# Huiweizhou/GCGCN

Measured on NVIDIA B200. Metric: document graphs/sec (fwd+bwd graph blocks), higher is better.
Workload: dtype f32

## Files before the change

### gcgcn_b200/_lib.py

```python
from __future__ import annotations

import ctypes
import glob
import os
import subprocess
import threading
from ctypes import c_float, c_int32, c_int64, c_size_t, c_uint64, c_void_p, c_char_p, POINTER

_HERE = os.path.dirname(os.path.abspath(__file__))
LIB_NAME = "libgcgcn_b200.so"
LIB_PATH = os.path.join(_HERE, LIB_NAME)
CSRC = os.path.join(_HERE, "csrc")
INCLUDE = os.path.join(os.path.dirname(_HERE), "include")

NVCC_FLAGS = [
    "-gencode", "arch=compute_100a,code=sm_100a", "-lineinfo", "-O3", "-std=c++17",
    "-Xcompiler", "-fPIC", "-shared",
]

F32, BF16 = 0, 1
STACK_RELU, STACK_RESIDUAL, STACK_LINEAR = 1, 2, 4


class GcgcnError(RuntimeError):
    pass


class Dropout(ctypes.Structure):
    _fields_ = [("seed", c_uint64), ("p_att", c_float), ("p_gcn", c_float)]


class Batch(ctypes.Structure):
    _fields_ = [
        ("num_docs", c_int32), ("total_nodes", c_int32), ("total_pairs", c_int64),
        ("max_nodes", c_int32), ("reserved", c_int32),
        ("node_ptr", c_void_p), ("pair_ptr", c_void_p), ("row_doc", c_void_p),
        ("doc_order", c_void_p), ("class_end", c_int32 * 4),
        ("tile_doc", c_void_p), ("num_tiles", c_int32), ("tile_rows", c_int32),
    ]


class EdgeTablesC(ctypes.Structure):
    _fields_ = [
        ("num_tokens", c_int32), ("num_slots", c_int32), ("num_pairs", c_int32), ("att_total", c_int32),
        ("dis_plus", c_int32), ("reserved", c_int32),
        ("tok_first", c_void_p), ("tok_slot_lo", c_void_p), ("tok_slot_hi", c_void_p),
        ("slot_tok0", c_void_p), ("slot_len", c_void_p), ("slot_span", c_void_p), ("slot_att", c_void_p),
        ("slot_rowi", c_void_p), ("slot_rowj", c_void_p), ("pair_idx", c_void_p), ("pair_slot_ptr", c_void_p),
        ("pair_denom", c_void_p), ("node_ctr_ptr", c_void_p), ("node_ctr", c_void_p),
        ("num_active_docs", c_int32), ("max_active_len", c_int32),
        ("adoc_tok0", c_void_p), ("adoc_len", c_void_p), ("adoc_slot_lo", c_void_p), ("adoc_slot_hi", c_void_p),
    ]


class RankResult(ctypes.Structure):
    _fields_ = [
        ("count", c_int64), ("total_recall", c_int64), ("best_pos", c_int64), ("w", c_int64),
        ("auc", ctypes.c_double), ("ign_auc", ctypes.c_double),
        ("f1", c_float), ("theta", c_float), ("f1_at_w", c_float), ("precision_at_w", c_float),
        ("recall_at_w", c_float), ("ign_f1", c_float), ("ign_f1_at_w", c_float), ("reserved", c_float),
    ]


def sources():
    return sorted(glob.glob(os.path.join(CSRC, "*.cu")))


def build(force: bool = False, verbose: bool = False) -> str:
    from concurrent.futures import ThreadPoolExecutor
    srcs = sources()
    hdrs = glob.glob(os.path.join(CSRC, "*.cuh")) + glob.glob(os.path.join(INCLUDE, "*.h"))
    newest_hdr = max(os.path.getmtime(p) for p in hdrs)
    if not force and os.path.exists(LIB_PATH):
        if os.path.getmtime(LIB_PATH) >= max([newest_hdr] + [os.path.getmtime(p) for p in srcs]):
            return LIB_PATH
    nvcc = os.environ.get("NVCC", "nvcc")
    objdir = os.path.join(os.path.dirname(_HERE), "build", "obj")
    os.makedirs(objdir, exist_ok=True)
    compile_flags = [f for f in NVCC_FLAGS if f != "-shared"]

    def compile_one(src):
        obj = os.path.join(objdir, os.path.basename(src)[:-3] + ".o")
        if not force and os.path.exists(obj) and os.path.getmtime(obj) >= max(newest_hdr, os.path.getmtime(src)):
            return obj, None
        cmd = [nvcc] + compile_flags + ["-I", INCLUDE, "-c", "-o", obj, src]
        if verbose:
            print(" ".join(cmd))
        res = subprocess.run(cmd, capture_output=True, text=True)
        return obj, (None if res.returncode == 0 else res.stdout + res.stderr)

    with ThreadPoolExecutor(max_workers=min(len(srcs), os.cpu_count() or 4)) as pool:
        results = list(pool.map(compile_one, srcs))
    errors = [e for _, e in results if e]
    if errors:
        raise GcgcnError("nvcc failed:\n" + "\n".join(errors))
    cmd = [nvcc, "-gencode", "arch=compute_100a,code=sm_100a", "-shared", "-o", LIB_PATH] + [o for o, _ in results]
    res = subprocess.run(cmd, capture_output=True, text=True)
    if res.returncode != 0:
        raise GcgcnError("nvcc link failed:\n" + res.stdout + res.stderr)
    return LIB_PATH


_P = c_void_p
_BT = POINTER(Batch)
_DP = POINTER(Dropout)
_ET = POINTER(EdgeTablesC)

SIGNATURES = {
    "gcgcn_version": (c_char_p, []),
    "gcgcn_last_error": (c_char_p, []),
    "gcgcn_launch_count": (c_uint64, []),
    "gcgcn_set_tile_blocks": (c_int32, [c_int32]),
    "gcgcn_device_info": (c_int32, [POINTER(c_int32)] * 3),
    "gcgcn_timing_begin": (c_int32, [_P]),
    "gcgcn_timing_end": (c_int32, [_P, c_char_p, c_size_t]),
    "gcgcn_workspace_bytes": (c_size_t, [c_int32, c_int64, c_int32]),
    "gcgcn_pool_fwd": (c_int32, [_P, _P, _P, _P, c_int32, _P, _P]),
    "gcgcn_pool_bwd": (c_int32, [_P, _P, _P, _P, c_int32, _P, _P]),
    "gcgcn_edge_mean_fwd": (c_int32, [_BT, _P, c_int32, _P, _P]),
    "gcgcn_edge_mean_bwd": (c_int32, [_BT, _P, c_int32, _P, _P]),
    "gcgcn_gat_fwd": (c_int32, [_BT, _P, _P, c_int32, _P, _P, _P, _P, c_int32, _P, _P, _P, _P,
                                _P, c_size_t, _P]),
    "gcgcn_gat_bwd": (c_int32, [_BT, _P, _P, c_int32, _P, _P, _P, c_int32, _P, _P, _P, _P,
                                _P, _P, _P, _P, _P, _P, c_size_t, _P]),
    "gcgcn_mha_fwd": (c_int32, [_BT, c_int32, _P, _P, _P, _P, _P, _P, _P, _P, c_size_t, _P]),
    "gcgcn_mha_bwd": (c_int32, [_BT, c_int32, _P, _P, _P, _P, _P, _P, _P, _P, _P, _P, c_size_t, _P]),
    "gcgcn_graphconv_stack_fwd": (c_int32, [_BT, c_int32, c_int32, c_int32, c_int32, c_int32]
                                  + [_P] * 13 + [_P, c_size_t, _P]),
    "gcgcn_graphconv_stack_bwd": (c_int32, [_BT, c_int32, c_int32, c_int32, c_int32, c_int32]
                                  + [_P] * 20 + [_P, c_size_t, _P]),
    "gcgcn_block_supported": (c_int32, [_BT, c_int32, c_int32, c_int32]),
    "gcgcn_dropout_mask": (c_int32, [c_uint64, c_int32, c_float, c_int64, _P, _P]),
    "gcgcn_mha_stack_fwd": (c_int32, [_BT, c_int32, c_int32] + [_P] * 15 + [_DP, _P, c_size_t, _P]),
    "gcgcn_mha_stack_bwd": (c_int32, [_BT, c_int32, c_int32] + [_P] * 22 + [_DP, _P, c_size_t, _P]),
    "gcgcn_pack_stack_weights": (c_int32, [_P, _P, c_int32, c_int32, c_int32, _P, _P, _P, _P]),
    "gcgcn_unpack_stack_grads": (c_int32, [_P, _P, _P, c_int32, c_int32, c_int32, _P, _P, _P]),
    "gcgcn_gat_collapse_fwd": (c_int32, [_P] * 8 + [c_int32, _P, _P]),
    "gcgcn_gat_collapse_bwd": (c_int32, [_P] * 8 + [c_int32] + [_P] * 8 + [_P]),
    "gcgcn_pack_rows": (c_int32, [_P, c_int32, c_int32, _P, _P]),
    "gcgcn_pair_gather_fwd": (c_int32, [_BT, _P, c_int32, _P, c_int32, _P, _P, _P, _P, _P, _P, _P]),
    "gcgcn_pair_gather_bwd": (c_int32, [_BT, _P, _P, c_int32, c_int32, c_int32, _P, _P, _P, _P,
                                        _P, c_size_t, _P]),
    "gcgcn_pair_dense_fwd": (c_int32, [_BT, _P, _P, _P, _P, _P, _P, _P, _P, _P]),
    "gcgcn_pair_dense_ws_bytes": (c_size_t, [c_int32]),
    "gcgcn_pair_dense_bwd": (c_int32, [_BT, _P, _P, _P, _P, c_int32, _P, _P, _P, _P, _P, _P, c_size_t, _P]),
    "gcgcn_block_saved_bytes": (c_size_t, [c_int32, c_int64, c_int32]),
    "gcgcn_caggc_fwd": (c_int32, [_BT, c_int32, _P, _P, c_int32] + [_P] * 8 + [_P, _P, _DP, _P, c_size_t, _P]),
    "gcgcn_caggc_bwd": (c_int32, [_BT, c_int32, _P, _P, c_int32] + [_P] * 6 + [_P, _P]
                        + [_P] * 10 + [_DP, _P, c_size_t, _P]),
    "gcgcn_maggc_fwd": (c_int32, [_BT, c_int32, c_int32, _P, _P, c_int32] + [_P] * 7
                        + [_P, _P, _DP, _P, c_size_t, _P]),
    "gcgcn_maggc_bwd": (c_int32, [_BT, c_int32, c_int32, _P, c_int32] + [_P] * 5 + [_P, _P]
                        + [_P] * 9 + [_DP, _P, c_size_t, _P]),
    "gcgcn_expand_pair_context": (c_int32, [_P, c_int32, c_int32, c_int32, c_int32, c_int32, _P, _P, _P, _P]),
    "gcgcn_edgefeat_ws_bytes": (c_size_t, [c_int32, c_int32, c_int32, c_int32, c_int64]),
    "gcgcn_word_table_fwd": (c_int32, [_P, _P, _P, _P, c_int32, _P, _P]),
    "gcgcn_word_table_bwd": (c_int32, [_P, _P, _P, _P, c_int32, _P, _P, _P, c_size_t, _P]),
    "gcgcn_word_pool_fwd": (c_int32, [_ET, _P, _P, _P, _P, _P]),
    "gcgcn_word_pool_bwd": (c_int32, [_ET, _P, _P, _P, _P, _P, _P, c_size_t, _P]),
    "gcgcn_sent_pool_fwd": (c_int32, [_ET, _P, _P, _P, _P, _P, _P, _P, _P]),
    "gcgcn_sent_pool_bwd": (c_int32, [_ET, c_int32] + [_P] * 10 + [_P, c_size_t, _P]),
    "gcgcn_edge_fill_fwd": (c_int32, [_P, _P, _P, c_int32, c_int64, c_int32, _P, _P]),
    "gcgcn_edge_fill_bwd": (c_int32, [_P, _P, c_int32, c_int64, c_int32, _P, _P, _P, c_size_t, _P]),
    "gcgcn_colsum": (c_int32, [_P, c_int32, c_int32, c_int32, _P, _P, c_size_t, _P]),
    "gcgcn_bilinear_ws_bytes": (c_size_t, [c_int32, c_int32]),
    "gcgcn_bilinear_fwd": (c_int32, [_P, _P, _P, _P, c_int32, c_int32, c_int32, _P, c_int32, _P, c_size_t, _P]),
    "gcgcn_bilinear_bwd_ws_bytes": (c_size_t, [c_int32, c_int32]),
    "gcgcn_bilinear_bwd": (c_int32, [_P, _P, _P, _P, _P, c_int32, c_int32, c_float, _P, _P, _P, _P, c_size_t, _P]),
    "gcgcn_bilinear_reduce_fwd": (c_int32, [_P, _P, _P, c_int32, c_int32, c_int32, _P, c_int32, _P]),
    "gcgcn_bilinear_outer_bwd": (c_int32, [_P, c_int32, _P, c_int32, c_int32, _P, _P]),
    "gcgcn_bilinear_dt_bwd": (c_int32, [_P, c_int32, _P, c_int32, c_int32, _P, _P]),
    "gcgcn_doc_bias_fwd": (c_int32, [_BT, _P, c_int32, _P, _P]),
    "gcgcn_doc_bias_bwd": (c_int32, [_BT, _P, c_int32, _P, _P]),
    "gcgcn_pair_bce_fwd": (c_int32, [_BT, _P, _P, c_int32, _P, _P]),
    "gcgcn_pair_bce_bwd": (c_int32, [_BT, _P, _P, c_int32, _P, _P, _P]),
    "gcgcn_rank_ws_bytes": (c_size_t, [c_int64]),
    "gcgcn_rank_candidates": (c_int32, [_BT, _P, c_int32, _P, _P, c_int64, _P, _P, _P, _P]),
    "gcgcn_rank_sort": (c_int32, [_P, _P, c_int64, _P, _P, _P, c_size_t, _P]),
    "gcgcn_rank_curve": (c_int32, [_P, _P, c_int64, c_int64, c_int32, ctypes.c_double, _P, _P, c_size_t, _P]),
    "gcgcn_rank_decode": (c_int32, [_P, _P, c_int64, c_int64, _P, _P, c_int32, c_int32, _P, _P, _P, _P, _P, _P]),
    "gcgcn_adam_step": (c_int32, [_P, _P, _P, _P, c_int64] + [c_float] * 6 + [c_int32, _P]),
    "gcgcn_gemm": (c_int32, [c_int32, c_int32, c_int32, c_int32, c_int32, c_float, _P, c_int32, _P,
                             c_int32, c_float, _P, c_int32, _P, _P, c_size_t, _P]),
}

_lib = None
_lock = threading.Lock()


def load() -> ctypes.CDLL:
    global _lib
    if _lib is not None:
        return _lib
    with _lock:
        if _lib is not None:
            return _lib
        if not os.path.exists(LIB_PATH):
            raise GcgcnError(
                f"{LIB_PATH} not found: run `python -c 'import __graft_entry__ as g; g.build()'`. "
                "gcgcn_b200 has no CPU or PyTorch fallback.")
        lib = ctypes.CDLL(LIB_PATH)
        for name, (res, args) in SIGNATURES.items():
            fn = getattr(lib, name)
            fn.restype = res
            fn.argtypes = args
        _lib = lib
    return _lib


def call(name: str, *args) -> None:
    lib = load()
    rc = getattr(lib, name)(*args)
    if rc != 0:
        raise GcgcnError(f"{name} failed (code {rc}): {lib.gcgcn_last_error().decode()}")


def launch_count() -> int:
    return int(load().gcgcn_launch_count())


def set_tile_blocks(enable: bool) -> bool:
    return bool(load().gcgcn_set_tile_blocks(1 if enable else 0))


def timing_begin(stream: int) -> None:
    call("gcgcn_timing_begin", stream)


def timing_end(stream: int) -> dict:
    buf = ctypes.create_string_buffer(1 << 16)
    call("gcgcn_timing_end", stream, buf, len(buf))
    out = {}
    for line in buf.value.decode().splitlines():
        name, cnt, ms, work = line.split("\t")
        out[name] = (int(cnt), float(ms), float(work))
    return out


def version() -> str:
    return load().gcgcn_version().decode()
```

### gcgcn_b200/csrc/api.cu

```cuda
#include <cstring>
#include <map>
#include <mutex>
#include <string>
#include <vector>

#include "common.cuh"

namespace gcgcn {

int launch_node_score(const float* x, const float* u, const float* c, float* ux, int rows, cudaStream_t st);
int launch_edge_fwd(const gcgcn_batch* bt, const void* e, int dtype, const float* v, const float* ux,
                    const uint8_t* mask, const float* keep, float* P, float* A, float* ebar, cudaStream_t st);
int launch_edge_bwd(const gcgcn_batch* bt, const void* e, int dtype, const float* v, const float* dS,
                    const float* debar, void* de, float* dv_partial, cudaStream_t st);
int edge_bwd_grid();
int node_bwd_grid();
int launch_softmax_bwd(const gcgcn_batch* bt, int heads, const float* P, const float* keep, const float* dA,
                       const uint8_t* mask, float* dS, cudaStream_t st);
int launch_gat_node_bwd(const gcgcn_batch* bt, const float* dS, const float* x, const float* u, float* dx,
                        float* partial, int* parts_out, cudaStream_t st);
int launch_reduce_partials(const float* partial, int parts, int width, float* out0, int width0, float* out1,
                           cudaStream_t st);
int launch_mha_fwd(const gcgcn_batch* bt, int heads, const float* q, const float* keep, float* P, float* A,
                   cudaStream_t st);
int launch_mha_bwd(const gcgcn_batch* bt, int heads, const float* q, const float* dS, float* dq, cudaStream_t st);
int launch_stack_fwd(const gcgcn_batch* bt, int heads, int layers, int slab, int flags, const float* A, float* Z,
                     const float* E, const float* Winner, const float* keep, const float* x, float* G, float* F,
                     float* frag_ws, cudaStream_t st);
int launch_stack_bwd(const gcgcn_batch* bt, int heads, int layers, int slab, int flags, const float* A, const float* Z,
                     const float* G, const float* Winner, const float* keep, const float* dF, float* dZ,
                     float* dE, float* dA, float* frag_ws, cudaStream_t st);
bool block_kernels_usable(const gcgcn_batch* bt, int heads, int layers, int slab, bool mha);
bool set_tile_blocks(bool on);
int launch_block_fwd(const gcgcn_batch* bt, int heads, int layers, const float* A, const float* q, float* P,
                     float* Z, const float* E, const float* Winner, const float* x, float* G, float* F,
                     float* frag_ws, const BlockDrop& drop, cudaStream_t st);
int launch_block_bwd(const gcgcn_batch* bt, int heads, int layers, int out_mode, const float* A, const float* q,
                     const float* Z, const float* G, const float* Winner, const float* dF, float* dZ, float* dE,
                     float* dOut, float* frag_ws, const BlockDrop& drop, cudaStream_t st);
int launch_dropout_mask(unsigned long long seed, uint32_t stream, uint32_t thr, float inv, long long count, float* out,
                        cudaStream_t st);
size_t block_frag_floats(int heads, int layers);
enum { ATT_GRAD_DA = 0, ATT_GRAD_DS = 1, ATT_GRAD_DQ = 2 };
int launch_gemm(int ta, int tb, int M, int N, int K, float alpha, const float* A, int lda, const float* B,
                int ldb, float beta, float* C, int ldc, const float* bias, void* ws, size_t ws_bytes,
                cudaStream_t st);
size_t gemm_presplit_bytes(int rows);
int launch_colsum(const float* X, int M, int N, int ldx, float* out, void* ws, size_t ws_bytes, cudaStream_t st);
int launch_gemm_batched(int ta, int tb, int M, int N, int K, float alpha, const float* A, int lda, const float* B,
                        int ldb, float beta, float* C, int ldc, int batch, long long sA, long long sB, long long sC,
                        void* ws, size_t ws_bytes, cudaStream_t st);
int launch_csr_gather(const float* src, const int* ptr, const int* idx, const float* w, int rows, float* out,
                      cudaStream_t st);
int launch_pair_gather_fwd(const gcgcn_batch* bt, const float* feat, int feat_w, const float* dis, int dis_w,
                           const int* h_idx, const int* t_idx, const int* dis_h, const int* dis_t, float* out_h,
                           float* out_t, cudaStream_t st);
int launch_pair_gather_bwd(const gcgcn_batch* bt, const float* dout_h, const float* dout_t, int feat_w,
                           int dis_w, int dis_rows, const int* dis_h, const int* dis_t, float* dfeat,
                           float* ddis, void* ws, size_t ws_bytes, cudaStream_t st);
int pair_dis_warps();
int launch_pair_dense_fwd(const gcgcn_batch* bt, const float* U, const float* Vd, const int* h_idx, const int* t_idx,
                          const int* dis_h, const int* dis_t, float* out_h, float* out_t, cudaStream_t st);
int launch_pair_dense_bwd(const gcgcn_batch* bt, const float* dout_h, const float* dout_t, const float* out_h,
                          const float* out_t, int dis_rows, const int* dis_h, const int* dis_t, float* dU, float* dVd,
                          float* dpre, void* ws, size_t ws_bytes, cudaStream_t st);
int launch_pack_stack(const float* const* wn_ptrs, const float* const* we_ptrs, int heads, int layers, int slab,
                      float* WnX, float* We, float* Winner, cudaStream_t st);
int launch_expand_pair_context(const int* slots, int num_slots, int n, int S, int L, int dis_plus, unsigned char* sen,
                               long long* pos_h, long long* pos_t, cudaStream_t st);
int launch_adam(float* p, const float* g, float* m, float* v, long long count, float lr, float b1, float b2,
                float eps, float wd, float gscale, int step, cudaStream_t st);
int launch_unpack_stack(const float* dWnX, const float* dWe, const float* dWinner, int heads, int layers, int slab,
                        float* dwn_flat, float* dwe_flat, cudaStream_t st);

int launch_word_table_fwd(const float* SF, const float* DF, const float* wa, const float* ba, int tokens, float* T,
                          cudaStream_t st);
int word_table_parts(int tokens);
int launch_word_table_bwd(const float* SF, const float* DF, const float* wa, const float* dT, int tokens, float* dSF,
                          float* out, float* partial, cudaStream_t st);
int launch_word_pool_fwd(const gcgcn_edge_tables* t, const float* T, const float* ctx, float* att, float* cwa,
                         cudaStream_t st);
int launch_word_pool_bwd(const gcgcn_edge_tables* t, const float* ctx, const float* att, const float* dcwa, float* dlog,
                         float* dctx, float* dT, cudaStream_t st);
int launch_sent_pool_fwd(const gcgcn_edge_tables* t, const float* cw, const float* sfeat, const float* nfeat,
                         const float* va, const float* ca, float* score, float* csa, cudaStream_t st);
int sent_pool_parts(int pairs);
int launch_sent_pool_bwd(const gcgcn_edge_tables* t, int total_nodes, const float* cw, const float* sfeat,
                         const float* nfeat, const float* va, const float* score, const float* dcsa, float* dcw,
                         float* dsfeat, float* dnfeat, float* out, float* dpre, float* partial, cudaStream_t st);
int launch_edge_fill_fwd(const float* bias, const float* rows, const void* pair_idx, int pairs, long long total_pairs,
                         int dtype, void* e, cudaStream_t st);
int edge_colsum_parts(long long total_pairs);
int launch_edge_fill_bwd(const void* de, const void* pair_idx, int pairs, long long total_pairs, int dtype, float* drows,
                         float* dbias, float* partial, cudaStream_t st);

int launch_bilinear_reduce(const float* Y, const float* t, const float* bias, int rows, int R, int accumulate, float* out,
                           int ldo, cudaStream_t st);
int launch_bilinear_finish(const float* part, long long ld, const float* bias, int rows, int R, int accumulate, float* out,
                           int ldo, cudaStream_t st);
int launch_gemm_rowop(int mode, int M, int N, int K, const float* A, int lda, const float* B, int ldb, const float* T,
                      float* out, long long ld, void* ws, size_t ws_bytes, cudaStream_t st);
int launch_gemm_wgrad_scaled(int M, int tiles, int K, const float* A, int lda, const float* T, const float* scale, int lds,
                             float beta, float* C, int ldc, void* ws, size_t ws_bytes, cudaStream_t st, void* pre_ws,
                             size_t pre_bytes);
int launch_bilinear_outer(const float* dout, int ldd, const float* t, int rows, int R, float* dY, cudaStream_t st);
int launch_bilinear_dt(const float* dout, int ldd, const float* Y, int rows, int R, float* dt, cudaStream_t st);
int launch_doc_bias_fwd(const gcgcn_batch* bt, const float* v, int R, float* z, cudaStream_t st);
int launch_doc_bias_bwd(const gcgcn_batch* bt, const float* dz, int R, float* dv, cudaStream_t st);
int launch_pair_bce_fwd(const gcgcn_batch* bt, const float* z, const float* y, int R, float* loss, cudaStream_t st);
int launch_pair_bce_bwd(const gcgcn_batch* bt, const float* z, const float* y, int R, const float* dloss, float* dz,
                        cudaStream_t st);

int launch_gat_collapse_fwd(const float* Wh, const float* bh, const float* Wt, const float* bt, const float* Wr,
                            const float* br, const float* w, const float* b, int hid, float* out, cudaStream_t st);
int launch_gat_collapse_bwd(const float* Wh, const float* bh, const float* Wt, const float* bt, const float* Wr,
                            const float* br, const float* w, const float* dout, int hid, float* dWh, float* dbh, float* dWt,
                            float* dbt, float* dWr, float* dbr, float* dw, float* db, cudaStream_t st);
int launch_pack_rows(const float* const* ptrs, int count, int elems, float* out, cudaStream_t st);
size_t rank_ws_bytes(long long count);
int launch_rank_candidates(const gcgcn_batch* bt, const float* z, const float* labels, const uint8_t* intrain, int R,
                           long long base_id, float* score, uint32_t* payload, unsigned long long* counters,
                           cudaStream_t st);
int launch_rank_sort(const float* score, const uint32_t* payload, long long count, uint32_t* sorted_key,
                     uint32_t* sorted_payload, void* ws, size_t ws_bytes, cudaStream_t st);
int launch_rank_curve(const uint32_t* key, const uint32_t* pay, long long count, long long T, int has_intrain,
                      double input_theta, gcgcn_rank_result* res, void* ws, size_t ws_bytes, cudaStream_t st);
int launch_rank_decode(const uint32_t* key, const uint32_t* pay, long long rows, const long long* doc_off,
                       const int* doc_n, int docs, int R, int* doc, int* row, int* col, int* rel, float* score,
                       cudaStream_t st);

std::atomic<uint64_t> g_launches{0};
std::atomic<bool> g_timing{false};

namespace {
// ... 363 lines not shown
    GCGCN_API_ENTER(stream);
    GCGCN_TRY(check_batch(bt));
    GCGCN_REQUIRE(heads >= 1 && D % heads == 0, "mha_bwd: head_num %d must divide %d", heads, D);
    if (bt->total_nodes == 0) return GCGCN_OK;
    GCGCN_TRY(check_device_ptr(x, "node_feat"));
    GCGCN_TRY(check_device_ptr(q, "q"));
    GCGCN_TRY(check_device_ptr(P, "P"));
    GCGCN_TRY(check_device_ptr(dA, "dA"));
    GCGCN_TRY(check_device_ptr(dx, "dx"));
    cudaStream_t st = static_cast<cudaStream_t>(stream);
    Arena ar(ws, ws_bytes);
    float* dS = ar.take<float>(static_cast<size_t>(bt->total_pairs) * heads);
    float* dq = ar.take<float>(static_cast<size_t>(bt->total_nodes) * D);
    float* gws = ar.take<float>(GEMM_WS_BYTES / sizeof(float));
    if (dS == nullptr || dq == nullptr || gws == nullptr)
        return fail(GCGCN_ERR_WORKSPACE, "mha_bwd: workspace too small");
    GCGCN_TRY(launch_softmax_bwd(bt, heads, P, keep, dA, nullptr, dS, st));
    GCGCN_TRY(launch_mha_bwd(bt, heads, q, dS, dq, st));
    GCGCN_TRY(launch_gemm(0, 0, bt->total_nodes, D, D, 1.f, dq, D, Wq, D, 0.f, dx, D, nullptr, gws, GEMM_WS_BYTES, st));
    if (dWq != nullptr)
        GCGCN_TRY(launch_gemm(1, 0, D, D, bt->total_nodes, 1.f, dq, D, x, D, 0.f, dWq, D, nullptr, gws, GEMM_WS_BYTES, st));
    if (dbq != nullptr) GCGCN_TRY(launch_colsum(dq, bt->total_nodes, D, D, dbq, gws, GEMM_WS_BYTES, st));
    return GCGCN_OK;
}

static int stack_fwd_impl(const gcgcn_batch* bt, int32_t heads, int32_t layers, int32_t in_dim, int32_t slab,
                          int32_t flags, const float* x, const float* ebar, const float* A, const float* q, float* P,
                          const float* WnX, const float* We, const float* Winner, const float* Wout,
                          const float* bout, const float* keep, float* Z, float* G, float* F, float* y, void* ws,
                          size_t ws_bytes, cudaStream_t st, const BlockDrop& drop = BlockDrop{}) {
    const bool linear = flags & GCGCN_STACK_LINEAR;
    const int HD = heads * slab, M = bt->total_nodes;
    Arena ar(ws, ws_bytes);
    float* E = ar.take<float>(static_cast<size_t>(M) * HD);
    float* gws = ar.take<float>(GEMM_WS_BYTES / sizeof(float));
    float* frag = (slab == D && layers > 1 && D % layers == 0) ? ar.take<float>(block_frag_floats(heads, layers)) : nullptr;
    if (E == nullptr || gws == nullptr) return fail(GCGCN_ERR_WORKSPACE, "stack_fwd: workspace too small");
    GCGCN_TRY(launch_gemm(0, 0, M, HD, in_dim, 1.f, x, in_dim, WnX, HD, 0.f, Z, HD, nullptr, gws, GEMM_WS_BYTES, st));
    GCGCN_TRY(launch_gemm(0, 0, M, HD, D, 1.f, ebar, D, We, HD, 0.f, E, HD, nullptr, gws, GEMM_WS_BYTES, st));
    float* Fout = linear ? F : y;
    if (q != nullptr)
        GCGCN_TRY(launch_block_fwd(bt, heads, layers, nullptr, q, P, Z, E, Winner, x, G, Fout, frag, drop, st));
    else if (drop_active(drop))
        GCGCN_TRY(launch_block_fwd(bt, heads, layers, A, nullptr, nullptr, Z, E, Winner, x, G, Fout, frag, drop, st));
    else
        GCGCN_TRY(launch_stack_fwd(bt, heads, layers, slab, flags, A, Z, E, Winner, keep, x, G, Fout, frag, st));
    if (linear)
        GCGCN_TRY(launch_gemm(0, 1, M, D, HD, 1.f, F, HD, Wout, HD, 0.f, y, D, bout, gws, GEMM_WS_BYTES, st));
    return GCGCN_OK;
}

int gcgcn_graphconv_stack_fwd(const gcgcn_batch* bt, int32_t heads, int32_t layers, int32_t in_dim,
                              int32_t slab, int32_t flags, const float* x, const float* ebar, const float* A,
                              const float* WnX, const float* We, const float* Winner, const float* Wout,
                              const float* bout, const float* keep, float* Z, float* G, float* F, float* y,
                              void* ws, size_t ws_bytes, void* stream) {
    GCGCN_API_ENTER(stream);
    GCGCN_TRY(check_batch(bt));
    GCGCN_REQUIRE(heads >= 1 && layers >= 1 && in_dim >= 1 && slab >= 1, "stack_fwd: bad heads/layers/widths");
    const bool linear = flags & GCGCN_STACK_LINEAR;
    GCGCN_REQUIRE(linear || heads == 1, "stack_fwd: without the output linear there can be only one head");
    GCGCN_REQUIRE(!(flags & GCGCN_STACK_RESIDUAL) || in_dim == slab,
                  "stack_fwd: the residual needs input width %d == output width %d", in_dim, slab);
    if (bt->total_nodes == 0) return GCGCN_OK;
    GCGCN_TRY(check_device_ptr(x, "node_feat"));
    GCGCN_TRY(check_device_ptr(ebar, "ebar"));
    GCGCN_TRY(check_device_ptr(A, "adj_matrix"));
    GCGCN_TRY(check_device_ptr(WnX, "WnX"));
    GCGCN_TRY(check_device_ptr(We, "We"));
    GCGCN_TRY(check_device_ptr(Z, "Z"));
    GCGCN_TRY(check_device_ptr(G, "G"));
    GCGCN_TRY(check_device_ptr(y, "y"));
    if (linear) GCGCN_TRY(check_device_ptr(F, "F"));
    return stack_fwd_impl(bt, heads, layers, in_dim, slab, flags, x, ebar, A, nullptr, nullptr, WnX, We, Winner, Wout,
                          bout, keep, Z, G, F, y, ws, ws_bytes, static_cast<cudaStream_t>(stream));
}

static int stack_bwd_impl(const gcgcn_batch* bt, int32_t heads, int32_t layers, int32_t in_dim, int32_t slab,
                          int32_t flags, int att_grad, const float* x, const float* ebar, const float* A,
                          const float* q, const float* WnX, const float* We, const float* Winner, const float* Wout,
                          const float* keep, const float* Z, const float* G, const float* F, const float* dy,
                          float* dx, float* debar, float* att_out, float* dWnX, float* dWe, float* dWinner,
                          float* dWout, float* dbout, void* ws, size_t ws_bytes, cudaStream_t st,
                          const BlockDrop& drop = BlockDrop{}) {
    const bool linear = flags & GCGCN_STACK_LINEAR;
    const int HD = heads * slab, M = bt->total_nodes, gd = slab / layers;
    Arena ar(ws, ws_bytes);
    float* dFbuf = linear ? ar.take<float>(static_cast<size_t>(M) * HD) : nullptr;
    float* dZ = ar.take<float>(static_cast<size_t>(M) * HD);
    float* dE = ar.take<float>(static_cast<size_t>(M) * HD);
    float* gws = ar.take<float>(GEMM_WS_BYTES / sizeof(float));
    float* frag = (slab == D && layers > 1 && D % layers == 0) ? ar.take<float>(block_frag_floats(heads, layers)) : nullptr;
    if ((linear && dFbuf == nullptr) || dZ == nullptr || dE == nullptr || gws == nullptr)
        return fail(GCGCN_ERR_WORKSPACE, "stack_bwd: workspace too small");
    const float* dF = dy;
    if (linear) {
        GCGCN_TRY(launch_gemm(0, 0, M, HD, D, 1.f, dy, D, Wout, HD, 0.f, dFbuf, HD, nullptr, gws, GEMM_WS_BYTES, st));
        if (dWout != nullptr)
            GCGCN_TRY(launch_gemm(1, 0, D, HD, M, 1.f, dy, D, F, HD, 0.f, dWout, HD, nullptr, gws, GEMM_WS_BYTES, st));
        if (dbout != nullptr) GCGCN_TRY(launch_colsum(dy, M, D, D, dbout, gws, GEMM_WS_BYTES, st));
        dF = dFbuf;
    }
    if (att_grad == ATT_GRAD_DA)
        GCGCN_TRY(launch_stack_bwd(bt, heads, layers, slab, flags, A, Z, G, Winner, keep, dF, dZ, dE, att_out, frag, st));
    else
        GCGCN_TRY(launch_block_bwd(bt, heads, layers, att_grad, A, q, Z, G, Winner, dF, dZ, dE, att_out, frag, drop, st));
    float beta = 0.f;
    if (flags & GCGCN_STACK_RESIDUAL) {
        float* Wsum = (linear && heads > 1 && slab == D && in_dim == D) ? ar.take<float>(static_cast<size_t>(D) * D) : nullptr;
        if (Wsum != nullptr) {
            wout_head_sum_kernel<<<ceil_div(D * D, 256), 256, 0, st>>>(Wout, heads, Wsum);
            GCGCN_CHECK_LAUNCH("wout_head_sum");
            GCGCN_TRY(launch_gemm(0, 0, M, D, D, 1.f, dy, D, Wsum, D, 0.f, dx, D, nullptr, gws, GEMM_WS_BYTES, st));
        } else {
            GCGCN_TRY(launch_head_sum(dF, heads, M, dx, st));
        }
        beta = 1.f;
    }
    GCGCN_TRY(launch_gemm(0, 1, M, in_dim, HD, 1.f, dZ, HD, WnX, HD, beta, dx, in_dim, nullptr, gws, GEMM_WS_BYTES, st));
    GCGCN_TRY(launch_gemm(0, 1, M, D, HD, 1.f, dE, HD, We, HD, 0.f, debar, D, nullptr, gws, GEMM_WS_BYTES, st));
    if (dWnX != nullptr)
        GCGCN_TRY(launch_gemm(1, 0, in_dim, HD, M, 1.f, x, in_dim, dZ, HD, 0.f, dWnX, HD, nullptr, gws, GEMM_WS_BYTES, st));
    if (dWe != nullptr)
        GCGCN_TRY(launch_gemm(1, 0, D, HD, M, 1.f, ebar, D, dE, HD, 0.f, dWe, HD, nullptr, gws, GEMM_WS_BYTES, st));
    if (dWinner != nullptr && layers > 1) {
        GCGCN_TRY(cuda_ok(cudaMemsetAsync(dWinner, 0, static_cast<size_t>(heads) * layers * slab * gd * sizeof(float), st),
                          "memset dWinner"));
        for (int l = 1; l < layers; ++l)
            GCGCN_TRY(launch_gemm_batched(1, 0, l * gd, gd, M, 1.f, G, HD, dZ + l * gd, HD, 0.f,
                                          dWinner + static_cast<size_t>(l) * slab * gd, gd, heads, slab, slab,
                                          static_cast<long long>(layers) * slab * gd, gws, GEMM_WS_BYTES, st));
    }
    return GCGCN_OK;
}

int gcgcn_graphconv_stack_bwd(const gcgcn_batch* bt, int32_t heads, int32_t layers, int32_t in_dim,
                              int32_t slab, int32_t flags, const float* x, const float* ebar, const float* A,
                              const float* WnX, const float* We, const float* Winner, const float* Wout,
                              const float* keep, const float* Z, const float* G, const float* F,
                              const float* dy, float* dx, float* debar, float* dA, float* dWnX, float* dWe,
                              float* dWinner, float* dWout, float* dbout, void* ws, size_t ws_bytes,
                              void* stream) {
    GCGCN_API_ENTER(stream);
    GCGCN_TRY(check_batch(bt));
    GCGCN_REQUIRE(heads >= 1 && layers >= 1 && in_dim >= 1 && slab >= 1 && slab % layers == 0,
                  "stack_bwd: bad heads/layers/widths");
    const bool linear = flags & GCGCN_STACK_LINEAR;
    GCGCN_REQUIRE(linear || heads == 1, "stack_bwd: without the output linear there can be only one head");
    GCGCN_REQUIRE(!(flags & GCGCN_STACK_RESIDUAL) || (in_dim == slab && slab == D),
                  "stack_bwd: the residual needs input width == output width == %d", D);
    if (bt->total_nodes == 0) return GCGCN_OK;
    GCGCN_TRY(check_device_ptr(x, "node_feat"));
    GCGCN_TRY(check_device_ptr(A, "adj_matrix"));
    GCGCN_TRY(check_device_ptr(Z, "Z"));
    GCGCN_TRY(check_device_ptr(G, "G"));
    GCGCN_TRY(check_device_ptr(dy, "dy"));
    GCGCN_TRY(check_device_ptr(dx, "dx"));
    GCGCN_TRY(check_device_ptr(debar, "debar"));
    GCGCN_TRY(check_device_ptr(dA, "dA"));
    return stack_bwd_impl(bt, heads, layers, in_dim, slab, flags, ATT_GRAD_DA, x, ebar, A, nullptr, WnX, We, Winner,
                          Wout, keep, Z, G, F, dy, dx, debar, dA, dWnX, dWe, dWinner, dWout, dbout, ws, ws_bytes,
                          static_cast<cudaStream_t>(stream));
}

int gcgcn_dropout_mask(uint64_t seed, int32_t stream_id, float p, int64_t count, float* out, void* stream) {
    GCGCN_API_ENTER(stream);
    GCGCN_REQUIRE(p >= 0.f && p < 1.f && count >= 0 && stream_id >= 0, "dropout_mask: bad arguments");
    if (count == 0) return GCGCN_OK;
    GCGCN_TRY(check_device_ptr(out, "out"));
    return launch_dropout_mask(seed, static_cast<uint32_t>(stream_id), drop_threshold(p), 1.0f / (1.0f - p), count, out,
                               static_cast<cudaStream_t>(stream));
}

int gcgcn_block_supported(const gcgcn_batch* bt, int32_t heads, int32_t layers, int32_t mha) {
    if (bt == nullptr || layers < 1 || D % layers != 0) return 0;
    return block_kernels_usable(bt, heads, layers, D, mha != 0) ? 1 : 0;
}

int gcgcn_mha_stack_fwd(const gcgcn_batch* bt, int32_t heads, int32_t layers, const float* x, const float* ebar,
                        const float* Wq, const float* bq, const float* WnX, const float* We, const float* Winner,
                        const float* Wout, const float* bout, float* q, float* P, float* Z, float* G, float* F,
                        float* y, const gcgcn_dropout* dropout, void* ws, size_t ws_bytes, void* stream) {
    GCGCN_API_ENTER(stream);
    GCGCN_TRY(check_batch(bt));
    BlockDrop drop;
    GCGCN_TRY(make_block_drop(dropout, DROP_STREAM_MHA, DROP_STREAM_MAGGC, &drop));
    GCGCN_REQUIRE(heads >= 1 && layers >= 1 && D % layers == 0, "mha_stack_fwd: bad heads/layers");
    if (!block_kernels_usable(bt, heads, layers, D, true))
        return fail(GCGCN_ERR_UNSUPPORTED, "mha_stack_fwd: needs documents of <= 64 nodes, 2 or 4 sub-layers and 4 or 8 "
                    "heads (got max_nodes %d, layers %d, heads %d); use gcgcn_mha_fwd + gcgcn_graphconv_stack_fwd",
                    bt->max_nodes, layers, heads);
    if (bt->total_nodes == 0) return GCGCN_OK;
    GCGCN_TRY(check_device_ptr(x, "node_feat"));
    GCGCN_TRY(check_device_ptr(ebar, "ebar"));
    GCGCN_TRY(check_device_ptr(Wq, "Wq"));
    GCGCN_TRY(check_device_ptr(WnX, "WnX"));
    GCGCN_TRY(check_device_ptr(We, "We"));
    GCGCN_TRY(check_device_ptr(Wout, "Wout"));
    GCGCN_TRY(check_device_ptr(q, "q"));
    GCGCN_TRY(check_device_ptr(P, "P"));
    GCGCN_TRY(check_device_ptr(Z, "Z"));
    GCGCN_TRY(check_device_ptr(G, "G"));
    GCGCN_TRY(check_device_ptr(F, "F"));
    GCGCN_TRY(check_device_ptr(y, "y"));
    cudaStream_t st = static_cast<cudaStream_t>(stream);
    GCGCN_TRY(launch_gemm(0, 1, bt->total_nodes, D, D, 1.f, x, D, Wq, D, 0.f, q, D, bq, ws, ws_bytes, st));
    return stack_fwd_impl(bt, heads, layers, D, D, BLOCK_FLAGS_ALL, x, ebar, nullptr, q, P, WnX, We, Winner, Wout, bout,
                          nullptr, Z, G, F, y, ws, ws_bytes, st, drop);
}

int gcgcn_mha_stack_bwd(const gcgcn_batch* bt, int32_t heads, int32_t layers, const float* x, const float* ebar,
                        const float* Wq, const float* WnX, const float* We, const float* Winner, const float* Wout,
                        const float* q, const float* P, const float* Z, const float* G, const float* F,
                        const float* dy, float* dx, float* debar, float* dWq, float* dbq, float* dWnX, float* dWe,
                        float* dWinner, float* dWout, float* dbout, const gcgcn_dropout* dropout, void* ws,
                        size_t ws_bytes, void* stream) {
    GCGCN_API_ENTER(stream);
    GCGCN_TRY(check_batch(bt));
    BlockDrop drop;
    GCGCN_TRY(make_block_drop(dropout, DROP_STREAM_MHA, DROP_STREAM_MAGGC, &drop));
    GCGCN_REQUIRE(heads >= 1 && layers >= 1 && D % layers == 0, "mha_stack_bwd: bad heads/layers");
    if (!block_kernels_usable(bt, heads, layers, D, true))
        return fail(GCGCN_ERR_UNSUPPORTED, "mha_stack_bwd: unsupported configuration (see gcgcn_mha_stack_fwd)");
    if (bt->total_nodes == 0) return GCGCN_OK;
    GCGCN_TRY(check_device_ptr(x, "node_feat"));
    GCGCN_TRY(check_device_ptr(q, "q"));
    GCGCN_TRY(check_device_ptr(P, "P"));
    GCGCN_TRY(check_device_ptr(Z, "Z"));
    GCGCN_TRY(check_device_ptr(G, "G"));
    GCGCN_TRY(check_device_ptr(dy, "dy"));
    GCGCN_TRY(check_device_ptr(dx, "dx"));
    GCGCN_TRY(check_device_ptr(debar, "debar"));
    cudaStream_t st = static_cast<cudaStream_t>(stream);
    Arena ar(ws, ws_bytes);
    float* dq = ar.take<float>(static_cast<size_t>(bt->total_nodes) * D);
    if (dq == nullptr) return fail(GCGCN_ERR_WORKSPACE, "mha_stack_bwd: workspace too small");
    void* rest = static_cast<char*>(ws) + ar.off;
    const size_t rest_bytes = ws_bytes - ar.off;
    GCGCN_TRY(stack_bwd_impl(bt, heads, layers, D, D, BLOCK_FLAGS_ALL, ATT_GRAD_DQ, x, ebar, P, q, WnX, We, Winner, Wout,
                             nullptr, Z, G, F, dy, dx, debar, dq, dWnX, dWe, dWinner, dWout, dbout, rest, rest_bytes, st,
                             drop));
    Arena ar2(rest, rest_bytes);
    float* gws = ar2.take<float>(GEMM_WS_BYTES / sizeof(float));
    if (gws == nullptr) return fail(GCGCN_ERR_WORKSPACE, "mha_stack_bwd: workspace too small");
    GCGCN_TRY(launch_gemm(0, 0, bt->total_nodes, D, D, 1.f, dq, D, Wq, D, 1.f, dx, D, nullptr, gws, GEMM_WS_BYTES, st));
    if (dWq != nullptr)
        GCGCN_TRY(launch_gemm(1, 0, D, D, bt->total_nodes, 1.f, dq, D, x, D, 0.f, dWq, D, nullptr, gws, GEMM_WS_BYTES, st));
    if (dbq != nullptr) GCGCN_TRY(launch_colsum(dq, bt->total_nodes, D, D, dbq, gws, GEMM_WS_BYTES, st));
    return GCGCN_OK;
}

int gcgcn_pack_stack_weights(const void* wn_ptrs, const void* we_ptrs, int32_t heads, int32_t layers, int32_t slab,
                             float* WnX, float* We, float* Winner, void* stream) {
    GCGCN_API_ENTER(stream);
    GCGCN_REQUIRE(heads >= 1 && layers >= 1 && slab >= 1 && slab % layers == 0, "pack_stack: bad heads/layers/slab");
    GCGCN_REQUIRE(layers == 1 || Winner != nullptr, "pack_stack: Winner is required when layers > 1");
    GCGCN_TRY(check_device_ptr(wn_ptrs, "wn_ptrs"));
    GCGCN_TRY(check_device_ptr(we_ptrs, "we_ptrs"));
    GCGCN_TRY(check_device_ptr(WnX, "WnX"));
    GCGCN_TRY(check_device_ptr(We, "We"));
    return launch_pack_stack(static_cast<const float* const*>(wn_ptrs), static_cast<const float* const*>(we_ptrs),
                             heads, layers, slab, WnX, We, Winner, static_cast<cudaStream_t>(stream));
}

int gcgcn_unpack_stack_grads(const float* dWnX, const float* dWe, const float* dWinner, int32_t heads,
                             int32_t layers, int32_t slab, float* dwn_flat, float* dwe_flat, void* stream) {
    GCGCN_API_ENTER(stream);
    GCGCN_REQUIRE(heads >= 1 && layers >= 1 && slab >= 1 && slab % layers == 0, "unpack_stack: bad heads/layers/slab");
    GCGCN_REQUIRE(layers == 1 || dWinner != nullptr, "unpack_stack: dWinner is required when layers > 1");
    GCGCN_TRY(check_device_ptr(dWnX, "dWnX"));
    GCGCN_TRY(check_device_ptr(dWe, "dWe"));
    GCGCN_TRY(check_device_ptr(dwn_flat, "dwn_flat"));
    GCGCN_TRY(check_device_ptr(dwe_flat, "dwe_flat"));
    return launch_unpack_stack(dWnX, dWe, dWinner, heads, layers, slab, dwn_flat, dwe_flat,
                               static_cast<cudaStream_t>(stream));
}

int gcgcn_gat_collapse_fwd(const float* Wh, const float* bh, const float* Wt, const float* bt, const float* Wr,
                           const float* br, const float* w, const float* b, int32_t hid, float* out, void* stream) {
    GCGCN_API_ENTER(stream);
    GCGCN_REQUIRE(hid >= 1, "gat_collapse_fwd: hidden_dim < 1");
    const void* ps[] = {Wh, bh, Wt, bt, Wr, br, w, b, out};
    for (const void* p : ps) GCGCN_TRY(check_device_ptr(p, "gat_collapse operand"));
    return launch_gat_collapse_fwd(Wh, bh, Wt, bt, Wr, br, w, b, hid, out, static_cast<cudaStream_t>(stream));
}
int gcgcn_gat_collapse_bwd(const float* Wh, const float* bh, const float* Wt, const float* bt, const float* Wr,
                           const float* br, const float* w, const float* dout, int32_t hid, float* dWh, float* dbh,
                           float* dWt, float* dbt, float* dWr, float* dbr, float* dw, float* db, void* stream) {
    GCGCN_API_ENTER(stream);
    GCGCN_REQUIRE(hid >= 1, "gat_collapse_bwd: hidden_dim < 1");
    const void* ps[] = {Wh, bh, Wt, bt, Wr, br, w, dout, dWh, dbh, dWt, dbt, dWr, dbr, dw, db};
    for (const void* p : ps) GCGCN_TRY(check_device_ptr(p, "gat_collapse operand"));
    return launch_gat_collapse_bwd(Wh, bh, Wt, bt, Wr, br, w, dout, hid, dWh, dbh, dWt, dbt, dWr, dbr, dw, db,
                                   static_cast<cudaStream_t>(stream));
}
int gcgcn_pack_rows(const void* ptrs, int32_t count, int32_t elems, float* out, void* stream) {
    GCGCN_API_ENTER(stream);
    GCGCN_REQUIRE(count >= 0 && elems >= 0, "pack_rows: negative size");
    if (count == 0 || elems == 0) return GCGCN_OK;
    GCGCN_TRY(check_device_ptr(ptrs, "ptrs"));
    GCGCN_TRY(check_device_ptr(out, "out"));
    return launch_pack_rows(static_cast<const float* const*>(ptrs), count, elems, out, static_cast<cudaStream_t>(stream));
}

int gcgcn_pair_gather_fwd(const gcgcn_batch* bt, const float* feat, int32_t feat_w, const float* dis,
                          int32_t dis_w, const int32_t* h_idx, const int32_t* t_idx, const int32_t* dis_h,
                          const int32_t* dis_t, float* out_h, float* out_t, void* stream) {
    GCGCN_API_ENTER(stream);
    GCGCN_TRY(check_batch(bt));
    GCGCN_REQUIRE(feat_w > 0 && feat_w % 4 == 0 && dis_w >= 0 && dis_w % 4 == 0,
                  "pair_gather: widths must be multiples of 4 (feat_w=%d, dis_w=%d)", feat_w, dis_w);
    if (bt->total_pairs == 0) return GCGCN_OK;
    GCGCN_TRY(check_device_ptr(feat, "feat"));
    GCGCN_TRY(check_device_ptr(h_idx, "h_idx"));
    GCGCN_TRY(check_device_ptr(t_idx, "t_idx"));
    GCGCN_TRY(check_device_ptr(out_h, "out_h"));
    GCGCN_TRY(check_device_ptr(out_t, "out_t"));
    if (dis_w > 0) {
        GCGCN_TRY(check_device_ptr(dis, "dis"));
        GCGCN_TRY(check_device_ptr(dis_h, "dis_h"));
        GCGCN_TRY(check_device_ptr(dis_t, "dis_t"));
    }
    return launch_pair_gather_fwd(bt, feat, feat_w, dis, dis_w, h_idx, t_idx, dis_h, dis_t, out_h, out_t,
                                  static_cast<cudaStream_t>(stream));
}

int gcgcn_pair_gather_bwd(const gcgcn_batch* bt, const float* dout_h, const float* dout_t, int32_t feat_w,
                          int32_t dis_w, int32_t dis_rows, const int32_t* dis_h, const int32_t* dis_t,
                          float* dfeat, float* ddis, void* ws, size_t ws_bytes, void* stream) {
    GCGCN_API_ENTER(stream);
// ... 399 lines not shown
                     int32_t has_intrain, double input_theta, gcgcn_rank_result* result, void* ws, size_t ws_bytes,
                     void* stream) {
    GCGCN_API_ENTER(stream);
    GCGCN_REQUIRE(count >= 1 && count < GCGCN_RANK_MAX_CANDIDATES, "rank_curve: count %lld outside [1, 2^30)",
                  static_cast<long long>(count));
    GCGCN_TRY(check_device_ptr(sorted_key, "sorted_key"));
    GCGCN_TRY(check_device_ptr(sorted_payload, "sorted_payload"));
    GCGCN_REQUIRE((reinterpret_cast<uintptr_t>(sorted_payload) & 15) == 0, "rank_curve: sorted_payload not 16-byte aligned");
    GCGCN_TRY(check_device_ptr(result, "result"));
    GCGCN_TRY(check_device_ptr(ws, "ws"));
    GCGCN_REQUIRE(ws_bytes >= rank_ws_bytes(count), "rank_curve: ws_bytes %zu < gcgcn_rank_ws_bytes = %zu", ws_bytes,
                  rank_ws_bytes(count));
    return launch_rank_curve(sorted_key, sorted_payload, count, total_recall < 1 ? 1 : total_recall, has_intrain ? 1 : 0,
                             input_theta, result, ws, ws_bytes, static_cast<cudaStream_t>(stream));
}
int gcgcn_rank_decode(const uint32_t* sorted_key, const uint32_t* sorted_payload, int64_t rows, int64_t count,
                      const int64_t* doc_offsets, const int32_t* doc_n, int32_t num_docs, int32_t relations, int32_t* doc,
                      int32_t* row, int32_t* col, int32_t* relation, float* score, void* stream) {
    GCGCN_API_ENTER(stream);
    GCGCN_REQUIRE(rows >= 0 && num_docs >= 1 && relations >= 2, "rank_decode: bad shape");
    GCGCN_REQUIRE(rows <= count, "rank_decode: rows %lld > count %lld of the ranking", static_cast<long long>(rows),
                  static_cast<long long>(count));
    if (rows == 0) return GCGCN_OK;
    GCGCN_TRY(check_device_ptr(sorted_key, "sorted_key"));
    GCGCN_TRY(check_device_ptr(sorted_payload, "sorted_payload"));
    GCGCN_TRY(check_device_ptr(doc_offsets, "doc_offsets"));
    GCGCN_TRY(check_device_ptr(doc_n, "doc_n"));
    GCGCN_TRY(check_device_ptr(doc, "doc"));
    GCGCN_TRY(check_device_ptr(row, "row"));
    GCGCN_TRY(check_device_ptr(col, "col"));
    GCGCN_TRY(check_device_ptr(relation, "relation"));
    GCGCN_TRY(check_device_ptr(score, "score"));
    return launch_rank_decode(sorted_key, sorted_payload, rows, reinterpret_cast<const long long*>(doc_offsets), doc_n,
                              num_docs, relations, doc, row, col, relation, score, static_cast<cudaStream_t>(stream));
}

int gcgcn_expand_pair_context(const int32_t* slots, int32_t num_slots, int32_t n, int32_t max_num, int32_t length,
                              int32_t dis_plus, uint8_t* sen_matrix, int64_t* pos_matrix_h, int64_t* pos_matrix_t,
                              void* stream) {
    GCGCN_API_ENTER(stream);
    GCGCN_REQUIRE(num_slots >= 0 && n >= 0 && max_num >= 0 && length >= 0, "expand_pair_context: negative size");
    if (static_cast<size_t>(n) * n * max_num * length == 0) return GCGCN_OK;
    GCGCN_TRY(check_device_ptr(sen_matrix, "sen_matrix"));
    GCGCN_TRY(check_device_ptr(pos_matrix_h, "pos_matrix_h"));
    GCGCN_TRY(check_device_ptr(pos_matrix_t, "pos_matrix_t"));
    if (num_slots > 0) GCGCN_TRY(check_device_ptr(slots, "slots"));
    return launch_expand_pair_context(slots, num_slots, n, max_num, length, dis_plus, sen_matrix,
                                      reinterpret_cast<long long*>(pos_matrix_h),
                                      reinterpret_cast<long long*>(pos_matrix_t), static_cast<cudaStream_t>(stream));
}

int gcgcn_adam_step(float* params, const float* grads, float* exp_avg, float* exp_avg_sq, int64_t count,
                    float lr, float beta1, float beta2, float eps, float weight_decay, float grad_scale,
                    int32_t step, void* stream) {
    GCGCN_API_ENTER(stream);
    GCGCN_REQUIRE(count >= 0 && step >= 1, "adam_step: count >= 0 and step >= 1 required");
    GCGCN_REQUIRE(beta1 >= 0.f && beta1 < 1.f && beta2 >= 0.f && beta2 < 1.f && eps > 0.f, "adam_step: bad betas/eps");
    if (count == 0) return GCGCN_OK;
    GCGCN_TRY(check_device_ptr(params, "params"));
    GCGCN_TRY(check_device_ptr(grads, "grads"));
    GCGCN_TRY(check_device_ptr(exp_avg, "exp_avg"));
    GCGCN_TRY(check_device_ptr(exp_avg_sq, "exp_avg_sq"));
    GCGCN_REQUIRE(((reinterpret_cast<uintptr_t>(params) | reinterpret_cast<uintptr_t>(grads) |
                    reinterpret_cast<uintptr_t>(exp_avg) | reinterpret_cast<uintptr_t>(exp_avg_sq)) & 15) == 0,
                  "adam_step: buffers must be 16-byte aligned");
    return launch_adam(params, grads, exp_avg, exp_avg_sq, count, lr, beta1, beta2, eps, weight_decay, grad_scale,
                       step, static_cast<cudaStream_t>(stream));
}

int gcgcn_gemm(int32_t ta, int32_t tb, int32_t M, int32_t N, int32_t K, float alpha, const float* A,
               int32_t lda, const float* B, int32_t ldb, float beta, float* C, int32_t ldc, const float* bias,
               void* ws, size_t ws_bytes, void* stream) {
    GCGCN_API_ENTER(stream);
    GCGCN_REQUIRE(M >= 0 && N >= 0 && K >= 0, "gemm: negative dimension");
    if (M == 0 || N == 0) return GCGCN_OK;
    GCGCN_TRY(check_device_ptr(C, "C"));
    if (K > 0) {
        GCGCN_TRY(check_device_ptr(A, "A"));
        GCGCN_TRY(check_device_ptr(B, "B"));
    }
    const size_t head = ws_bytes < GEMM_WS_BYTES ? ws_bytes : GEMM_WS_BYTES;
    return launch_gemm(ta, tb, M, N, K, alpha, A, lda, B, ldb, beta, C, ldc, bias, ws, head,
                       static_cast<cudaStream_t>(stream));
}

namespace {
struct CagSaved { float *P, *ebar, *Z, *G, *F; };
struct MagSaved { float *ebar, *q, *P, *Z, *G, *F; };

CagSaved carve_cag(void* saved, int nodes, long long pairs) {
    Arena ar(saved, ~size_t(0) >> 1);
    CagSaved s;
    s.P = ar.take<float>(pairs);
    s.ebar = ar.take<float>(static_cast<size_t>(nodes) * D);
    s.Z = ar.take<float>(static_cast<size_t>(nodes) * D);
    s.G = ar.take<float>(static_cast<size_t>(nodes) * D);
    s.F = ar.take<float>(static_cast<size_t>(nodes) * D);
    return s;
}
MagSaved carve_mag(void* saved, int nodes, long long pairs, int heads) {
    Arena ar(saved, ~size_t(0) >> 1);
    MagSaved s;
    s.ebar = ar.take<float>(static_cast<size_t>(nodes) * D);
    s.q = ar.take<float>(static_cast<size_t>(nodes) * D);
    s.P = ar.take<float>(static_cast<size_t>(pairs) * heads);
    s.Z = ar.take<float>(static_cast<size_t>(nodes) * heads * D);
    s.G = ar.take<float>(static_cast<size_t>(nodes) * heads * D);
    s.F = ar.take<float>(static_cast<size_t>(nodes) * heads * D);
    return s;
}
constexpr int BLOCK_FLAGS = GCGCN_STACK_RELU | GCGCN_STACK_RESIDUAL | GCGCN_STACK_LINEAR;
}

size_t gcgcn_block_saved_bytes(int32_t total_nodes, int64_t total_pairs, int32_t heads) {
    const size_t nodes = static_cast<size_t>(total_nodes), h = static_cast<size_t>(heads < 1 ? 1 : heads);
    return align256(static_cast<size_t>(total_pairs) * h * sizeof(float)) +
           2 * align256(nodes * D * sizeof(float)) + 3 * align256(nodes * h * D * sizeof(float)) + 1024;
}

int gcgcn_caggc_fwd(const gcgcn_batch* bt, int32_t layers, const float* x, const void* e, int32_t edge_dtype,
                    const float* u, const float* v, const float* c, const float* WnX, const float* We,
                    const float* Winner, const float* Wout, const float* bout, float* y, void* saved,
                    const gcgcn_dropout* dropout, void* ws, size_t ws_bytes, void* stream) {
    ::gcgcn::StreamDeviceGuard outer_guard__(static_cast<cudaStream_t>(stream));
    GCGCN_TRY(check_batch(bt));
    GCGCN_TRY(check_device_ptr(saved, "saved"));
    BlockDrop drop;
    GCGCN_TRY(make_block_drop(dropout, DROP_STREAM_GAT, DROP_STREAM_CAGGC, &drop));
    CagSaved s = carve_cag(saved, bt->total_nodes, bt->total_pairs);
    GCGCN_TRY(gcgcn_gat_fwd(bt, x, e, edge_dtype, u, v, c, nullptr, 0, nullptr, s.P, s.P, s.ebar, ws, ws_bytes, stream));
    if (!drop_active(drop))
        return gcgcn_graphconv_stack_fwd(bt, 1, layers, D, D, BLOCK_FLAGS, x, s.ebar, s.P, WnX, We, Winner, Wout, bout,
                                         nullptr, s.Z, s.G, s.F, y, ws, ws_bytes, stream);
    if (!block_kernels_usable(bt, 1, layers, D, false))
        return fail(GCGCN_ERR_UNSUPPORTED, "caggc_fwd: in-kernel dropout needs documents of <= 64 nodes and 2 or 4 "
                    "sub-layers; pass keep masks through gcgcn_gat_fwd / gcgcn_graphconv_stack_fwd instead");
    GCGCN_API_ENTER(stream);
    return stack_fwd_impl(bt, 1, layers, D, D, BLOCK_FLAGS, x, s.ebar, s.P, nullptr, nullptr, WnX, We, Winner, Wout, bout,
                          nullptr, s.Z, s.G, s.F, y, ws, ws_bytes, static_cast<cudaStream_t>(stream), drop);
}

int gcgcn_caggc_bwd(const gcgcn_batch* bt, int32_t layers, const float* x, const void* e, int32_t edge_dtype,
                    const float* u, const float* v, const float* WnX, const float* We, const float* Winner,
                    const float* Wout, const float* dy, const void* saved, float* dx, void* de, float* du,
                    float* dv, float* dc, float* dWnX, float* dWe, float* dWinner, float* dWout, float* dbout,
                    const gcgcn_dropout* dropout, void* ws, size_t ws_bytes, void* stream) {
    ::gcgcn::StreamDeviceGuard outer_guard__(static_cast<cudaStream_t>(stream));
    GCGCN_TRY(check_batch(bt));
    GCGCN_TRY(check_device_ptr(saved, "saved"));
    BlockDrop drop;
    GCGCN_TRY(make_block_drop(dropout, DROP_STREAM_GAT, DROP_STREAM_CAGGC, &drop));
    CagSaved s = carve_cag(const_cast<void*>(saved), bt->total_nodes, bt->total_pairs);
    Arena ar(ws, ws_bytes);
    float* dx_stack = ar.take<float>(static_cast<size_t>(bt->total_nodes) * D);
    float* debar = ar.take<float>(static_cast<size_t>(bt->total_nodes) * D);
    float* dA = ar.take<float>(bt->total_pairs);
    if (dx_stack == nullptr || debar == nullptr || dA == nullptr)
        return fail(GCGCN_ERR_WORKSPACE, "caggc_bwd: workspace too small");
    void* rest = static_cast<char*>(ws) + ar.off;
    const size_t rest_bytes = ws_bytes - ar.off;
    cudaStream_t st = static_cast<cudaStream_t>(stream);
    if (block_kernels_usable(bt, 1, layers, D, false)) {
        float* dS = dA;
        GCGCN_API_ENTER(stream);
        GCGCN_TRY(stack_bwd_impl(bt, 1, layers, D, D, BLOCK_FLAGS, ATT_GRAD_DS, x, s.ebar, s.P, nullptr, WnX, We, Winner,
                                 Wout, nullptr, s.Z, s.G, s.F, dy, dx_stack, debar, dS, dWnX, dWe, dWinner, dWout, dbout,
// ... 68 lines not shown
```

### gcgcn_b200/csrc/common.cuh

```cuda
#pragma once

#include <cuda_bf16.h>
#include <cuda_runtime.h>

#include <algorithm>
#include <atomic>
#include <cstdarg>
#include <cstdint>
#include <cstdio>

#include "../../include/gcgcn_b200.h"

namespace gcgcn {

constexpr int D = GCGCN_HIDDEN;
constexpr int WARP = 32;

char* error_buffer();
int fail(int code, const char* fmt, ...);
extern std::atomic<uint64_t> g_launches;
extern std::atomic<bool> g_timing;
void timing_mark(const char* name, cudaStream_t st);
void timing_set_work(double work);

// ... 16 lines not shown
    explicit StreamDeviceGuard(cudaStream_t st) {
        int dev = -1;
        if (st == nullptr) return;
        cudaStreamCaptureStatus cap = cudaStreamCaptureStatusNone;
        if (cudaStreamIsCapturing(st, &cap) != cudaSuccess) { cudaGetLastError(); return; }
        if (cap != cudaStreamCaptureStatusNone) return;
        if (cudaStreamGetDevice(st, &dev) != cudaSuccess) { cudaGetLastError(); return; }
        if (cudaGetDevice(&prev) != cudaSuccess) { cudaGetLastError(); return; }
        if (prev != dev && cudaSetDevice(dev) == cudaSuccess) switched = true;
    }
    ~StreamDeviceGuard() { if (switched) cudaSetDevice(prev); }
    StreamDeviceGuard(const StreamDeviceGuard&) = delete;
    StreamDeviceGuard& operator=(const StreamDeviceGuard&) = delete;
};

inline bool device_prepared(const std::atomic<unsigned long long>& mask) {
    int dev = 0;
    if (cudaGetDevice(&dev) != cudaSuccess || dev < 0 || dev >= 64) return false;
    return (mask.load(std::memory_order_acquire) >> dev) & 1ULL;
}
inline void device_mark_prepared(std::atomic<unsigned long long>& mask) {
    int dev = 0;
    if (cudaGetDevice(&dev) != cudaSuccess || dev < 0 || dev >= 64) return;
    mask.fetch_or(1ULL << dev, std::memory_order_release);
}

template <typename K>
inline int set_smem(K kernel, size_t bytes, const char* name) {
    if (bytes > 227 * 1024)
        return fail(GCGCN_ERR_UNSUPPORTED, "%s needs %zu bytes of shared memory (> 227 KB): documents "
                    "this large are not supported", name, bytes);
    if (bytes > 48 * 1024)
        return cuda_ok(cudaFuncSetAttribute(kernel, cudaFuncAttributeMaxDynamicSharedMemorySize,
                                            static_cast<int>(bytes)), name);
    return GCGCN_OK;
}
template <typename K>
inline int set_smem_once(std::atomic<unsigned long long>& mask, K kernel, size_t bytes, const char* name) {
    if (device_prepared(mask)) return GCGCN_OK;
    const int rc = set_smem(kernel, bytes, name);
    if (rc == GCGCN_OK) device_mark_prepared(mask);
    return rc;
}

#define GCGCN_API_ENTER(stream)                                                          \
    ::gcgcn::StreamDeviceGuard device_guard__(static_cast<cudaStream_t>(stream));        \
    do {                                                                                 \
        if (::gcgcn::g_timing.load(std::memory_order_relaxed))                           \
            ::gcgcn::timing_mark("(between calls)", static_cast<cudaStream_t>(stream));  \
    } while (0)

#define GCGCN_TRY(expr)                    \
    do {                                   \
        int rc__ = (expr);                 \
        if (rc__ != GCGCN_OK) return rc__; \
    } while (0)

#define GCGCN_REQUIRE(cond, ...)                                        \
    do {                                                                \
        if (!(cond)) return ::gcgcn::fail(GCGCN_ERR_INVALID_ARG, __VA_ARGS__); \
    } while (0)

int sm_count();
int check_batch(const gcgcn_batch* bt);
int check_device_ptr(const void* p, const char* name);

struct Arena {
    char* base;
    size_t cap;
    size_t off = 0;
    Arena(void* p, size_t bytes) : base(static_cast<char*>(p)), cap(bytes) {}
    template <typename T>
    T* take(size_t count) {
        size_t bytes = (count * sizeof(T) + 255) & ~size_t(255);
        if (base == nullptr || off + bytes > cap) return nullptr;
        T* p = reinterpret_cast<T*>(base + off);
        off += bytes;
        return p;
    }
};

static inline int ceil_div(long long a, long long b) { return static_cast<int>((a + b - 1) / b); }

template <class LaunchFn>
inline int for_each_size_class(const gcgcn_batch* bt, LaunchFn fn) {
    if (bt->doc_order == nullptr) return fn(bt->num_docs, 0, bt->max_nodes, static_cast<const int*>(nullptr));
    static const int cap[4] = {64, 48, 32, 16};
    int first = 0;
    for (int c = 0; c < 4; ++c) {
        const int count = bt->class_end[c] - first;
        if (count > 0) GCGCN_TRY(fn(count, first, cap[c] < bt->max_nodes ? cap[c] : bt->max_nodes, bt->doc_order));
        first = bt->class_end[c] > first ? bt->class_end[c] : first;
    }
    return GCGCN_OK;
}

__device__ __forceinline__ float logit_sigmoid(float z) { return 1.0f / (1.0f + expf(-z)); }
__device__ __forceinline__ float warp_sum(float v) {
#pragma unroll
    for (int o = 16; o > 0; o >>= 1) v += __shfl_xor_sync(0xffffffffu, v, o);
    return v;
}
__device__ __forceinline__ float warp_max(float v) {
#pragma unroll
    for (int o = 16; o > 0; o >>= 1) v = fmaxf(v, __shfl_xor_sync(0xffffffffu, v, o));
    return v;
}

struct BlockDrop {
    unsigned long long seed;
    uint32_t thr_att, thr_gcn;
    float inv_att, inv_gcn;
    uint32_t s_att, s_gcn;
};
__host__ __device__ __forceinline__ unsigned long long drop_hash(unsigned long long seed, uint32_t stream,
                                                                  unsigned long long pair_idx) {
    unsigned long long z = seed + 0x9E3779B97F4A7C15ULL * (pair_idx + (static_cast<unsigned long long>(stream) << 56) + 1ULL);
    z = (z ^ (z >> 30)) * 0xBF58476D1CE4E5B9ULL;
    z = (z ^ (z >> 27)) * 0x94D049BB133111EBULL;
    return z ^ (z >> 31);
}
__host__ __device__ __forceinline__ float drop_keep(unsigned long long seed, uint32_t stream, unsigned long long idx,
                                                    uint32_t thr, float inv) {
    const unsigned long long h = drop_hash(seed, stream, idx >> 1);
    const uint32_t r = (idx & 1ULL) ? static_cast<uint32_t>(h >> 32) : static_cast<uint32_t>(h);
    return r >= thr ? inv : 0.f;
}
__host__ __device__ __forceinline__ float2 drop_keep2(unsigned long long seed, uint32_t stream, unsigned long long idx,
                                                      uint32_t thr, float inv) {
    const unsigned long long h = drop_hash(seed, stream, idx >> 1);
    return make_float2(static_cast<uint32_t>(h) >= thr ? inv : 0.f, static_cast<uint32_t>(h >> 32) >= thr ? inv : 0.f);
}

template <typename T>
struct Vec4;

template <>
struct Vec4<float> {
    static __device__ __forceinline__ float4 load(const float* p) {
        float4 r;
        asm volatile("ld.global.nc.L1::no_allocate.v4.f32 {%0,%1,%2,%3}, [%4];"
                     : "=f"(r.x), "=f"(r.y), "=f"(r.z), "=f"(r.w)
                     : "l"(p));
        return r;
    }
    static __device__ __forceinline__ void store(float* p, float4 v) {
        asm volatile("st.global.L1::no_allocate.v4.f32 [%0], {%1,%2,%3,%4};" ::"l"(p), "f"(v.x),
                     "f"(v.y), "f"(v.z), "f"(v.w)
                     : "memory");
    }
};

template <>
struct Vec4<__nv_bfloat16> {
    static __device__ __forceinline__ float4 load(const __nv_bfloat16* p) {
        uint32_t a, b;
        asm volatile("ld.global.nc.L1::no_allocate.v2.u32 {%0,%1}, [%2];" : "=r"(a), "=r"(b) : "l"(p));
        float4 r;
        r.x = __uint_as_float(a << 16);
        r.y = __uint_as_float(a & 0xffff0000u);
        r.z = __uint_as_float(b << 16);
        r.w = __uint_as_float(b & 0xffff0000u);
        return r;
    }
    static __device__ __forceinline__ void store(__nv_bfloat16* p, float4 v) {
        __nv_bfloat162 lo = __floats2bfloat162_rn(v.x, v.y);
// ... 10 lines not shown
```

### gcgcn_b200/csrc/gemm.cu

```cuda
#include "common.cuh"

namespace gcgcn {

constexpr int GM = 64, GN = 64, GK = 16, GEMM_THREADS = 256;
constexpr int LDS_A = GM + 4, LDS_B = GN + 4;

template <bool TA, bool TB>
__global__ void __launch_bounds__(GEMM_THREADS)
gemm_kernel(int M, int N, int K, float alpha, const float* __restrict__ A, int lda,
            const float* __restrict__ B, int ldb, float beta, float* __restrict__ C, int ldc,
            const float* __restrict__ bias, float* __restrict__ partial, int k_per_split) {
    __shared__ __align__(16) float As[2][GK * LDS_A];
    __shared__ __align__(16) float Bs[2][GK * LDS_B];
    const int m0 = blockIdx.y * GM, n0 = blockIdx.x * GN;
    const int kbeg = blockIdx.z * k_per_split;
    const int kend = min(K, kbeg + k_per_split);
    const int tid = threadIdx.x;
    const int tx = tid & 15, ty = tid >> 4;

    float acc[4][4];
#pragma unroll
    for (int i = 0; i < 4; ++i)
#pragma unroll
        for (int j = 0; j < 4; ++j) acc[i][j] = 0.f;
// ... 25 lines not shown
            }
        } else {
            const int m = tid >> 2, k4 = (tid & 3) * 4;
            float v[4];
            if (a_vec && m0 + m < M && k0 + k4 + 4 <= kend) {
                float4 t = *reinterpret_cast<const float4*>(A + static_cast<size_t>(m0 + m) * lda + k0 + k4);
                v[0] = t.x; v[1] = t.y; v[2] = t.z; v[3] = t.w;
            } else {
#pragma unroll
                for (int q = 0; q < 4; ++q) v[q] = a_at(m0 + m, k0 + k4 + q);
            }
#pragma unroll
            for (int q = 0; q < 4; ++q) as[(k4 + q) * LDS_A + m] = v[q];
        }
        if (!TB) {
            const int k = tid >> 4, n4 = (tid & 15) * 4;
            if (b_vec && k0 + k < kend) {
                float4 v = *reinterpret_cast<const float4*>(B + static_cast<size_t>(k0 + k) * ldb + n0 + n4);
                *reinterpret_cast<float4*>(bs + k * LDS_B + n4) = v;
            } else {
#pragma unroll
                for (int q = 0; q < 4; ++q) bs[k * LDS_B + n4 + q] = b_at(k0 + k, n0 + n4 + q);
            }
        } else {
            const int n = tid >> 2, k4 = (tid & 3) * 4;
            float v[4];
            if (b_vec && n0 + n < N && k0 + k4 + 4 <= kend) {
                float4 t = *reinterpret_cast<const float4*>(B + static_cast<size_t>(n0 + n) * ldb + k0 + k4);
                v[0] = t.x; v[1] = t.y; v[2] = t.z; v[3] = t.w;
            } else {
#pragma unroll
                for (int q = 0; q < 4; ++q) v[q] = b_at(k0 + k4 + q, n0 + n);
            }
#pragma unroll
            for (int q = 0; q < 4; ++q) bs[(k4 + q) * LDS_B + n] = v[q];
        }
    };

    int buf = 0;
    if (kbeg < kend) load_tiles(0, kbeg);
    __syncthreads();
    for (int k0 = kbeg; k0 < kend; k0 += GK) {
        if (k0 + GK < kend) load_tiles(buf ^ 1, k0 + GK);
        const float* as = As[buf];
        const float* bs = Bs[buf];
#pragma unroll
        for (int k = 0; k < GK; ++k) {
            const float4 a = *reinterpret_cast<const float4*>(as + k * LDS_A + ty * 4);
            const float4 b = *reinterpret_cast<const float4*>(bs + k * LDS_B + tx * 4);
            const float av[4] = {a.x, a.y, a.z, a.w};
            const float bv[4] = {b.x, b.y, b.z, b.w};
#pragma unroll
            for (int i = 0; i < 4; ++i)
#pragma unroll
                for (int j = 0; j < 4; ++j) acc[i][j] = fmaf(av[i], bv[j], acc[i][j]);
        }
        __syncthreads();
        buf ^= 1;
    }

#pragma unroll
    for (int i = 0; i < 4; ++i) {
        const int m = m0 + ty * 4 + i;
        if (m >= M) continue;
#pragma unroll
        for (int j = 0; j < 4; ++j) {
            const int n = n0 + tx * 4 + j;
            if (n >= N) continue;
            if (partial != nullptr) {
                partial[(static_cast<size_t>(blockIdx.z) * M + m) * N + n] = acc[i][j];
            } else {
                float v = alpha * acc[i][j];
                if (bias != nullptr) v += bias[n];
                float* c = C + static_cast<size_t>(m) * ldc + n;
                if (beta != 0.f) v += beta * (*c);
                *c = v;
            }
        }
    }
}

__global__ void __launch_bounds__(256)
splitk_reduce_kernel(const float* __restrict__ partial, int splits, int M, int N, float alpha, float beta,
                     float* __restrict__ C, int ldc, const float* __restrict__ bias, long long batch_stride_c) {
    const size_t idx = static_cast<size_t>(blockIdx.x) * blockDim.x + threadIdx.x;
    const size_t total = static_cast<size_t>(M) * N;
    if (idx >= total) return;
    partial += static_cast<size_t>(blockIdx.y) * splits * total;
    C += static_cast<size_t>(blockIdx.y) * batch_stride_c;
    float s0 = 0.f, s1 = 0.f, s2 = 0.f, s3 = 0.f;
    int p = 0;
    for (; p + 4 <= splits; p += 4) {
        s0 += partial[(p + 0) * total + idx];
        s1 += partial[(p + 1) * total + idx];
        s2 += partial[(p + 2) * total + idx];
        s3 += partial[(p + 3) * total + idx];
    }
    for (; p < splits; ++p) s0 += partial[p * total + idx];
    const float s = (s0 + s1) + (s2 + s3);
    const int m = static_cast<int>(idx / N), n = static_cast<int>(idx - static_cast<size_t>(m) * N);
    float v = alpha * s;
    if (bias != nullptr) v += bias[n];
    float* c = C + static_cast<size_t>(m) * ldc + n;
    if (beta != 0.f) v += beta * (*c);
    *c = v;
}

__global__ void __launch_bounds__(256)
splitk_reduce4_kernel(const float* __restrict__ partial, int splits, int M, int N, float alpha, float beta,
                      float* __restrict__ C, int ldc, const float* __restrict__ bias, long long batch_stride_c) {
    const size_t idx = static_cast<size_t>(blockIdx.x) * blockDim.x + threadIdx.x;
    const size_t total4 = static_cast<size_t>(M) * N / 4;
    if (idx >= total4) return;
    const float4* part = reinterpret_cast<const float4*>(partial) + static_cast<size_t>(blockIdx.y) * splits * total4;
    C += static_cast<size_t>(blockIdx.y) * batch_stride_c;
    float4 a = make_float4(0.f, 0.f, 0.f, 0.f), b = a;
    int p = 0;
    for (; p + 2 <= splits; p += 2) {
        const float4 u = part[(p + 0) * total4 + idx], w = part[(p + 1) * total4 + idx];
        a.x += u.x; a.y += u.y; a.z += u.z; a.w += u.w;
        b.x += w.x; b.y += w.y; b.z += w.z; b.w += w.w;
    }
    if (p < splits) {
        const float4 u = part[p * total4 + idx];
        a.x += u.x; a.y += u.y; a.z += u.z; a.w += u.w;
    }
    const int m = static_cast<int>(idx / (N / 4)), n = static_cast<int>(idx - static_cast<size_t>(m) * (N / 4)) * 4;
    float4 v = make_float4(alpha * (a.x + b.x), alpha * (a.y + b.y), alpha * (a.z + b.z), alpha * (a.w + b.w));
    if (bias != nullptr) {
        const float4 bb = *reinterpret_cast<const float4*>(bias + n);
        v.x += bb.x; v.y += bb.y; v.z += bb.z; v.w += bb.w;
    }
    float4* c = reinterpret_cast<float4*>(C + static_cast<size_t>(m) * ldc + n);
    if (beta != 0.f) {
        const float4 cur = *c;
        v.x += beta * cur.x; v.y += beta * cur.y; v.z += beta * cur.z; v.w += beta * cur.w;
    }
    *c = v;
}

__global__ void __launch_bounds__(256)
splitk_reduce4_wide_kernel(const float* __restrict__ partial, int splits, int M, int N, float alpha, float beta,
                           float* __restrict__ C, int ldc, const float* __restrict__ bias, long long batch_stride_c) {
    __shared__ float4 sm[8][32];
    const int cx = threadIdx.x & 31, sy = threadIdx.x >> 5;
    const size_t idx = static_cast<size_t>(blockIdx.x) * 32 + cx;
    const size_t total4 = static_cast<size_t>(M) * N / 4;
    const float4* part = reinterpret_cast<const float4*>(partial) + static_cast<size_t>(blockIdx.y) * splits * total4;
    C += static_cast<size_t>(blockIdx.y) * batch_stride_c;
    float4 a = make_float4(0.f, 0.f, 0.f, 0.f);
    if (idx < total4) {
#pragma unroll 4
        for (int p = sy; p < splits; p += 8) {
            const float4 u = part[static_cast<size_t>(p) * total4 + idx];
            a.x += u.x; a.y += u.y; a.z += u.z; a.w += u.w;
        }
    }
    sm[sy][cx] = a;
    __syncthreads();
    if (sy != 0 || idx >= total4) return;
#pragma unroll
    for (int y = 1; y < 8; ++y) {
        const float4 u = sm[y][cx];
        a.x += u.x; a.y += u.y; a.z += u.z; a.w += u.w;
    }
    const int m = static_cast<int>(idx / (N / 4)), n = static_cast<int>(idx - static_cast<size_t>(m) * (N / 4)) * 4;
    float4 v = make_float4(alpha * a.x, alpha * a.y, alpha * a.z, alpha * a.w);
    if (bias != nullptr) {
        const float4 bb = *reinterpret_cast<const float4*>(bias + n);
        v.x += bb.x; v.y += bb.y; v.z += bb.z; v.w += bb.w;
    }
    float4* c = reinterpret_cast<float4*>(C + static_cast<size_t>(m) * ldc + n);
    if (beta != 0.f) {
        const float4 cur = *c;
        v.x += beta * cur.x; v.y += beta * cur.y; v.z += beta * cur.z; v.w += beta * cur.w;
    }
    *c = v;
}

__global__ void __launch_bounds__(256)
colsum_partial_kernel(const float* __restrict__ X, int M, int N, int ldx, int rows_per_block,
                      float* __restrict__ partial) {
    const int c = blockIdx.x * blockDim.x + threadIdx.x;
    if (c >= N) return;
    const int r0 = blockIdx.y * rows_per_block;
    const int r1 = min(M, r0 + rows_per_block);
    float s = 0.f;
    for (int r = r0; r < r1; ++r) s += X[static_cast<size_t>(r) * ldx + c];
    partial[static_cast<size_t>(blockIdx.y) * N + c] = s;
}

__global__ void __launch_bounds__(256)
colsum128_partial_kernel(const float* __restrict__ X, int M, int ldx, int rows_per_block, float* __restrict__ partial) {
    __shared__ float4 red[8][32];
    const int cl = threadIdx.x & 31, rl = threadIdx.x >> 5;
    const int r0 = blockIdx.x * rows_per_block;
    const int r1 = min(M, r0 + rows_per_block);
    float4 s = make_float4(0.f, 0.f, 0.f, 0.f);
    for (int r = r0 + rl; r < r1; r += 8) {
        const float4 v = *reinterpret_cast<const float4*>(X + static_cast<size_t>(r) * ldx + 4 * cl);
        s.x += v.x; s.y += v.y; s.z += v.z; s.w += v.w;
    }
    red[rl][cl] = s;
    __syncthreads();
    if (rl == 0) {
        float4 t = red[0][cl];
#pragma unroll
        for (int r = 1; r < 8; ++r) { const float4 v = red[r][cl]; t.x += v.x; t.y += v.y; t.z += v.z; t.w += v.w; }
        *reinterpret_cast<float4*>(partial + static_cast<size_t>(blockIdx.x) * 128 + 4 * cl) = t;
    }
}

int launch_reduce_partials(const float* partial, int parts, int width, float* out0, int width0,
                           float* out1, cudaStream_t st);

int launch_splitk_reduce(const float* partial, int splits, int M, int N, float alpha, float beta, float* C,
                         int ldc, const float* bias, cudaStream_t st, int batch = 1, long long sC = 0) {
    const size_t total = static_cast<size_t>(M) * N;
    const bool vec = N % 4 == 0 && ldc % 4 == 0 && sC % 4 == 0 && (reinterpret_cast<uintptr_t>(C) & 15) == 0 &&
                     (reinterpret_cast<uintptr_t>(partial) & 15) == 0 &&
                     (bias == nullptr || (reinterpret_cast<uintptr_t>(bias) & 15) == 0);
    if (vec && splits >= 16 && total / 4 <= 64 * 1024) {
        dim3 grid(ceil_div(total / 4, 32), batch);
        splitk_reduce4_wide_kernel<<<grid, 256, 0, st>>>(partial, splits, M, N, alpha, beta, C, ldc, bias, sC);
    } else if (vec) {
        dim3 grid(ceil_div(total / 4, 256), batch);
        splitk_reduce4_kernel<<<grid, 256, 0, st>>>(partial, splits, M, N, alpha, beta, C, ldc, bias, sC);
    } else {
        dim3 grid(ceil_div(total, 256), batch);
        splitk_reduce_kernel<<<grid, 256, 0, st>>>(partial, splits, M, N, alpha, beta, C, ldc, bias, sC);
    }
    GCGCN_CHECK_LAUNCH("splitk_reduce");
    return GCGCN_OK;
}

int launch_gemm_tc(int ta, int tb, int M, int N, int K, float alpha, const float* A, int lda, const float* B,
                   int ldb, float beta, float* C, int ldc, const float* bias, void* ws, size_t ws_bytes,
                   cudaStream_t st, int* taken, int batch, long long sA, long long sB, long long sC, void* pre_ws,
                   size_t pre_bytes, const float* bscale = nullptr, int lds = 0);

int launch_gemm(int ta, int tb, int M, int N, int K, float alpha, const float* A, int lda,
                const float* B, int ldb, float beta, float* C, int ldc, const float* bias, void* ws,
                size_t ws_bytes, cudaStream_t st) {
    if (M <= 0 || N <= 0) return GCGCN_OK;
    if (K < 0) return fail(GCGCN_ERR_INVALID_ARG, "gemm: K < 0");
    int taken = 0;
    GCGCN_TRY(launch_gemm_tc(ta, tb, M, N, K, alpha, A, lda, B, ldb, beta, C, ldc, bias, ws, ws_bytes, st, &taken,
                             1, 0, 0, 0, nullptr, 0));
    if (taken) return GCGCN_OK;
    const int tiles = ceil_div(M, GM) * ceil_div(N, GN);
    int splits = 1;
    const int target = 2 * sm_count();
    if (tiles < target && K >= 2048) {
        splits = min(ceil_div(target, tiles), ceil_div(K, 512));
        const size_t per = static_cast<size_t>(M) * N * sizeof(float);
        if (ws == nullptr || per == 0) splits = 1;
        else splits = static_cast<int>(std::min<size_t>(splits, ws_bytes / per));
        if (splits < 2) splits = 1;
    }
    int k_per = K;
    float* partial = nullptr;
    if (splits > 1) {
        k_per = ceil_div(ceil_div(K, splits), GK) * GK;
        splits = ceil_div(K, k_per);
        partial = static_cast<float*>(ws);
    }
    if (k_per == 0) k_per = GK;
    dim3 grid(ceil_div(N, GN), ceil_div(M, GM), splits);
#define GCGCN_GEMM(TA, TB)                                                                          \
    gemm_kernel<TA, TB><<<grid, GEMM_THREADS, 0, st>>>(M, N, K, alpha, A, lda, B, ldb, beta, C, ldc, \
                                                       bias, partial, k_per)
    if (!ta && !tb) GCGCN_GEMM(false, false);
    else if (!ta && tb) GCGCN_GEMM(false, true);
    else if (ta && !tb) GCGCN_GEMM(true, false);
    else GCGCN_GEMM(true, true);
#undef GCGCN_GEMM
    timing_set_work(2.0 * M * N * K);
    GCGCN_CHECK_LAUNCH(ta ? (tb ? "gemm_tt" : "gemm_tn") : (tb ? "gemm_nt" : "gemm_nn"));
    if (splits > 1) GCGCN_TRY(launch_splitk_reduce(partial, splits, M, N, alpha, beta, C, ldc, bias, st));
    return GCGCN_OK;
}

int launch_gemm_wgrad_scaled(int M, int tiles, int K, const float* A, int lda, const float* T, const float* scale, int lds,
                             float beta, float* C, int ldc, void* ws, size_t ws_bytes, cudaStream_t st, void* pre_ws,
                             size_t pre_bytes) {
    int taken = 0;
    GCGCN_TRY(launch_gemm_tc(1, 0, M, tiles * 128, K, 1.f, A, lda, T, 128, beta, C, ldc, nullptr, ws, ws_bytes, st, &taken, 1, 0,
                             0, 0, pre_ws, pre_bytes, scale, lds));
    if (!taken) return fail(GCGCN_ERR_UNSUPPORTED, "gemm_wgrad_scaled: shape not covered by the tensor-core path");
    return GCGCN_OK;
}

int launch_gemm_batched(int ta, int tb, int M, int N, int K, float alpha, const float* A, int lda, const float* B,
                        int ldb, float beta, float* C, int ldc, int batch, long long sA, long long sB, long long sC,
                        void* ws, size_t ws_bytes, cudaStream_t st) {
    if (M <= 0 || N <= 0 || batch <= 0) return GCGCN_OK;
    int taken = 0;
    GCGCN_TRY(launch_gemm_tc(ta, tb, M, N, K, alpha, A, lda, B, ldb, beta, C, ldc, nullptr, ws, ws_bytes, st, &taken,
                             batch, sA, sB, sC, nullptr, 0));
    if (taken) return GCGCN_OK;
    for (int b = 0; b < batch; ++b)
        GCGCN_TRY(launch_gemm(ta, tb, M, N, K, alpha, A + b * sA, lda, B + b * sB, ldb, beta, C + b * sC, ldc, nullptr,
                              ws, ws_bytes, st));
    return GCGCN_OK;
}

int launch_colsum(const float* X, int M, int N, int ldx, float* out, void* ws, size_t ws_bytes,
                  cudaStream_t st) {
    if (N <= 0) return GCGCN_OK;
    if (N == D && ldx % 4 == 0 && (reinterpret_cast<uintptr_t>(X) & 15) == 0 && M > 0) {
        const int rows_per_block = max(64, ceil_div(M, sm_count() * 4));
        const int parts = ceil_div(M, rows_per_block);
        if (ws == nullptr || ws_bytes < static_cast<size_t>(parts) * N * sizeof(float))
            return fail(GCGCN_ERR_WORKSPACE, "colsum: workspace too small");
        colsum128_partial_kernel<<<parts, 256, 0, st>>>(X, M, ldx, rows_per_block, static_cast<float*>(ws));
        GCGCN_CHECK_LAUNCH("colsum_partial");
        return launch_reduce_partials(static_cast<const float*>(ws), parts, N, out, N, nullptr, st);
    }
    int parts = max(1, min(ceil_div(M, 64), sm_count() * 16));
    const size_t need = static_cast<size_t>(parts) * N * sizeof(float);
    if (ws == nullptr || ws_bytes < need) return fail(GCGCN_ERR_WORKSPACE, "colsum: workspace too small");
    const int rows_per_block = max(1, ceil_div(M, parts));
    parts = max(1, ceil_div(M, rows_per_block));
    dim3 grid(ceil_div(N, 256), parts);
    colsum_partial_kernel<<<grid, 256, 0, st>>>(X, M, N, ldx, rows_per_block, static_cast<float*>(ws));
    GCGCN_CHECK_LAUNCH("colsum_partial");
    return launch_reduce_partials(static_cast<const float*>(ws), parts, N, out, N, nullptr, st);
}

}
```

### gcgcn_b200/csrc/gemm_tc.cu

```cuda
#include "common.cuh"
#include "tc_ptx.cuh"

namespace gcgcn {

constexpr int TC_BM = 128, TC_BN = 128, TC_BK = 32, TC_STAGES = 3;
constexpr int TC_PLANE_BYTES = 128 * 16 + 16;
constexpr int TC_PART_BYTES = (TC_BK / 4) * TC_PLANE_BYTES;
constexpr int TC_STAGE_BYTES = 4 * TC_PART_BYTES;
constexpr int TC_EPI_WARP_FLOATS = 32 * 32;
constexpr int TC_EPI_BYTES = 4 * TC_EPI_WARP_FLOATS * 4;
constexpr int tc_threads(int groups) { return (4 * groups + 5) * 32; }
constexpr int TC_TMEM_COLS = 256;
constexpr size_t TC_SMEM_BYTES = size_t(TC_STAGES) * TC_STAGE_BYTES + TC_EPI_BYTES + 1024  + 256 ;

struct TcArgs {
    int M, N, K, lda, ldb, ldc;
    const float* A;
    const float* B;
    const float* bias;
    float* C;
    float* partial;
    float alpha, beta;
    int tiles_m, tiles_n, k_splits, k_per_split;
    const uint8_t* Bpre;
    const uint8_t* Apre;
    int kblocks;
    int batch;
    long long sA, sB, sC;
    const float* rd_t;
    float* rd_out;
    long long rd_ld;
    const float* bscale;
    int lds;
    int seq_k;
};


__device__ __forceinline__ uint64_t make_desc(uint32_t smem_addr) {
    uint64_t d = (smem_addr >> 4) & 0x3FFFu;
    d |= static_cast<uint64_t>(TC_PLANE_BYTES >> 4) << 16;
    d |= static_cast<uint64_t>(128 >> 4) << 32;
    d |= static_cast<uint64_t>(1) << 46;
    return d;
}
constexpr uint32_t TC_IDESC = (1u << 4) | (2u << 7) | (2u << 10) | ((TC_BN >> 3) << 17) | ((TC_BM >> 4) << 24);

__device__ __forceinline__ void split_store(float* hi_base, float* lo_base, int chunk, int row, float4 a) {
    float4 h, l;
    h.x = __uint_as_float(__float_as_uint(a.x) & 0xffffe000u);
    h.y = __uint_as_float(__float_as_uint(a.y) & 0xffffe000u);
    h.z = __uint_as_float(__float_as_uint(a.z) & 0xffffe000u);
    h.w = __uint_as_float(__float_as_uint(a.w) & 0xffffe000u);
    l.x = a.x - h.x; l.y = a.y - h.y; l.z = a.z - h.z; l.w = a.w - h.w;
    const int off = chunk * (TC_PLANE_BYTES / 4) + row * 4;
    *reinterpret_cast<float4*>(hi_base + off) = h;
    *reinterpret_cast<float4*>(lo_base + off) = l;
}

template <bool KCONTIG>
__device__ __forceinline__ void tile_coord(int tid, int i, int& row, int& chunk) {
    if (KCONTIG) {
        const int w = tid >> 5, l = tid & 31;
        row = 32 * w + 4 * i + (l >> 3);
        chunk = l & 7;
    } else {
        row = tid;
        chunk = i;
    }
}

template <bool KCONTIG>
__device__ __forceinline__ void fetch_operand(const float* __restrict__ src, int ld, int row0, int rows_total,
                                              int k0, int kend, bool vec_ok, int tid, float4 (&v)[8]) {
#pragma unroll
    for (int i = 0; i < 8; ++i) {
        int r, c;
        tile_coord<KCONTIG>(tid, i, r, c);
        const int row = row0 + r, k = k0 + 4 * c;
        const bool row_ok = row < rows_total;
        if (KCONTIG) {
            const float* p = src + static_cast<size_t>(row) * ld + k;
            if (row_ok && vec_ok && k + 4 <= kend) {
                v[i] = *reinterpret_cast<const float4*>(p);
            } else {
                float t[4];
#pragma unroll
                for (int q = 0; q < 4; ++q) t[q] = (row_ok && k + q < kend) ? p[q] : 0.f;
                v[i] = make_float4(t[0], t[1], t[2], t[3]);
            }
        } else {
            float t[4];
#pragma unroll
            for (int q = 0; q < 4; ++q)
                t[q] = (row_ok && k + q < kend) ? src[static_cast<size_t>(k + q) * ld + row] : 0.f;
            v[i] = make_float4(t[0], t[1], t[2], t[3]);
        }
    }
}

template <bool KCONTIG>
__device__ __forceinline__ void store_operand(float* hi, float* lo, int tid, const float4 (&v)[8]) {
#pragma unroll
    for (int i = 0; i < 8; ++i) {
        int r, c;
        tile_coord<KCONTIG>(tid, i, r, c);
        split_store(hi, lo, c, r, v[i]);
    }
}

constexpr int TC_MN_BLOCK_BYTES = TC_BK * 128;
constexpr int TC_MN_PART_BYTES = 4 * TC_MN_BLOCK_BYTES;
static_assert(4 * TC_MN_PART_BYTES <= TC_STAGE_BYTES, "MN-major parts fit a stage");
__device__ __forceinline__ uint64_t make_desc_mn(uint32_t smem_addr) {
    uint64_t d = (smem_addr >> 4) & 0x3FFFu;
    d |= static_cast<uint64_t>(TC_MN_BLOCK_BYTES >> 4) << 16;
    d |= static_cast<uint64_t>(512 >> 4) << 32;
    d |= static_cast<uint64_t>(1) << 46;
    d |= static_cast<uint64_t>(1) << 61;
    return d;
}
constexpr uint32_t TC_IDESC_MN = TC_IDESC | (1u << 15) | (1u << 16);
__device__ __forceinline__ void fetch_operand_mn(const float* __restrict__ src, int ld, int mn0, int mn_total, int k0, int kend,
                                                 bool vec_ok, int tid, float4 (&v)[8]) {
    const int w = tid >> 5, l = tid & 31;
    const int mn = mn0 + 32 * w + 4 * (l & 7);
#pragma unroll
    for (int i = 0; i < 8; ++i) {
        const int k = k0 + 4 * i + (l >> 3);
        const float* p = src + static_cast<size_t>(k) * ld + mn;
        if (k < kend && vec_ok && mn + 4 <= mn_total) {
            v[i] = *reinterpret_cast<const float4*>(p);
        } else {
            float t[4];
#pragma unroll
            for (int q = 0; q < 4; ++q) t[q] = (k < kend && mn + q < mn_total) ? p[q] : 0.f;
            v[i] = make_float4(t[0], t[1], t[2], t[3]);
        }
    }
}
__device__ __forceinline__ void store_operand_mn(uint8_t* hi, uint8_t* lo, int tid, const float4 (&v)[8]) {
    const int w = tid >> 5, l = tid & 31, c = l & 7;
#pragma unroll
    for (int i = 0; i < 8; ++i) {
        const int krow = 4 * i + (l >> 3);
        const int off = w * TC_MN_BLOCK_BYTES + krow * 128 + (((((c >> 1) ^ (krow & 3)) << 1) | (c & 1)) << 4);
        const float4 a = v[i];
        float4 h, lw;
        h.x = __uint_as_float(__float_as_uint(a.x) & 0xffffe000u);
        h.y = __uint_as_float(__float_as_uint(a.y) & 0xffffe000u);
        h.z = __uint_as_float(__float_as_uint(a.z) & 0xffffe000u);
        h.w = __uint_as_float(__float_as_uint(a.w) & 0xffffe000u);
        lw.x = a.x - h.x; lw.y = a.y - h.y; lw.z = a.z - h.z; lw.w = a.w - h.w;
        *reinterpret_cast<float4*>(hi + off) = h;
        *reinterpret_cast<float4*>(lo + off) = lw;
    }
}

__device__ __forceinline__ void tc_epilogue_tile(const TcArgs& args, uint32_t tmem_base, int acc, uint32_t tempty_bar_addr,
                                                 int quarter, float* stg, int m0, int n0, int bi, int ks, bool has_k,
                                                 int lane, int chunk0 = 0, int chunks = TC_BN / 32, float beta_override = -1.f) {
    const float beta = beta_override >= 0.f ? beta_override : args.beta;
    const int row_base = m0 + quarter * 32;
    float* out_base;
    int ldo;
    if (args.partial != nullptr) {
        out_base = args.partial + (static_cast<size_t>(bi) * args.k_splits + ks) * args.M * args.N;
        ldo = args.N;
    } else {
        out_base = args.C + bi * args.sC;
        ldo = args.ldc;
    }
    const int rows_valid = min(32, args.M - row_base);
    const bool final_out = args.partial == nullptr;
    const bool vec = (ldo % 4 == 0) && ((reinterpret_cast<uintptr_t>(out_base) & 15) == 0) && (n0 + TC_BN <= args.N);
#pragma unroll 1
    for (int chunk = chunk0; chunk < chunk0 + chunks; ++chunk) {
        uint32_t v[32];
        const uint32_t taddr = tmem_base + (static_cast<uint32_t>(quarter * 32) << 16) +
                               static_cast<uint32_t>(acc * TC_BN + chunk * 32);
        tmem_ld32(taddr, v);
        if (chunk == chunk0 + chunks - 1) {
            tc_fence_before();
            __syncwarp();
            if (lane == 0) mbar_arrive(tempty_bar_addr);
        }
#pragma unroll
        for (int j = 0; j < 32; j += 4)
            *reinterpret_cast<float4*>(stg + lane * 32 + (((j >> 2) ^ (lane & 7)) << 2)) =
                has_k ? make_float4(__uint_as_float(v[j]), __uint_as_float(v[j + 1]), __uint_as_float(v[j + 2]),
                                    __uint_as_float(v[j + 3]))
                      : make_float4(0.f, 0.f, 0.f, 0.f);
        __syncwarp();
        if (vec) {
            const int c4 = (lane & 7) * 4, col = n0 + chunk * 32 + c4;
            float4 bias4 = make_float4(0.f, 0.f, 0.f, 0.f);
            if (final_out && args.bias != nullptr) bias4 = *reinterpret_cast<const float4*>(args.bias + col);
            float4 cold[8];
            const bool rmw = final_out && beta != 0.f;
            if (rmw) {
#pragma unroll
                for (int it = 0; it < 8; ++it) {
                    const int rr = 4 * it + (lane >> 3);
                    cold[it] = make_float4(0.f, 0.f, 0.f, 0.f);
                    if (rr < rows_valid)
                        cold[it] = *reinterpret_cast<const float4*>(out_base + static_cast<size_t>(row_base + rr) * ldo + col);
                }
            }
#pragma unroll
            for (int it = 0; it < 8; ++it) {
                const int rr = 4 * it + (lane >> 3);
                if (rr < rows_valid) {
                    float4 val = *reinterpret_cast<const float4*>(stg + rr * 32 + (((lane & 7) ^ (rr & 7)) << 2));
                    float4* p = reinterpret_cast<float4*>(out_base + static_cast<size_t>(row_base + rr) * ldo + col);
                    if (final_out) {
                        val.x = val.x * args.alpha + bias4.x; val.y = val.y * args.alpha + bias4.y;
                        val.z = val.z * args.alpha + bias4.z; val.w = val.w * args.alpha + bias4.w;
                        if (rmw) {
                            val.x += beta * cold[it].x; val.y += beta * cold[it].y;
                            val.z += beta * cold[it].z; val.w += beta * cold[it].w;
                        }
                    }
                    *p = val;
                }
            }
        } else {
            const int col = n0 + chunk * 32 + lane;
            if (col < args.N) {
                const float bias = (final_out && args.bias != nullptr) ? args.bias[col] : 0.f;
                for (int rr = 0; rr < rows_valid; ++rr) {
                    float val = stg[rr * 32 + ((((lane >> 2) ^ (rr & 7)) << 2) | (lane & 3))];
                    float* p = out_base + static_cast<size_t>(row_base + rr) * ldo + col;
                    if (final_out) {
                        val = val * args.alpha + bias;
                        if (beta != 0.f) val += beta * (*p);
                    }
                    *p = val;
                }
            }
        }
        __syncwarp();
    }
}

constexpr uint32_t TC_B_BLOB_BYTES = 2 * TC_PART_BYTES;

template <bool A_KCONTIG, bool B_KCONTIG, int GROUPS, bool BPRE, bool APRE = false, bool MNMAJ = false>
__global__ void __launch_bounds__(tc_threads(GROUPS), 1) gemm_tc_kernel(const TcArgs args) {
    constexpr int TC_PRODUCER_WARPS = 4 * GROUPS, TC_MMA_WARP = 4 * GROUPS, TC_GROUPS = GROUPS;
    static_assert(GROUPS <= TC_STAGES, "a producer group may run at most one stage-round ahead of the MMA warp");
    extern __shared__ __align__(1024) uint8_t smem[];
    float* epi_stage = reinterpret_cast<float*>(smem + size_t(TC_STAGES) * TC_STAGE_BYTES);
    uint64_t* bars = reinterpret_cast<uint64_t*>(smem + size_t(TC_STAGES) * TC_STAGE_BYTES + TC_EPI_BYTES);
    uint32_t* tmem_slot = reinterpret_cast<uint32_t*>(bars + 10);
    const uint32_t bar0 = smem_u32(bars);
    auto full_bar = [&](int s) { return bar0 + 8u * s; };
    auto empty_bar = [&](int s) { return bar0 + 8u * (TC_STAGES + s); };
    auto tfull_bar = [&](int a) { return bar0 + 8u * (2 * TC_STAGES + a); };
    auto tempty_bar = [&](int a) { return bar0 + 8u * (2 * TC_STAGES + 2 + a); };

    const int warp = threadIdx.x >> 5, lane = threadIdx.x & 31;

    if (threadIdx.x == 0) {
        for (int s = 0; s < TC_STAGES; ++s) {
            mbar_init(full_bar(s), (BPRE || APRE) ? 5 : 4);
            mbar_init(empty_bar(s), 1);
        }
        for (int a = 0; a < 2; ++a) {
            mbar_init(tfull_bar(a), 1);
            mbar_init(tempty_bar(a), 4);
        }
        fence_barrier_init();
    }
    if (warp == TC_MMA_WARP) tmem_alloc(smem_u32(tmem_slot), TC_TMEM_COLS);
    tc_fence_before();
    __syncthreads();
    tc_fence_after();
    const uint32_t tmem_base = *tmem_slot;

    const int tiles_mn = args.tiles_m * args.tiles_n;
    const int total_tiles = tiles_mn * args.k_splits * args.batch;

    if (warp < TC_PRODUCER_WARPS) {
        const bool a_vec = (args.lda % 4 == 0) && ((reinterpret_cast<uintptr_t>(args.A) & 15) == 0) && (args.sA % 4 == 0);
        const bool b_vec = (args.ldb % 4 == 0) && ((reinterpret_cast<uintptr_t>(args.B) & 15) == 0) && (args.sB % 4 == 0);
        const int group = warp >> 2, tid = threadIdx.x & 127;
        if (BPRE) {
            const int kblocks = args.kblocks;
            const int my_tiles = blockIdx.x < total_tiles ? (total_tiles - 1 - blockIdx.x) / static_cast<int>(gridDim.x) + 1 : 0;
            const int total_q = my_tiles * kblocks;
            auto fetch = [&](int q, float4 (&v)[8]) {
                const int tile = blockIdx.x + (q / kblocks) * gridDim.x, kb = q % kblocks;
                fetch_operand<A_KCONTIG>(args.A, args.lda, (tile / args.tiles_n) * TC_BM, args.M, kb * TC_BK, args.K, a_vec,
                                         tid, v);
            };
            auto commit = [&](int q, const float4 (&v)[8]) {
                const int stage = q % TC_STAGES;
                const uint32_t phase = (q / TC_STAGES) & 1;
                mbar_wait(empty_bar(stage), phase ^ 1);
                uint8_t* stb = smem + size_t(stage) * TC_STAGE_BYTES;
                if (tid == 0) {
                    const int tile = blockIdx.x + (q / kblocks) * gridDim.x, kb = q % kblocks;
                    const uint8_t* blob = args.Bpre + (static_cast<size_t>(tile % args.tiles_n) * kblocks + kb) * TC_B_BLOB_BYTES;
                    mbar_arrive_expect_tx(full_bar(stage), TC_B_BLOB_BYTES);
                    bulk_copy_g2s(smem_u32(stb + 2 * TC_PART_BYTES), blob, TC_B_BLOB_BYTES, full_bar(stage));
                }
                float* st = reinterpret_cast<float*>(stb);
                store_operand<A_KCONTIG>(st, st + TC_PART_BYTES / 4, tid, v);
                fence_proxy_async();
                __syncwarp();
                if (lane == 0) mbar_arrive(full_bar(stage));
            };
            float4 va0[8], va1[8];
            int q = group;
            if (q < total_q) fetch(q, va0);
            while (q < total_q) {
                if (q + GROUPS < total_q) fetch(q + GROUPS, va1);
                commit(q, va0);
                q += GROUPS;
                if (q >= total_q) break;
                if (q + GROUPS < total_q) fetch(q + GROUPS, va0);
                commit(q, va1);
                q += GROUPS;
            }
        }
        if (APRE) {
            int jbase = 0;
            for (int t = blockIdx.x; t < total_tiles; t += gridDim.x) {
                const int ks = t / tiles_mn, rem = t - ks * tiles_mn;
                const int mtile = rem / args.tiles_n, n0 = (rem % args.tiles_n) * TC_BN;
                const int kbeg = ks * args.k_per_split, kend = min(args.K, kbeg + args.k_per_split);
                const int total_q = kend > kbeg ? (kend - kbeg + TC_BK - 1) / TC_BK : 0;
                auto fetch = [&](int q, float4 (&v)[8]) {
                    if (args.bscale == nullptr) {
                        fetch_operand<B_KCONTIG>(args.B, args.ldb, n0, args.N, kbeg + q * TC_BK, kend, b_vec, tid, v);
                    } else {
                        const int kq = kbeg + q * TC_BK, nt = n0 / TC_BN;
                        fetch_operand<B_KCONTIG>(args.B, args.ldb, 0, TC_BN, kq, kend, b_vec, tid, v);
#pragma unroll
                        for (int i = 0; i < 8; ++i) {
                            int r, c;
                            tile_coord<B_KCONTIG>(tid, i, r, c);
                            const int k = kq + 4 * c;
                            const float* sp = args.bscale + static_cast<size_t>(k) * args.lds + nt;
                            v[i].x *= k < kend ? sp[0] : 0.f;
                            v[i].y *= k + 1 < kend ? sp[args.lds] : 0.f;
                            v[i].z *= k + 2 < kend ? sp[2 * static_cast<size_t>(args.lds)] : 0.f;
                            v[i].w *= k + 3 < kend ? sp[3 * static_cast<size_t>(args.lds)] : 0.f;
                        }
                    }
                };
                auto commit = [&](int q, const float4 (&v)[8]) {
                    const int j = jbase + q, stage = j % TC_STAGES;
                    const uint32_t phase = (j / TC_STAGES) & 1;
                    mbar_wait(empty_bar(stage), phase ^ 1);
                    uint8_t* stb = smem + size_t(stage) * TC_STAGE_BYTES;
                    if (tid == 0) {
                        const uint8_t* blob = args.Apre + (static_cast<size_t>(mtile) * args.kblocks + kbeg / TC_BK + q) * TC_B_BLOB_BYTES;
                        mbar_arrive_expect_tx(full_bar(stage), TC_B_BLOB_BYTES);
                        bulk_copy_g2s(smem_u32(stb), blob, TC_B_BLOB_BYTES, full_bar(stage));
                    }
                    float* st = reinterpret_cast<float*>(stb);
                    store_operand<B_KCONTIG>(st + 2 * (TC_PART_BYTES / 4), st + 3 * (TC_PART_BYTES / 4), tid, v);
                    fence_proxy_async();
                    __syncwarp();
                    if (lane == 0) mbar_arrive(full_bar(stage));
                };
                float4 vb0[8], vb1[8];
                int q = ((group - jbase) % GROUPS + GROUPS) % GROUPS;
                if (q < total_q) fetch(q, vb0);
                while (q < total_q) {
                    if (q + GROUPS < total_q) fetch(q + GROUPS, vb1);
                    commit(q, vb0);
                    q += GROUPS;
                    if (q >= total_q) break;
                    if (q + GROUPS < total_q) fetch(q + GROUPS, vb0);
                    commit(q, vb1);
                    q += GROUPS;
                }
                jbase += total_q;
            }
        }
        int j = 0;
        for (int t = blockIdx.x; !BPRE && !APRE && t < total_tiles; t += gridDim.x) {
            const int bi = t / (tiles_mn * args.k_splits), tb = t - bi * (tiles_mn * args.k_splits);
            const int ks = tb / tiles_mn, rem = tb - ks * tiles_mn;
            const int m0 = (rem / args.tiles_n) * TC_BM, n0 = (rem % args.tiles_n) * TC_BN;
            const int kbeg = ks * args.k_per_split;
            const int kend = min(args.K, kbeg + args.k_per_split);
            const float* Ab = args.A + bi * args.sA;
            const float* Bb = args.B + bi * args.sB;
            for (int k0 = kbeg; k0 < kend; k0 += TC_BK, ++j) {
                if ((j % TC_GROUPS) != group) continue;
                const int stage = j % TC_STAGES;
                const uint32_t phase = (j / TC_STAGES) & 1;
                float4 va[8], vb[8];
                if (MNMAJ) {
                    fetch_operand_mn(Ab, args.lda, m0, args.M, k0, kend, a_vec, tid, va);
                    fetch_operand_mn(Bb, args.ldb, n0, args.N, k0, kend, b_vec, tid, vb);
                } else {
                    fetch_operand<A_KCONTIG>(Ab, args.lda, m0, args.M, k0, kend, a_vec, tid, va);
                    fetch_operand<B_KCONTIG>(Bb, args.ldb, n0, args.N, k0, kend, b_vec, tid, vb);
                }
                mbar_wait(empty_bar(stage), phase ^ 1);
                float* st = reinterpret_cast<float*>(smem + size_t(stage) * TC_STAGE_BYTES);
                if (MNMAJ) {
                    uint8_t* sb = smem + size_t(stage) * TC_STAGE_BYTES;
                    store_operand_mn(sb, sb + TC_MN_PART_BYTES, tid, va);
                    store_operand_mn(sb + 2 * TC_MN_PART_BYTES, sb + 3 * TC_MN_PART_BYTES, tid, vb);
                } else {
                    store_operand<A_KCONTIG>(st, st + TC_PART_BYTES / 4, tid, va);
                    store_operand<B_KCONTIG>(st + 2 * (TC_PART_BYTES / 4), st + 3 * (TC_PART_BYTES / 4), tid, vb);
                }
                fence_proxy_async();
                __syncwarp();
                if (lane == 0) mbar_arrive(full_bar(stage));
            }
        }
    } else if (warp == TC_MMA_WARP) {
        if (lane == 0) {
            int stage = 0;
            uint32_t phase = 0;
            int acc = 0;
            uint32_t acc_phase = 0;
            for (int t = blockIdx.x; t < total_tiles; t += gridDim.x) {
                const int ks = (t % (tiles_mn * args.k_splits)) / tiles_mn;
                const int kbeg = ks * args.k_per_split;
                const int kend = min(args.K, kbeg + args.k_per_split);
                mbar_wait(tempty_bar(acc), acc_phase ^ 1);
                tc_fence_after();
                const uint32_t d_tmem = tmem_base + static_cast<uint32_t>(acc * TC_BN);
                uint32_t accumulate = 0;
                for (int k0 = kbeg; k0 < kend; k0 += TC_BK) {
                    mbar_wait(full_bar(stage), phase);
                    tc_fence_after();
                    const uint32_t sa = smem_u32(smem + size_t(stage) * TC_STAGE_BYTES);
                    if (MNMAJ) {
                        const uint32_t a_hi = sa, a_lo = sa + TC_MN_PART_BYTES;
                        const uint32_t b_hi = sa + 2 * TC_MN_PART_BYTES, b_lo = sa + 3 * TC_MN_PART_BYTES;
#pragma unroll
                        for (int kk = 0; kk < TC_BK / 8; ++kk) {
                            const uint32_t koff = kk * 8 * 128;
                            umma_tf32(d_tmem, make_desc_mn(a_lo + koff), make_desc_mn(b_hi + koff), TC_IDESC_MN, accumulate);
                            umma_tf32(d_tmem, make_desc_mn(a_hi + koff), make_desc_mn(b_lo + koff), TC_IDESC_MN, 1u);
                            umma_tf32(d_tmem, make_desc_mn(a_hi + koff), make_desc_mn(b_hi + koff), TC_IDESC_MN, 1u);
                            accumulate = 1u;
                        }
                    } else {
                        const uint32_t a_hi = sa, a_lo = sa + TC_PART_BYTES;
                        const uint32_t b_hi = sa + 2 * TC_PART_BYTES, b_lo = sa + 3 * TC_PART_BYTES;
#pragma unroll
                        for (int kk = 0; kk < TC_BK / 8; ++kk) {
                            const uint32_t koff = kk * 2 * TC_PLANE_BYTES;
                            umma_tf32(d_tmem, make_desc(a_lo + koff), make_desc(b_hi + koff), TC_IDESC, accumulate);
                            umma_tf32(d_tmem, make_desc(a_hi + koff), make_desc(b_lo + koff), TC_IDESC, 1u);
                            umma_tf32(d_tmem, make_desc(a_hi + koff), make_desc(b_hi + koff), TC_IDESC, 1u);
                            accumulate = 1u;
                        }
                    }
                    umma_commit(empty_bar(stage));
                    if (++stage == TC_STAGES) { stage = 0; phase ^= 1; }
                }
                umma_commit(tfull_bar(acc));
                if (++acc == 2) { acc = 0; acc_phase ^= 1; }
            }
        }
        __syncwarp();
    } else {
        const int quarter = warp & 3;
        float* stg = epi_stage + quarter * TC_EPI_WARP_FLOATS;
        int acc = 0;
        uint32_t acc_phase = 0;
        for (int t = blockIdx.x; t < total_tiles; t += gridDim.x) {
            const int bi = t / (tiles_mn * args.k_splits), tb = t - bi * (tiles_mn * args.k_splits);
            const int ks = tb / tiles_mn, rem = tb - ks * tiles_mn;
            const int m0 = (rem / args.tiles_n) * TC_BM, n0 = (rem % args.tiles_n) * TC_BN;
            const bool has_k = ks * args.k_per_split < args.K;
            mbar_wait(tfull_bar(acc), acc_phase);
            tc_fence_after();
            tc_epilogue_tile(args, tmem_base, acc, tempty_bar(acc), quarter, stg, m0, n0, bi, ks, has_k, lane, 0, TC_BN / 32,
                             (args.seq_k && ks > 0) ? 1.f : -1.f);
            if (++acc == 2) { acc = 0; acc_phase ^= 1; }
        }
    }

    tc_fence_before();
    __syncthreads();
    if (warp == TC_MMA_WARP) tmem_dealloc(tmem_base, TC_TMEM_COLS);
}

constexpr int TA_PRODUCER_WARPS = 8, TA_LOADER_WARP = 8, TA_MMA_WARP = 9, TA_KB = 4;
constexpr int TA_BSTAGES = 5, TA_EPI_WARPS = 8, TA_THREADS = (10 + TA_EPI_WARPS) * 32;
constexpr size_t TA_EPI_BYTES = size_t(TA_EPI_WARPS) * TC_EPI_WARP_FLOATS * 4;
constexpr size_t TA_SMEM_BYTES = size_t(TA_BSTAGES) * TC_B_BLOB_BYTES + TA_EPI_BYTES + 768 + 256;
constexpr uint32_t TA_COL_AHI = 256, TA_COL_ALO = 384;

template <int MODE>
__global__ void __launch_bounds__(TA_THREADS, 1) gemm_tc_tmema_kernel(const TcArgs args) {
    constexpr bool ROWDOT = MODE == 1, ROWACC = MODE == 2;
    extern __shared__ __align__(1024) uint8_t smem[];
    uint8_t* b_stage = smem;
    float* epi_stage = reinterpret_cast<float*>(b_stage + size_t(TA_BSTAGES) * TC_B_BLOB_BYTES);
    uint64_t* bars = reinterpret_cast<uint64_t*>(reinterpret_cast<uint8_t*>(epi_stage) + TA_EPI_BYTES);
    uint32_t* tmem_slot = reinterpret_cast<uint32_t*>(bars + 6 + 2 * TA_BSTAGES);
    const uint32_t bar0 = smem_u32(bars);
    const uint32_t a_full = bar0, a_empty = bar0 + 8;
    auto tfull_bar = [&](int a) { return bar0 + 8u * (2 + a); };
    auto tempty_bar = [&](int a) { return bar0 + 8u * (4 + a); };
    auto b_full = [&](int s) { return bar0 + 8u * (6 + s); };
    auto b_empty = [&](int s) { return bar0 + 8u * (6 + TA_BSTAGES + s); };
    const int warp = threadIdx.x >> 5, lane = threadIdx.x & 31;

    if (threadIdx.x == 0) {
        mbar_init(a_full, TA_PRODUCER_WARPS);
        mbar_init(a_empty, 1);
        for (int a = 0; a < 2; ++a) { mbar_init(tfull_bar(a), 1); mbar_init(tempty_bar(a), TA_EPI_WARPS); }
        for (int i = 0; i < TA_BSTAGES; ++i) { mbar_init(b_full(i), 1); mbar_init(b_empty(i), 1); }
        fence_barrier_init();
    }
    if (warp == TA_MMA_WARP) tmem_alloc(smem_u32(tmem_slot), 512);
    tc_fence_before();
    __syncthreads();
    tc_fence_after();
    const uint32_t tmem_base = *tmem_slot;
    const int kblocks = args.kblocks, tiles_n = args.tiles_n, tiles_m = args.tiles_m;

    if (warp < TA_PRODUCER_WARPS) {
        const int quarter = warp & 3, khalf = warp >> 2;
        const bool a_vec = (args.lda % 4 == 0) && ((reinterpret_cast<uintptr_t>(args.A) & 15) == 0);
        int it = 0;
        for (int mi = blockIdx.x; mi < tiles_m; mi += gridDim.x, ++it) {
            const int row = mi * TC_BM + quarter * 32 + lane;
            const float* src = args.A + static_cast<size_t>(row) * args.lda;
            float4 av[16];
            const int kbase = khalf * 64;
#pragma unroll
            for (int j = 0; j < 16; ++j) {
                const int k = kbase + 4 * j;
                if (k >= kblocks * TC_BK) {
                    av[j] = make_float4(0.f, 0.f, 0.f, 0.f);
                } else if (row < args.M && a_vec && k + 4 <= args.K) {
                    av[j] = *reinterpret_cast<const float4*>(src + k);
                } else {
                    float t[4];
#pragma unroll
                    for (int e = 0; e < 4; ++e) t[e] = (row < args.M && k + e < args.K) ? src[k + e] : 0.f;
                    av[j] = make_float4(t[0], t[1], t[2], t[3]);
                }
            }
            mbar_wait(a_empty, (it & 1) ^ 1);
            tc_fence_after();
#pragma unroll
            for (int c16 = 0; c16 < 4; ++c16) {
                const int k0 = kbase + c16 * 16;
                if (k0 >= kblocks * TC_BK) break;
                uint32_t hi[16], lo[16];
#pragma unroll
                for (int j = 0; j < 4; ++j) {
                    const float4 v = av[4 * c16 + j];
                    const float t[4] = {v.x, v.y, v.z, v.w};
#pragma unroll
                    for (int e = 0; e < 4; ++e) {
                        const uint32_t h = __float_as_uint(t[e]) & 0xffffe000u;
                        hi[4 * j + e] = h;
                        lo[4 * j + e] = __float_as_uint(t[e] - __uint_as_float(h));
                    }
                }
                const uint32_t lane_base = tmem_base + (static_cast<uint32_t>(quarter * 32) << 16);
                tmem_st16(lane_base + TA_COL_AHI + k0, hi);
                tmem_st16(lane_base + TA_COL_ALO + k0, lo);
            }
// ... 58 lines not shown
        float* stg = epi_stage + ew * TC_EPI_WARP_FLOATS;
        int acc = 0;
        uint32_t acc_phase = 0;
        if (ROWDOT) {
            static_assert(CH == 2, "row-dot epilogue assumes two 32-column chunks per epilogue warp");
            const int half = ew / 4;
            for (int mi = blockIdx.x; mi < tiles_m; mi += gridDim.x) {
                const int row = mi * TC_BM + quarter * 32 + lane;
                float4 t[16];
#pragma unroll
                for (int j = 0; j < 16; ++j)
                    t[j] = row < args.M ? *reinterpret_cast<const float4*>(args.rd_t + static_cast<size_t>(row) * 128 + half * 64 + 4 * j)
                                        : make_float4(0.f, 0.f, 0.f, 0.f);
                for (int n = 0; n < tiles_n; ++n) {
                    mbar_wait(tfull_bar(acc), acc_phase);
                    tc_fence_after();
                    float s = 0.f;
#pragma unroll
                    for (int c = 0; c < 2; ++c) {
                        uint32_t v[32];
                        const uint32_t taddr = tmem_base + (static_cast<uint32_t>(quarter * 32) << 16) +
                                               static_cast<uint32_t>(acc * TC_BN + (half * 2 + c) * 32);
                        tmem_ld32(taddr, v);
                        if (c == 1) {
                            tc_fence_before();
                            __syncwarp();
                            if (lane == 0) mbar_arrive(tempty_bar(acc));
                        }
#pragma unroll
                        for (int j = 0; j < 8; ++j) {
                            const float4 tv = t[c * 8 + j];
                            s += __uint_as_float(v[4 * j]) * tv.x + __uint_as_float(v[4 * j + 1]) * tv.y +
                                 __uint_as_float(v[4 * j + 2]) * tv.z + __uint_as_float(v[4 * j + 3]) * tv.w;
                        }
                    }
                    if (row < args.M) args.rd_out[(static_cast<long long>(n) * 2 + half) * args.rd_ld + row] = s;
                    if (++acc == 2) { acc = 0; acc_phase ^= 1; }
                }
            }
        } else if (ROWACC) {
            static_assert(CH == 2, "row-accumulate epilogue assumes two 32-column chunks per epilogue warp");
            const int half = ew / 4;
            for (int mi = blockIdx.x; mi < tiles_m; mi += gridDim.x) {
                const int row = mi * TC_BM + quarter * 32 + lane;
                const float* wrow = args.rd_t + static_cast<size_t>(row < args.M ? row : 0) * args.rd_ld;
                float4 sum[16];
#pragma unroll
                for (int j = 0; j < 16; ++j) sum[j] = make_float4(0.f, 0.f, 0.f, 0.f);
                for (int n = 0; n < tiles_n; ++n) {
                    const float wgt = row < args.M ? wrow[n] : 0.f;
                    mbar_wait(tfull_bar(acc), acc_phase);
                    tc_fence_after();
#pragma unroll
                    for (int c = 0; c < 2; ++c) {
                        uint32_t v[32];
                        const uint32_t taddr = tmem_base + (static_cast<uint32_t>(quarter * 32) << 16) +
                                               static_cast<uint32_t>(acc * TC_BN + (half * 2 + c) * 32);
                        tmem_ld32(taddr, v);
                        if (c == 1) {
                            tc_fence_before();
                            __syncwarp();
                            if (lane == 0) mbar_arrive(tempty_bar(acc));
                        }
#pragma unroll
                        for (int j = 0; j < 8; ++j) {
                            float4& a4 = sum[c * 8 + j];
                            a4.x += wgt * __uint_as_float(v[4 * j]);     a4.y += wgt * __uint_as_float(v[4 * j + 1]);
                            a4.z += wgt * __uint_as_float(v[4 * j + 2]); a4.w += wgt * __uint_as_float(v[4 * j + 3]);
                        }
                    }
                    if (++acc == 2) { acc = 0; acc_phase ^= 1; }
                }
                if (row < args.M) {
                    float* o = args.rd_out + static_cast<size_t>(row) * 128 + half * 64;
#pragma unroll
                    for (int j = 0; j < 16; ++j) *reinterpret_cast<float4*>(o + 4 * j) = sum[j];
                }
            }
        } else {
            for (int mi = blockIdx.x; mi < tiles_m; mi += gridDim.x)
                for (int n = 0; n < tiles_n; ++n) {
                    mbar_wait(tfull_bar(acc), acc_phase);
                    tc_fence_after();
                    tc_epilogue_tile(args, tmem_base, acc, tempty_bar(acc), quarter, stg, mi * TC_BM, n * TC_BN, 0, 0, true, lane,
                                     (ew / 4) * CH, CH);
                    if (++acc == 2) { acc = 0; acc_phase ^= 1; }
                }
        }
    }
    tc_fence_before();
    __syncthreads();
    if (warp == TA_MMA_WARP) tmem_dealloc(tmem_base, 512);
}

__global__ void __launch_bounds__(256)
tc_presplit_b_kernel(const float* __restrict__ B, int ldb, int b_kcontig, int N, int K, int kblocks,
                     uint8_t* __restrict__ blobs) {
    const int blob = blockIdx.x, nt = blob / kblocks, kb = blob - nt * kblocks;
    const int n0 = nt * TC_BN, k0 = kb * TC_BK;
    float* hi = reinterpret_cast<float*>(blobs + static_cast<size_t>(blob) * TC_B_BLOB_BYTES);
    float* lo = hi + TC_PART_BYTES / 4;
    for (int idx = blockIdx.y * 256 + threadIdx.x; idx < TC_BN * (TC_BK / 4); idx += 256 * gridDim.y) {
        int r, c;
        if (b_kcontig) { c = idx & 7; r = idx >> 3; } else { r = idx & (TC_BN - 1); c = idx >> 7; }
        const int n = n0 + r, k = k0 + 4 * c;
        float t[4];
#pragma unroll
        for (int q = 0; q < 4; ++q) {
            t[q] = 0.f;
            if (n < N && k + q < K)
                t[q] = b_kcontig ? B[static_cast<size_t>(n) * ldb + k + q] : B[static_cast<size_t>(k + q) * ldb + n];
        }
        split_store(hi, lo, c, r, make_float4(t[0], t[1], t[2], t[3]));
    }
}

size_t gemm_presplit_bytes(int rows) {
    return static_cast<size_t>(ceil_div(rows < 0 ? 0 : rows, TC_BK)) * TC_B_BLOB_BYTES;
}

int launch_splitk_reduce(const float* partial, int splits, int M, int N, float alpha, float beta, float* C,
                         int ldc, const float* bias, cudaStream_t st, int batch, long long sC);

int launch_gemm_tc(int ta, int tb, int M, int N, int K, float alpha, const float* A, int lda, const float* B,
                   int ldb, float beta, float* C, int ldc, const float* bias, void* ws, size_t ws_bytes,
                   cudaStream_t st, int* taken, int batch, long long sA, long long sB, long long sC, void* pre_ws,
                   size_t pre_bytes, const float* bscale, int lds) {
    *taken = 0;
    if (K < 1 || batch < 1) return GCGCN_OK;
    if (static_cast<double>(M) * N * K * batch < 2.0e6) return GCGCN_OK;
    TcArgs a;
    a.M = M; a.N = N; a.K = K; a.lda = lda; a.ldb = ldb; a.ldc = ldc;
    a.A = A; a.B = B; a.bias = bias; a.C = C; a.alpha = alpha; a.beta = beta;
    a.tiles_m = ceil_div(M, TC_BM);
    a.tiles_n = ceil_div(N, TC_BN);
    a.batch = batch; a.sA = sA; a.sB = sB; a.sC = sC;
    a.rd_t = nullptr; a.rd_out = nullptr; a.rd_ld = 0; a.bscale = bscale; a.lds = lds; a.seq_k = 0;
    const int tiles = a.tiles_m * a.tiles_n * batch;
    const int sms = sm_count();
    int splits = 1;
    if (tiles < sms && K >= 4096) {
        splits = std::min(std::max(sms / tiles, 1), ceil_div(K, 512));
        const size_t per = static_cast<size_t>(M) * N * sizeof(float) * batch;
        if (ws == nullptr) splits = 1;
        else splits = static_cast<int>(std::min<size_t>(splits, ws_bytes / per));
        if (splits < 2) splits = 1;
    }
    a.k_per_split = K;
    a.partial = nullptr;
    if (splits > 1) {
        a.k_per_split = ceil_div(ceil_div(K, splits), TC_BK) * TC_BK;
        splits = ceil_div(K, a.k_per_split);
        a.partial = static_cast<float*>(ws);
    }
    a.k_splits = splits;
    int grid = std::min(sms, tiles * splits);
    const bool seq = bscale != nullptr;
    if (seq) {
        a.k_per_split = 4096;
        a.k_splits = splits = ceil_div(K, a.k_per_split);
        const size_t per = static_cast<size_t>(M) * N * sizeof(float);
        if (splits > 1 && ws != nullptr && per * splits <= ws_bytes && (reinterpret_cast<uintptr_t>(ws) & 15) == 0) {
            a.partial = static_cast<float*>(ws);
            a.seq_k = 0;
            grid = std::min(sms, tiles * splits);
        } else {
            a.partial = nullptr;
            a.seq_k = splits > 1 ? 1 : 0;
            grid = std::min(sms, tiles);
        }
    }
    a.Bpre = nullptr;
    a.kblocks = ceil_div(K, TC_BK);
    const size_t blob_total = static_cast<size_t>(a.tiles_n) * a.kblocks * TC_B_BLOB_BYTES;
    const bool bpre = batch == 1 && splits == 1 && !seq && !ta && M >= 4096 &&
                      static_cast<size_t>(N) * K * sizeof(float) <= (size_t(8) << 20) && ws != nullptr &&
                      blob_total <= ws_bytes && (reinterpret_cast<uintptr_t>(ws) & 15) == 0;
    if (bpre) {
        tc_presplit_b_kernel<<<dim3(a.tiles_n * a.kblocks, 4), 256, 0, st>>>(B, ldb, tb != 0, N, K, a.kblocks, static_cast<uint8_t*>(ws));
        GCGCN_CHECK_LAUNCH("gemm_presplit_b");
        a.Bpre = static_cast<const uint8_t*>(ws);
    }
    a.Apre = nullptr;
    const size_t ablob_total = static_cast<size_t>(a.tiles_m) * a.kblocks * TC_B_BLOB_BYTES;
    const bool apre = bscale != nullptr && !bpre && batch == 1 && ta && !tb && K >= 8192 && M <= 2 * TC_BM &&
                      a.tiles_n >= 2 && (seq ? (a.partial != nullptr || tiles <= sms) : tiles * splits <= sms) &&
                      pre_ws != nullptr && ablob_total <= pre_bytes && (reinterpret_cast<uintptr_t>(pre_ws) & 15) == 0;
    if (bscale != nullptr && !apre)
        return fail(GCGCN_ERR_UNSUPPORTED, "gemm: the generated-operand product needs the pre-split weight-gradient path "
                    "(A transposed, K >= 8192, M <= 256, N >= 256, a pre-split workspace)");
    if (apre) {
        tc_presplit_b_kernel<<<dim3(a.tiles_m * a.kblocks, 4), 256, 0, st>>>(A, lda, 0, M, K, a.kblocks,
                                                                  static_cast<uint8_t*>(pre_ws));
        GCGCN_CHECK_LAUNCH("gemm_presplit_a");
        a.Apre = static_cast<const uint8_t*>(pre_ws);
    }
    const bool a_kc = !ta, b_kc = (tb != 0);
#define GCGCN_TC_LAUNCH(AK, BK, G, ...)                                                                                 \
    do {                                                                                                                \
        static std::atomic<unsigned long long> prepared{0};                                                             \
        GCGCN_TRY(set_smem_once(prepared, gemm_tc_kernel<AK, BK, G, __VA_ARGS__>, TC_SMEM_BYTES, "gemm_tc smem"));      \
        gemm_tc_kernel<AK, BK, G, __VA_ARGS__><<<grid, tc_threads(G), TC_SMEM_BYTES, st>>>(a);                          \
    } while (0)
    const bool tmema = bpre && a.kblocks <= TA_KB;
    if (tmema) {
        static std::atomic<unsigned long long> prepared{0};
        GCGCN_TRY(set_smem_once(prepared, gemm_tc_tmema_kernel<0>, TA_SMEM_BYTES, "gemm_tc_tmema smem"));
        gemm_tc_tmema_kernel<0><<<std::min(sms, a.tiles_m), TA_THREADS, TA_SMEM_BYTES, st>>>(a);
    } else if (apre) GCGCN_TC_LAUNCH(false, false, 2, false, true);
    else if (bpre) GCGCN_TC_LAUNCH(true, true, 3, true);
    else if (a_kc && b_kc) GCGCN_TC_LAUNCH(true, true, 3, false);
    else if (a_kc && !b_kc) GCGCN_TC_LAUNCH(true, false, 3, false);
    else if (!a_kc && b_kc) GCGCN_TC_LAUNCH(false, true, 3, false);
    else GCGCN_TC_LAUNCH(false, false, 3, false, false, true);
#undef GCGCN_TC_LAUNCH
    timing_set_work(2.0 * M * N * K * batch);
    GCGCN_CHECK_LAUNCH(tmema ? "gemm_tc_nn<A in TMEM>"
                             : apre ? "gemm_tc_tn<presplit A>"
                             : bpre ? (tb ? "gemm_tc_nt<presplit B>" : "gemm_tc_nn<presplit B>")
                             : ta ? (tb ? "gemm_tc_tt" : "gemm_tc_tn<MN-major>") : (tb ? "gemm_tc_nt" : "gemm_tc_nn"));
    if (splits > 1 && a.partial != nullptr)
        GCGCN_TRY(launch_splitk_reduce(a.partial, splits, M, N, alpha, beta, C, ldc, bias, st, batch, sC));
    *taken = 1;
    return GCGCN_OK;
}

int launch_gemm_rowop(int mode, int M, int N, int K, const float* A, int lda, const float* B, int ldb, const float* T,
                      float* out, long long ld, void* ws, size_t ws_bytes, cudaStream_t st) {
    if (M <= 0 || N <= 0) return GCGCN_OK;
    if (K < 1 || K > TA_KB * TC_BK || N % TC_BN != 0)
        return fail(GCGCN_ERR_UNSUPPORTED, "gemm_rowop: needs 1 <= K <= %d and N a multiple of %d (K %d, N %d)", TA_KB * TC_BK,
                    TC_BN, K, N);
    TcArgs a;
    a.M = M; a.N = N; a.K = K; a.lda = lda; a.ldb = ldb; a.ldc = 0;
    a.A = A; a.B = B; a.bias = nullptr; a.C = nullptr; a.partial = nullptr; a.alpha = 1.f; a.beta = 0.f;
    a.tiles_m = ceil_div(M, TC_BM); a.tiles_n = N / TC_BN; a.k_splits = 1; a.k_per_split = K;
    a.kblocks = ceil_div(K, TC_BK); a.batch = 1; a.sA = a.sB = a.sC = 0; a.Apre = nullptr;
    a.rd_t = T; a.rd_out = out; a.rd_ld = ld; a.bscale = nullptr; a.lds = 0; a.seq_k = 0;
    const size_t blob_total = static_cast<size_t>(a.tiles_n) * a.kblocks * TC_B_BLOB_BYTES;
    if (ws == nullptr || blob_total > ws_bytes || (reinterpret_cast<uintptr_t>(ws) & 15) != 0)
        return fail(GCGCN_ERR_WORKSPACE, "gemm_rowop: workspace of %zu bytes needed for the pre-split weights", blob_total);
    tc_presplit_b_kernel<<<dim3(a.tiles_n * a.kblocks, 4), 256, 0, st>>>(B, ldb, 0, N, K, a.kblocks, static_cast<uint8_t*>(ws));
    GCGCN_CHECK_LAUNCH("gemm_presplit_b");
    a.Bpre = static_cast<const uint8_t*>(ws);
    const int grid = std::min(sm_count(), a.tiles_m);
    if (mode == 1) {
        static std::atomic<unsigned long long> prepared{0};
        GCGCN_TRY(set_smem_once(prepared, gemm_tc_tmema_kernel<1>, TA_SMEM_BYTES, "gemm_tc_rowdot smem"));
        gemm_tc_tmema_kernel<1><<<grid, TA_THREADS, TA_SMEM_BYTES, st>>>(a);
    } else {
        static std::atomic<unsigned long long> prepared{0};
        GCGCN_TRY(set_smem_once(prepared, gemm_tc_tmema_kernel<2>, TA_SMEM_BYTES, "gemm_tc_rowacc smem"));
        gemm_tc_tmema_kernel<2><<<grid, TA_THREADS, TA_SMEM_BYTES, st>>>(a);
    }
    timing_set_work(2.0 * M * N * K);
    GCGCN_CHECK_LAUNCH(mode == 1 ? "gemm_tc_rowdot<A in TMEM>" : "gemm_tc_rowacc<A in TMEM>");
    return GCGCN_OK;
}

}
```

### gcgcn_b200/functional.py

```python
from __future__ import annotations

from typing import Optional

import torch
from torch.autograd import Function

from . import _lib
from .batch import PairTables, PoolTable, RaggedBatch

D = 128

_WS: dict = {}


def _stream(device) -> int:
    return torch.cuda.current_stream(device).cuda_stream


def workspace(device: torch.device, nbytes: int) -> torch.Tensor:
    key = (device.index, _stream(device))
    t = _WS.get(key)
    if t is None or t.numel() < nbytes:
        t = torch.empty(int(nbytes) + (1 << 20), dtype=torch.uint8, device=device)
        _WS[key] = t
    return t


def _ws_for(batch: RaggedBatch, heads: int, device):
    n = _lib.load().gcgcn_workspace_bytes(batch.total_nodes, batch.total_pairs, heads)
    t = workspace(device, n)
    return t.data_ptr(), t.numel()


def _p(t: Optional[torch.Tensor]):
    return None if t is None else t.data_ptr()


def _cuda(t: torch.Tensor, name: str, dtype=torch.float32) -> torch.Tensor:
    if not t.is_cuda:
        raise _lib.GcgcnError(f"{name} is a CPU tensor: gcgcn_b200 runs on CUDA only (no CPU fallback)")
    if dtype is not None and t.dtype != dtype:
        t = t.to(dtype)
    return t.contiguous()


def _edge(t: torch.Tensor, name: str):
    if not t.is_cuda:
        raise _lib.GcgcnError(f"{name} is a CPU tensor: gcgcn_b200 runs on CUDA only (no CPU fallback)")
    if t.dtype == torch.float32:
        return t.contiguous(), _lib.F32
    if t.dtype == torch.bfloat16:
        return t.contiguous(), _lib.BF16
    raise _lib.GcgcnError(f"{name}: edge features must be float32 or bfloat16, got {t.dtype}")


class PoolFn(Function):

    @staticmethod
    def forward(ctx, context: torch.Tensor, table: PoolTable):
        context = _cuda(context, "context_output")
        if context.shape != (table.total_tokens, D):
            raise _lib.GcgcnError(f"context must be [{table.total_tokens}, {D}], got {tuple(context.shape)}")
        x0 = torch.empty(table.total_nodes, D, device=context.device, dtype=torch.float32)
        _lib.call("gcgcn_pool_fwd", _p(context), _p(table.ent_ptr), _p(table.tok_idx), _p(table.w),
                  table.total_nodes, _p(x0), _stream(context.device))
        ctx.table = table
        return x0

    @staticmethod
    def backward(ctx, dx0):
        t = ctx.table
        dx0 = _cuda(dx0, "dx0")
        dctx = torch.empty(t.total_tokens, D, device=dx0.device, dtype=torch.float32)
        _lib.call("gcgcn_pool_bwd", _p(dx0), _p(t.tok_ptr), _p(t.ent_idx), _p(t.w_t), t.total_tokens,
                  _p(dctx), _stream(dx0.device))
        return dctx, None


class EdgeMeanFn(Function):

    @staticmethod
    def forward(ctx, e: torch.Tensor, batch: RaggedBatch):
        e, dt = _edge(e, "edge_feat")
        ebar = torch.empty(batch.total_nodes, D, device=e.device, dtype=torch.float32)
# ... 331 lines not shown
        ctx.rows, ctx.count = ps[0].shape[0], len(ps)
        ctx._keepalive = ps
        return out

    @staticmethod
    def backward(ctx, dout):
        return tuple(dout[i * ctx.rows:(i + 1) * ctx.rows] for i in range(ctx.count))


class PairGatherFn(Function):

    @staticmethod
    def forward(ctx, feat, dis, tables: PairTables, batch: RaggedBatch):
        feat = _cuda(feat, "node_feats")
        fw = feat.shape[1]
        dw = 0
        if dis is not None:
            dis = _cuda(dis, "dis_embed")
            dw = dis.shape[1]
            if not tables.has_dis:
                raise _lib.GcgcnError("PairTables were built without node_relative_pos")
            tables.check_dis_rows(dis.shape[0])
        dev = feat.device
        out_h = torch.empty(batch.total_pairs, fw + dw, device=dev)
        out_t = torch.empty(batch.total_pairs, fw + dw, device=dev)
        _lib.call("gcgcn_pair_gather_fwd", batch.ref, _p(feat), fw, _p(dis), dw, _p(tables.h_idx),
                  _p(tables.t_idx), _p(tables.dis_h) if dw else None, _p(tables.dis_t) if dw else None,
                  _p(out_h), _p(out_t), _stream(dev))
        ctx.cfg = (tables, batch, fw, dw, 0 if dis is None else dis.shape[0], feat.shape[0])
        return out_h, out_t

    @staticmethod
    def backward(ctx, dh, dt):
        tables, batch, fw, dw, rows, nrows = ctx.cfg
        dev = dh.device if dh is not None else dt.device
        shape = (batch.total_pairs, fw + dw)
        dh = torch.zeros(shape, device=dev) if dh is None else _cuda(dh, "dout_h")
        dt = torch.zeros(shape, device=dev) if dt is None else _cuda(dt, "dout_t")
        dfeat = torch.empty(nrows, fw, device=dev)
        ddis = torch.empty(rows, dw, device=dev) if dw else None
        ws, wsb = _ws_for(batch, 1, dev)
        _lib.call("gcgcn_pair_gather_bwd", batch.ref, _p(dh), _p(dt), fw, dw, rows,
                  _p(tables.dis_h) if dw else None, _p(tables.dis_t) if dw else None, _p(dfeat), _p(ddis),
                  ws, wsb, _stream(dev))
        return dfeat, ddis, None, None


class PairDenseFn(Function):

    @staticmethod
    def forward(ctx, U, Vd, tables: PairTables, batch: RaggedBatch):
        U, Vd = _cuda(U, "U"), _cuda(Vd, "Vd")
        if U.shape != (batch.total_nodes, D) or Vd.shape[1] != D:
            raise _lib.GcgcnError(f"pair_dense: U must be [{batch.total_nodes}, {D}] and Vd [rows, {D}]")
        if not tables.has_dis:
            raise _lib.GcgcnError("PairTables were built without node_relative_pos")
        tables.check_dis_rows(Vd.shape[0])
        dev = U.device
        out_h = torch.empty(batch.total_pairs, D, device=dev)
        out_t = torch.empty(batch.total_pairs, D, device=dev)
        _lib.call("gcgcn_pair_dense_fwd", batch.ref, _p(U), _p(Vd), _p(tables.h_idx), _p(tables.t_idx),
                  _p(tables.dis_h), _p(tables.dis_t), _p(out_h), _p(out_t), _stream(dev))
        ctx.save_for_backward(out_h, out_t)
        ctx.cfg = (tables, batch, Vd.shape[0])
        return out_h, out_t

    @staticmethod
    def backward(ctx, dh, dt):
        out_h, out_t = ctx.saved_tensors
        tables, batch, rows = ctx.cfg
        dev = out_h.device
        dh = torch.zeros_like(out_h) if dh is None else _cuda(dh, "dout_h")
        dt = torch.zeros_like(out_t) if dt is None else _cuda(dt, "dout_t")
        dU = torch.empty(batch.total_nodes, D, device=dev)
        dVd = torch.empty(rows, D, device=dev)
        dpre = torch.empty(2 * batch.total_pairs, D, device=dev)
        wsb = int(_lib.load().gcgcn_pair_dense_ws_bytes(rows))
        ws = workspace(dev, wsb)
        _lib.call("gcgcn_pair_dense_bwd", batch.ref, _p(dh), _p(dt), _p(out_h), _p(out_t), rows, _p(tables.dis_h),
                  _p(tables.dis_t), _p(dU), _p(dVd), _p(dpre), ws.data_ptr(), ws.numel(), _stream(dev))
        return dU, dVd, None, None


def gemm(a: torch.Tensor, b: torch.Tensor, trans_a=False, trans_b=False, bias=None,
         out: Optional[torch.Tensor] = None, alpha=1.0, beta=0.0) -> torch.Tensor:
    a, b = _cuda(a, "A"), _cuda(b, "B")
    M = a.shape[1] if trans_a else a.shape[0]
    K = a.shape[0] if trans_a else a.shape[1]
    N = b.shape[0] if trans_b else b.shape[1]
    if out is None:
        out = torch.empty(M, N, device=a.device) if (beta == 0.0 and K > 0) else torch.zeros(M, N, device=a.device)
    ws = workspace(a.device, (24 << 20) + 4096)
    _lib.call("gcgcn_gemm", int(trans_a), int(trans_b), M, N, K, float(alpha), _p(a), a.shape[1], _p(b),
              b.shape[1], float(beta), _p(out), out.shape[1], _p(bias), ws.data_ptr(), ws.numel(),
              _stream(a.device))
    return out


class LinearFn(Function):

    @staticmethod
    def forward(ctx, x, W, b):
        x, W = _cuda(x, "x"), _cuda(W, "weight")
        b = None if b is None else _cuda(b, "bias")
        ctx.save_for_backward(x, W)
        ctx.has_bias = b is not None
        if x.shape[0] == 0:
            return x.new_zeros(0, W.shape[0])
        return gemm(x, W, trans_b=True, bias=b)

    @staticmethod
    def backward(ctx, dy):
        x, W = ctx.saved_tensors
        dy = _cuda(dy, "dy")
        M = x.shape[0]
        dev = x.device
        if M == 0:
            return x.new_zeros(x.shape), torch.zeros_like(W), (torch.zeros(W.shape[0], device=dev) if ctx.has_bias else None)
        dx = gemm(dy, W) if ctx.needs_input_grad[0] else None
        dW = gemm(dy, x, trans_a=True) if ctx.needs_input_grad[1] else None
        db = None
        if ctx.has_bias and ctx.needs_input_grad[2]:
            db = torch.empty(W.shape[0], device=dev)
            ws = workspace(dev, 8 << 20)
            _lib.call("gcgcn_colsum", _p(dy), M, W.shape[0], dy.shape[1], _p(db), ws.data_ptr(), ws.numel(), _stream(dev))
        return dx, dW, db


def linear(x, layer):
    return LinearFn.apply(x, layer.weight, layer.bias)
```

### include/gcgcn_b200.h

```cpp
#ifndef GCGCN_B200_H
#define GCGCN_B200_H

#include <stddef.h>
#include <stdint.h>

#ifdef __cplusplus
extern "C" {
#endif

#define GCGCN_HIDDEN 128

#define GCGCN_OK 0
#define GCGCN_ERR_INVALID_ARG (-1)
#define GCGCN_ERR_UNSUPPORTED (-2)
#define GCGCN_ERR_CUDA (-3)
#define GCGCN_ERR_WORKSPACE (-4)

#define GCGCN_F32 0
#define GCGCN_BF16 1

#define GCGCN_STACK_RELU 1
#define GCGCN_STACK_RESIDUAL 2
#define GCGCN_STACK_LINEAR 4

// ... 181 lines not shown
size_t gcgcn_edgefeat_ws_bytes(int32_t num_tokens, int32_t att_total, int32_t num_slots, int32_t num_pairs,
                               int64_t total_pairs);
int gcgcn_word_table_fwd(const float* SF, const float* DF, const float* wa, const float* ba, int32_t tokens, float* T,
                         void* stream);
int gcgcn_word_table_bwd(const float* SF, const float* DF, const float* wa, const float* dT, int32_t tokens, float* dSF,
                         float* dparams, void* ws, size_t ws_bytes, void* stream);
int gcgcn_word_pool_fwd(const gcgcn_edge_tables* tabs, const float* T, const float* ctx, float* att, float* cwa,
                        void* stream);
int gcgcn_word_pool_bwd(const gcgcn_edge_tables* tabs, const float* ctx, const float* att, const float* dcwa,
                        float* dctx, float* dT, void* ws, size_t ws_bytes, void* stream);
int gcgcn_sent_pool_fwd(const gcgcn_edge_tables* tabs, const float* cw, const float* sfeat, const float* nfeat,
                        const float* va, const float* ca, float* score, float* csa, void* stream);
int gcgcn_sent_pool_bwd(const gcgcn_edge_tables* tabs, int32_t total_nodes, const float* cw, const float* sfeat,
                        const float* nfeat, const float* va, const float* score, const float* dcsa, float* dcw,
                        float* dsfeat, float* dnfeat, float* dparams, void* ws, size_t ws_bytes, void* stream);
int gcgcn_edge_fill_fwd(const float* bias, const float* rows, const int64_t* pair_idx, int32_t num_pairs,
                        int64_t total_pairs, int32_t edge_dtype, void* e, void* stream);
int gcgcn_edge_fill_bwd(const void* de, const int64_t* pair_idx, int32_t num_pairs, int64_t total_pairs,
                        int32_t edge_dtype, float* drows, float* dbias, void* ws, size_t ws_bytes, void* stream);
int gcgcn_colsum(const float* X, int32_t M, int32_t N, int32_t ldx, float* out, void* ws, size_t ws_bytes, void* stream);

size_t gcgcn_bilinear_ws_bytes(int32_t rows, int32_t relations);
int gcgcn_bilinear_fwd(const float* h, const float* t, const float* Wm, const float* bias, int32_t rows,
                       int32_t relations, int32_t accumulate, float* out, int32_t ldo, void* ws, size_t ws_bytes,
                       void* stream);
size_t gcgcn_bilinear_bwd_ws_bytes(int32_t rows, int32_t relations);
int gcgcn_bilinear_bwd(const float* h, const float* t, const float* Wm, const float* Wm2, const float* dout, int32_t rows,
                       int32_t relations, float beta, float* dh, float* dt, float* dWm, void* ws, size_t ws_bytes,
                       void* stream);
int gcgcn_bilinear_reduce_fwd(const float* Y, const float* t, const float* bias, int32_t rows, int32_t relations,
                              int32_t accumulate, float* out, int32_t ldo, void* stream);
int gcgcn_bilinear_outer_bwd(const float* dout, int32_t ldd, const float* t, int32_t rows, int32_t relations, float* dY,
                             void* stream);
int gcgcn_bilinear_dt_bwd(const float* dout, int32_t ldd, const float* Y, int32_t rows, int32_t relations, float* dt,
                          void* stream);
int gcgcn_doc_bias_fwd(const gcgcn_batch* bt, const float* v, int32_t relations, float* z, void* stream);
int gcgcn_doc_bias_bwd(const gcgcn_batch* bt, const float* dz, int32_t relations, float* dv, void* stream);
int gcgcn_pair_bce_fwd(const gcgcn_batch* bt, const float* logits, const float* labels, int32_t relations, float* loss,
                       void* stream);
int gcgcn_pair_bce_bwd(const gcgcn_batch* bt, const float* logits, const float* labels, int32_t relations,
                       const float* dloss, float* dlogits, void* stream);

#define GCGCN_RANK_TILE 4096
#define GCGCN_RANK_MAX_CANDIDATES (1LL << 30)

typedef struct gcgcn_rank_result {
    int64_t count;
    int64_t total_recall;
    int64_t best_pos;
    int64_t w;
    double auc;
    double ign_auc;
    float f1;
    float theta;
    float f1_at_w;
    float precision_at_w;
    float recall_at_w;
    float ign_f1;
    float ign_f1_at_w;
    float reserved;
} gcgcn_rank_result;

size_t gcgcn_rank_ws_bytes(int64_t count);
int gcgcn_rank_candidates(const gcgcn_batch* bt, const float* logits, int32_t relations, const float* labels,
                          const uint8_t* intrain, int64_t base_id, float* score, uint32_t* payload, int64_t* counters,
                          void* stream);
int gcgcn_rank_sort(const float* score, const uint32_t* payload, int64_t count, uint32_t* sorted_key,
                    uint32_t* sorted_payload, void* ws, size_t ws_bytes, void* stream);
int gcgcn_rank_curve(const uint32_t* sorted_key, const uint32_t* sorted_payload, int64_t count, int64_t total_recall,
                     int32_t has_intrain, double input_theta, gcgcn_rank_result* result, void* ws, size_t ws_bytes,
                     void* stream);
int gcgcn_rank_decode(const uint32_t* sorted_key, const uint32_t* sorted_payload, int64_t rows, int64_t count,
                      const int64_t* doc_offsets, const int32_t* doc_n, int32_t num_docs, int32_t relations, int32_t* doc,
                      int32_t* row, int32_t* col, int32_t* relation, float* score, void* stream);

int gcgcn_adam_step(float* params, const float* grads, float* exp_avg, float* exp_avg_sq, int64_t count,
                    float lr, float beta1, float beta2, float eps, float weight_decay, float grad_scale,
                    int32_t step, void* stream);

int gcgcn_gemm(int32_t trans_a, int32_t trans_b, int32_t M, int32_t N, int32_t K, float alpha,
               const float* A, int32_t lda, const float* B, int32_t ldb, float beta, float* C,
               int32_t ldc, const float* bias, void* ws, size_t ws_bytes, void* stream);

#ifdef __cplusplus
}
#endif
#endif
```

Before: 898,000.

## Group all backward weight-gradient GEMMs into one split-K tensor-core launch

Measured after the change: 901,800, median of 6. No clear change (+0.4%).

```diff
diff --git a/gcgcn_b200/_lib.py b/gcgcn_b200/_lib.py
--- a/gcgcn_b200/_lib.py
+++ b/gcgcn_b200/_lib.py
@@ -59,6 +59,14 @@
         ("auc", ctypes.c_double), ("ign_auc", ctypes.c_double),
         ("f1", c_float), ("theta", c_float), ("f1_at_w", c_float), ("precision_at_w", c_float),
         ("recall_at_w", c_float), ("ign_f1", c_float), ("ign_f1_at_w", c_float), ("reserved", c_float),
+    ]
+
+
+class WgradProblem(ctypes.Structure):
+    _fields_ = [
+        ("A", c_void_p), ("B", c_void_p), ("C", c_void_p),
+        ("lda", c_int32), ("ldb", c_int32), ("ldc", c_int32), ("M", c_int32), ("N", c_int32), ("heads", c_int32),
+        ("sA", c_int64), ("sB", c_int64), ("sC", c_int64), ("alpha", c_float), ("beta", c_float),
     ]
 
 
@@ -182,6 +190,7 @@
     "gcgcn_adam_step": (c_int32, [_P, _P, _P, _P, c_int64] + [c_float] * 6 + [c_int32, _P]),
     "gcgcn_gemm": (c_int32, [c_int32, c_int32, c_int32, c_int32, c_int32, c_float, _P, c_int32, _P,
                              c_int32, c_float, _P, c_int32, _P, _P, c_size_t, _P]),
+    "gcgcn_wgrad_group": (c_int32, [_P, c_int32, c_int32, _P, c_size_t, _P]),
 }
 
 _lib = None
diff --git a/gcgcn_b200/csrc/api.cu b/gcgcn_b200/csrc/api.cu
--- a/gcgcn_b200/csrc/api.cu
+++ b/gcgcn_b200/csrc/api.cu
@@ -47,9 +47,6 @@
                 cudaStream_t st);
 size_t gemm_presplit_bytes(int rows);
 int launch_colsum(const float* X, int M, int N, int ldx, float* out, void* ws, size_t ws_bytes, cudaStream_t st);
-int launch_gemm_batched(int ta, int tb, int M, int N, int K, float alpha, const float* A, int lda, const float* B,
-                        int ldb, float beta, float* C, int ldc, int batch, long long sA, long long sB, long long sC,
-                        void* ws, size_t ws_bytes, cudaStream_t st);
 int launch_csr_gather(const float* src, const int* ptr, const int* idx, const float* w, int rows, float* out,
                       cudaStream_t st);
 int launch_pair_gather_fwd(const gcgcn_batch* bt, const float* feat, int feat_w, const float* dis, int dis_w,
@@ -579,7 +576,7 @@
                           const float* keep, const float* Z, const float* G, const float* F, const float* dy,
                           float* dx, float* debar, float* att_out, float* dWnX, float* dWe, float* dWinner,
                           float* dWout, float* dbout, void* ws, size_t ws_bytes, cudaStream_t st,
-                          const BlockDrop& drop = BlockDrop{}) {
+                          const BlockDrop& drop = BlockDrop{}, const WgradProblem* extra = nullptr) {
     const bool linear = flags & GCGCN_STACK_LINEAR;
     const int HD = heads * slab, M = bt->total_nodes, gd = slab / layers;
     Arena ar(ws, ws_bytes);
@@ -593,8 +590,6 @@
     const float* dF = dy;
     if (linear) {
         GCGCN_TRY(launch_gemm(0, 0, M, HD, D, 1.f, dy, D, Wout, HD, 0.f, dFbuf, HD, nullptr, gws, GEMM_WS_BYTES, st));
-        if (dWout != nullptr)
-            GCGCN_TRY(launch_gemm(1, 0, D, HD, M, 1.f, dy, D, F, HD, 0.f, dWout, HD, nullptr, gws, GEMM_WS_BYTES, st));
         if (dbout != nullptr) GCGCN_TRY(launch_colsum(dy, M, D, D, dbout, gws, GEMM_WS_BYTES, st));
         dF = dFbuf;
     }
@@ -616,19 +611,20 @@
     }
     GCGCN_TRY(launch_gemm(0, 1, M, in_dim, HD, 1.f, dZ, HD, WnX, HD, beta, dx, in_dim, nullptr, gws, GEMM_WS_BYTES, st));
     GCGCN_TRY(launch_gemm(0, 1, M, D, HD, 1.f, dE, HD, We, HD, 0.f, debar, D, nullptr, gws, GEMM_WS_BYTES, st));
-    if (dWnX != nullptr)
-        GCGCN_TRY(launch_gemm(1, 0, in_dim, HD, M, 1.f, x, in_dim, dZ, HD, 0.f, dWnX, HD, nullptr, gws, GEMM_WS_BYTES, st));
-    if (dWe != nullptr)
-        GCGCN_TRY(launch_gemm(1, 0, D, HD, M, 1.f, ebar, D, dE, HD, 0.f, dWe, HD, nullptr, gws, GEMM_WS_BYTES, st));
+    WgradProblem wg[4 + 4];
+    int nwg = 0;
+    wg[nwg++] = WgradProblem{dy, F, linear ? dWout : nullptr, D, HD, HD, D, HD, 1, 0, 0, 0, 1.f, 0.f};
+    wg[nwg++] = WgradProblem{x, dZ, dWnX, in_dim, HD, HD, in_dim, HD, 1, 0, 0, 0, 1.f, 0.f};
+    wg[nwg++] = WgradProblem{ebar, dE, dWe, D, HD, HD, D, HD, 1, 0, 0, 0, 1.f, 0.f};
+    if (extra != nullptr) wg[nwg++] = *extra;
     if (dWinner != nullptr && layers > 1) {
         GCGCN_TRY(cuda_ok(cudaMemsetAsync(dWinner, 0, static_cast<size_t>(heads) * layers * slab * gd * sizeof(float), st),
                           "memset dWinner"));
         for (int l = 1; l < layers; ++l)
-            GCGCN_TRY(launch_gemm_batched(1, 0, l * gd, gd, M, 1.f, G, HD, dZ + l * gd, HD, 0.f,
-                                          dWinner + static_cast<size_t>(l) * slab * gd, gd, heads, slab, slab,
-                                          static_cast<long long>(layers) * slab * gd, gws, GEMM_WS_BYTES, st));
-    }
-    return GCGCN_OK;
+            wg[nwg++] = WgradProblem{G, dZ + l * gd, dWinner + static_cast<size_t>(l) * slab * gd, HD, HD, gd, l * gd, gd,
+                                     heads, slab, slab, static_cast<long long>(layers) * slab * gd, 1.f, 0.f};
+    }
+    return launch_wgrad_group(wg, nwg, M, gws, GEMM_WS_BYTES, st);
 }
 
 int gcgcn_graphconv_stack_bwd(const gcgcn_batch* bt, int32_t heads, int32_t layers, int32_t in_dim,
@@ -734,15 +730,14 @@
     if (dq == nullptr) return fail(GCGCN_ERR_WORKSPACE, "mha_stack_bwd: workspace too small");
     void* rest = static_cast<char*>(ws) + ar.off;
     const size_t rest_bytes = ws_bytes - ar.off;
+    const WgradProblem wq{dq, x, dWq, D, D, D, D, D, 1, 0, 0, 0, 1.f, 0.f};
     GCGCN_TRY(stack_bwd_impl(bt, heads, layers, D, D, BLOCK_FLAGS_ALL, ATT_GRAD_DQ, x, ebar, P, q, WnX, We, Winner, Wout,
                              nullptr, Z, G, F, dy, dx, debar, dq, dWnX, dWe, dWinner, dWout, dbout, rest, rest_bytes, st,
-                             drop));
+                             drop, &wq));
     Arena ar2(rest, rest_bytes);
     float* gws = ar2.take<float>(GEMM_WS_BYTES / sizeof(float));
     if (gws == nullptr) return fail(GCGCN_ERR_WORKSPACE, "mha_stack_bwd: workspace too small");
     GCGCN_TRY(launch_gemm(0, 0, bt->total_nodes, D, D, 1.f, dq, D, Wq, D, 1.f, dx, D, nullptr, gws, GEMM_WS_BYTES, st));
-    if (dWq != nullptr)
-        GCGCN_TRY(launch_gemm(1, 0, D, D, bt->total_nodes, 1.f, dq, D, x, D, 0.f, dWq, D, nullptr, gws, GEMM_WS_BYTES, st));
     if (dbq != nullptr) GCGCN_TRY(launch_colsum(dq, bt->total_nodes, D, D, dbq, gws, GEMM_WS_BYTES, st));
     return GCGCN_OK;
 }
@@ -1308,6 +1303,23 @@
     const size_t head = ws_bytes < GEMM_WS_BYTES ? ws_bytes : GEMM_WS_BYTES;
     return launch_gemm(ta, tb, M, N, K, alpha, A, lda, B, ldb, beta, C, ldc, bias, ws, head,
                        static_cast<cudaStream_t>(stream));
+}
+
+int gcgcn_wgrad_group(const gcgcn_wgrad_problem* list, int32_t count, int32_t K, void* ws, size_t ws_bytes, void* stream) {
+    GCGCN_API_ENTER(stream);
+    GCGCN_REQUIRE(count >= 0 && K >= 0 && (count == 0 || list != nullptr), "wgrad_group: bad count / K");
+    for (int i = 0; i < count; ++i) {
+        const gcgcn_wgrad_problem& q = list[i];
+        if (q.C == nullptr) continue;
+        GCGCN_REQUIRE(q.M >= 0 && q.N >= 0 && q.heads >= 0 && q.sA >= 0 && q.sB >= 0 && q.sC >= 0 && q.ldc >= q.N &&
+                      q.lda >= 1 && q.ldb >= 1, "wgrad_group: bad shape in problem %d", i);
+        GCGCN_TRY(check_device_ptr(q.C, "C"));
+        if (K > 0) {
+            GCGCN_TRY(check_device_ptr(q.A, "A"));
+            GCGCN_TRY(check_device_ptr(q.B, "B"));
+        }
+    }
+    return launch_wgrad_group(list, count, K, ws, ws_bytes, static_cast<cudaStream_t>(stream));
 }
 
 namespace {
diff --git a/gcgcn_b200/csrc/common.cuh b/gcgcn_b200/csrc/common.cuh
--- a/gcgcn_b200/csrc/common.cuh
+++ b/gcgcn_b200/csrc/common.cuh
@@ -122,6 +122,9 @@
 
 static inline int ceil_div(long long a, long long b) { return static_cast<int>((a + b - 1) / b); }
 
+using WgradProblem = gcgcn_wgrad_problem;
+int launch_wgrad_group(const WgradProblem* list, int count, int K, void* ws, size_t ws_bytes, cudaStream_t st);
+
 template <class LaunchFn>
 inline int for_each_size_class(const gcgcn_batch* bt, LaunchFn fn) {
     if (bt->doc_order == nullptr) return fn(bt->num_docs, 0, bt->max_nodes, static_cast<const int*>(nullptr));
diff --git a/gcgcn_b200/csrc/gemm.cu b/gcgcn_b200/csrc/gemm.cu
--- a/gcgcn_b200/csrc/gemm.cu
+++ b/gcgcn_b200/csrc/gemm.cu
@@ -131,12 +131,10 @@
 
 __global__ void __launch_bounds__(256)
 splitk_reduce_kernel(const float* __restrict__ partial, int splits, int M, int N, float alpha, float beta,
-                     float* __restrict__ C, int ldc, const float* __restrict__ bias, long long batch_stride_c) {
+                     float* __restrict__ C, int ldc, const float* __restrict__ bias) {
     const size_t idx = static_cast<size_t>(blockIdx.x) * blockDim.x + threadIdx.x;
     const size_t total = static_cast<size_t>(M) * N;
     if (idx >= total) return;
-    partial += static_cast<size_t>(blockIdx.y) * splits * total;
-    C += static_cast<size_t>(blockIdx.y) * batch_stride_c;
     float s0 = 0.f, s1 = 0.f, s2 = 0.f, s3 = 0.f;
     int p = 0;
     for (; p + 4 <= splits; p += 4) {
@@ -157,12 +155,11 @@
 
 __global__ void __launch_bounds__(256)
 splitk_reduce4_kernel(const float* __restrict__ partial, int splits, int M, int N, float alpha, float beta,
-                      float* __restrict__ C, int ldc, const float* __restrict__ bias, long long batch_stride_c) {
+                      float* __restrict__ C, int ldc, const float* __restrict__ bias) {
     const size_t idx = static_cast<size_t>(blockIdx.x) * blockDim.x + threadIdx.x;
     const size_t total4 = static_cast<size_t>(M) * N / 4;
     if (idx >= total4) return;
-    const float4* part = reinterpret_cast<const float4*>(partial) + static_cast<size_t>(blockIdx.y) * splits * total4;
-    C += static_cast<size_t>(blockIdx.y) * batch_stride_c;
+    const float4* part = reinterpret_cast<const float4*>(partial);
     float4 a = make_float4(0.f, 0.f, 0.f, 0.f), b = a;
     int p = 0;
     for (; p + 2 <= splits; p += 2) {
@@ -190,13 +187,12 @@
 
 __global__ void __launch_bounds__(256)
 splitk_reduce4_wide_kernel(const float* __restrict__ partial, int splits, int M, int N, float alpha, float beta,
-                           float* __restrict__ C, int ldc, const float* __restrict__ bias, long long batch_stride_c) {
+                           float* __restrict__ C, int ldc, const float* __restrict__ bias) {
     __shared__ float4 sm[8][32];
     const int cx = threadIdx.x & 31, sy = threadIdx.x >> 5;
     const size_t idx = static_cast<size_t>(blockIdx.x) * 32 + cx;
     const size_t total4 = static_cast<size_t>(M) * N / 4;
-    const float4* part = reinterpret_cast<const float4*>(partial) + static_cast<size_t>(blockIdx.y) * splits * total4;
-    C += static_cast<size_t>(blockIdx.y) * batch_stride_c;
+    const float4* part = reinterpret_cast<const float4*>(partial);
     float4 a = make_float4(0.f, 0.f, 0.f, 0.f);
     if (idx < total4) {
 #pragma unroll 4
@@ -264,20 +260,17 @@
                            float* out1, cudaStream_t st);
 
 int launch_splitk_reduce(const float* partial, int splits, int M, int N, float alpha, float beta, float* C,
-                         int ldc, const float* bias, cudaStream_t st, int batch = 1, long long sC = 0) {
+                         int ldc, const float* bias, cudaStream_t st) {
     const size_t total = static_cast<size_t>(M) * N;
-    const bool vec = N % 4 == 0 && ldc % 4 == 0 && sC % 4 == 0 && (reinterpret_cast<uintptr_t>(C) & 15) == 0 &&
+    const bool vec = N % 4 == 0 && ldc % 4 == 0 && (reinterpret_cast<uintptr_t>(C) & 15) == 0 &&
                      (reinterpret_cast<uintptr_t>(partial) & 15) == 0 &&
                      (bias == nullptr || (reinterpret_cast<uintptr_t>(bias) & 15) == 0);
     if (vec && splits >= 16 && total / 4 <= 64 * 1024) {
-        dim3 grid(ceil_div(total / 4, 32), batch);
-        splitk_reduce4_wide_kernel<<<grid, 256, 0, st>>>(partial, splits, M, N, alpha, beta, C, ldc, bias, sC);
+        splitk_reduce4_wide_kernel<<<ceil_div(total / 4, 32), 256, 0, st>>>(partial, splits, M, N, alpha, beta, C, ldc, bias);
     } else if (vec) {
-        dim3 grid(ceil_div(total / 4, 256), batch);
-        splitk_reduce4_kernel<<<grid, 256, 0, st>>>(partial, splits, M, N, alpha, beta, C, ldc, bias, sC);
+        splitk_reduce4_kernel<<<ceil_div(total / 4, 256), 256, 0, st>>>(partial, splits, M, N, alpha, beta, C, ldc, bias);
     } else {
-        dim3 grid(ceil_div(total, 256), batch);
-        splitk_reduce_kernel<<<grid, 256, 0, st>>>(partial, splits, M, N, alpha, beta, C, ldc, bias, sC);
+        splitk_reduce_kernel<<<ceil_div(total, 256), 256, 0, st>>>(partial, splits, M, N, alpha, beta, C, ldc, bias);
     }
     GCGCN_CHECK_LAUNCH("splitk_reduce");
     return GCGCN_OK;
@@ -285,7 +278,7 @@
 
 int launch_gemm_tc(int ta, int tb, int M, int N, int K, float alpha, const float* A, int lda, const float* B,
                    int ldb, float beta, float* C, int ldc, const float* bias, void* ws, size_t ws_bytes,
-                   cudaStream_t st, int* taken, int batch, long long sA, long long sB, long long sC, void* pre_ws,
+                   cudaStream_t st, int* taken, void* pre_ws,
                    size_t pre_bytes, const float* bscale = nullptr, int lds = 0);
 
 int launch_gemm(int ta, int tb, int M, int N, int K, float alpha, const float* A, int lda,
@@ -295,7 +288,7 @@
     if (K < 0) return fail(GCGCN_ERR_INVALID_ARG, "gemm: K < 0");
     int taken = 0;
     GCGCN_TRY(launch_gemm_tc(ta, tb, M, N, K, alpha, A, lda, B, ldb, beta, C, ldc, bias, ws, ws_bytes, st, &taken,
-                             1, 0, 0, 0, nullptr, 0));
+                             nullptr, 0));
     if (taken) return GCGCN_OK;
     const int tiles = ceil_div(M, GM) * ceil_div(N, GN);
     int splits = 1;
@@ -334,23 +327,9 @@
                              float beta, float* C, int ldc, void* ws, size_t ws_bytes, cudaStream_t st, void* pre_ws,
                              size_t pre_bytes) {
     int taken = 0;
-    GCGCN_TRY(launch_gemm_tc(1, 0, M, tiles * 128, K, 1.f, A, lda, T, 128, beta, C, ldc, nullptr, ws, ws_bytes, st, &taken, 1, 0,
-                             0, 0, pre_ws, pre_bytes, scale, lds));
+    GCGCN_TRY(launch_gemm_tc(1, 0, M, tiles * 128, K, 1.f, A, lda, T, 128, beta, C, ldc, nullptr, ws, ws_bytes, st, &taken,
+                             pre_ws, pre_bytes, scale, lds));
     if (!taken) return fail(GCGCN_ERR_UNSUPPORTED, "gemm_wgrad_scaled: shape not covered by the tensor-core path");
-    return GCGCN_OK;
-}
-
-int launch_gemm_batched(int ta, int tb, int M, int N, int K, float alpha, const float* A, int lda, const float* B,
-                        int ldb, float beta, float* C, int ldc, int batch, long long sA, long long sB, long long sC,
-                        void* ws, size_t ws_bytes, cudaStream_t st) {
-    if (M <= 0 || N <= 0 || batch <= 0) return GCGCN_OK;
-    int taken = 0;
-    GCGCN_TRY(launch_gemm_tc(ta, tb, M, N, K, alpha, A, lda, B, ldb, beta, C, ldc, nullptr, ws, ws_bytes, st, &taken,
-                             batch, sA, sB, sC, nullptr, 0));
-    if (taken) return GCGCN_OK;
-    for (int b = 0; b < batch; ++b)
-        GCGCN_TRY(launch_gemm(ta, tb, M, N, K, alpha, A + b * sA, lda, B + b * sB, ldb, beta, C + b * sC, ldc, nullptr,
-                              ws, ws_bytes, st));
     return GCGCN_OK;
 }
 
diff --git a/gcgcn_b200/csrc/gemm_tc.cu b/gcgcn_b200/csrc/gemm_tc.cu
--- a/gcgcn_b200/csrc/gemm_tc.cu
+++ b/gcgcn_b200/csrc/gemm_tc.cu
@@ -25,8 +25,6 @@
     const uint8_t* Bpre;
     const uint8_t* Apre;
     int kblocks;
-    int batch;
-    long long sA, sB, sC;
     const float* rd_t;
     float* rd_out;
     long long rd_ld;
@@ -120,23 +118,27 @@
     return d;
 }
 constexpr uint32_t TC_IDESC_MN = TC_IDESC | (1u << 15) | (1u << 16);
-__device__ __forceinline__ void fetch_operand_mn(const float* __restrict__ src, int ld, int mn0, int mn_total, int k0, int kend,
-                                                 bool vec_ok, int tid, float4 (&v)[8]) {
-    const int w = tid >> 5, l = tid & 31;
-    const int mn = mn0 + 32 * w + 4 * (l & 7);
+__device__ __forceinline__ void fetch_block_mn(const float* __restrict__ src, int ld, int valid, int k0, int kend,
+                                               bool vec_ok, int l, float4 (&v)[8]) {
+    const int mn = 4 * (l & 7);
 #pragma unroll
     for (int i = 0; i < 8; ++i) {
         const int k = k0 + 4 * i + (l >> 3);
         const float* p = src + static_cast<size_t>(k) * ld + mn;
-        if (k < kend && vec_ok && mn + 4 <= mn_total) {
+        if (k < kend && vec_ok && mn + 4 <= valid) {
             v[i] = *reinterpret_cast<const float4*>(p);
         } else {
             float t[4];
 #pragma unroll
-            for (int q = 0; q < 4; ++q) t[q] = (k < kend && mn + q < mn_total) ? p[q] : 0.f;
+            for (int q = 0; q < 4; ++q) t[q] = (k < kend && mn + q < valid) ? p[q] : 0.f;
             v[i] = make_float4(t[0], t[1], t[2], t[3]);
         }
     }
+}
+__device__ __forceinline__ void fetch_operand_mn(const float* __restrict__ src, int ld, int mn0, int mn_total, int k0, int kend,
+                                                 bool vec_ok, int tid, float4 (&v)[8]) {
+    const int c0 = mn0 + 32 * (tid >> 5);
+    fetch_block_mn(src + c0, ld, mn_total - c0, k0, kend, vec_ok, tid & 31, v);
 }
 __device__ __forceinline__ void store_operand_mn(uint8_t* hi, uint8_t* lo, int tid, const float4 (&v)[8]) {
     const int w = tid >> 5, l = tid & 31, c = l & 7;
@@ -157,17 +159,17 @@
 }
 
 __device__ __forceinline__ void tc_epilogue_tile(const TcArgs& args, uint32_t tmem_base, int acc, uint32_t tempty_bar_addr,
-                                                 int quarter, float* stg, int m0, int n0, int bi, int ks, bool has_k,
+                                                 int quarter, float* stg, int m0, int n0, int ks, bool has_k,
                                                  int lane, int chunk0 = 0, int chunks = TC_BN / 32, float beta_override = -1.f) {
     const float beta = beta_override >= 0.f ? beta_override : args.beta;
     const int row_base = m0 + quarter * 32;
     float* out_base;
     int ldo;
     if (args.partial != nullptr) {
-        out_base = args.partial + (static_cast<size_t>(bi) * args.k_splits + ks) * args.M * args.N;
+        out_base = args.partial + static_cast<size_t>(ks) * args.M * args.N;
         ldo = args.N;
     } else {
-        out_base = args.C + bi * args.sC;
+        out_base = args.C;
         ldo = args.ldc;
     }
     const int rows_valid = min(32, args.M - row_base);
@@ -278,11 +280,11 @@
     const uint32_t tmem_base = *tmem_slot;
 
     const int tiles_mn = args.tiles_m * args.tiles_n;
-    const int total_tiles = tiles_mn * args.k_splits * args.batch;
+    const int total_tiles = tiles_mn * args.k_splits;
 
     if (warp < TC_PRODUCER_WARPS) {
-        const bool a_vec = (args.lda % 4 == 0) && ((reinterpret_cast<uintptr_t>(args.A) & 15) == 0) && (args.sA % 4 == 0);
-        const bool b_vec = (args.ldb % 4 == 0) && ((reinterpret_cast<uintptr_t>(args.B) & 15) == 0) && (args.sB % 4 == 0);
+        const bool a_vec = (args.lda % 4 == 0) && ((reinterpret_cast<uintptr_t>(args.A) & 15) == 0);
+        const bool b_vec = (args.ldb % 4 == 0) && ((reinterpret_cast<uintptr_t>(args.B) & 15) == 0);
         const int group = warp >> 2, tid = threadIdx.x & 127;
         if (BPRE) {
             const int kblocks = args.kblocks;
@@ -382,13 +384,12 @@
         }
         int j = 0;
         for (int t = blockIdx.x; !BPRE && !APRE && t < total_tiles; t += gridDim.x) {
-            const int bi = t / (tiles_mn * args.k_splits), tb = t - bi * (tiles_mn * args.k_splits);
-            const int ks = tb / tiles_mn, rem = tb - ks * tiles_mn;
+            const int ks = t / tiles_mn, rem = t - ks * tiles_mn;
             const int m0 = (rem / args.tiles_n) * TC_BM, n0 = (rem % args.tiles_n) * TC_BN;
             const int kbeg = ks * args.k_per_split;
             const int kend = min(args.K, kbeg + args.k_per_split);
-            const float* Ab = args.A + bi * args.sA;
-            const float* Bb = args.B + bi * args.sB;
+            const float* Ab = args.A;
+            const float* Bb = args.B;
             for (int k0 = kbeg; k0 < kend; k0 += TC_BK, ++j) {
                 if ((j % TC_GROUPS) != group) continue;
                 const int stage = j % TC_STAGES;
@@ -471,13 +472,12 @@
         int acc = 0;
         uint32_t acc_phase = 0;
         for (int t = blockIdx.x; t < total_tiles; t += gridDim.x) {
-            const int bi = t / (tiles_mn * args.k_splits), tb = t - bi * (tiles_mn * args.k_splits);
-            const int ks = tb / tiles_mn, rem = tb - ks * tiles_mn;
+            const int ks = t / tiles_mn, rem = t - ks * tiles_mn;
             const int m0 = (rem / args.tiles_n) * TC_BM, n0 = (rem % args.tiles_n) * TC_BN;
             const bool has_k = ks * args.k_per_split < args.K;
             mbar_wait(tfull_bar(acc), acc_phase);
             tc_fence_after();
-            tc_epilogue_tile(args, tmem_base, acc, tempty_bar(acc), quarter, stg, m0, n0, bi, ks, has_k, lane, 0, TC_BN / 32,
+            tc_epilogue_tile(args, tmem_base, acc, tempty_bar(acc), quarter, stg, m0, n0, ks, has_k, lane, 0, TC_BN / 32,
                              (args.seq_k && ks > 0) ? 1.f : -1.f);
             if (++acc == 2) { acc = 0; acc_phase ^= 1; }
         }
@@ -486,6 +486,187 @@
     tc_fence_before();
     __syncthreads();
     if (warp == TC_MMA_WARP) tmem_dealloc(tmem_base, TC_TMEM_COLS);
+}
+
+constexpr int WG_MAX = 8, WG_CHUNK = 6144;
+constexpr size_t WG_PART_FLOATS = size_t(TC_BM) * TC_BN;
+struct WgDesc {
+    const float* A;
+    const float* B;
+    float* C;
+    int lda, ldb, ldc, M, N;
+    long long sA, sB, sC;
+    float alpha, beta;
+    int tile0, tiles_m, tiles_n, pack, vec;
+};
+struct WgArgs {
+    WgDesc p[WG_MAX];
+    int count, K, tiles, splits, k_per_split;
+    float* partial;
+};
+
+__device__ __forceinline__ const WgDesc& wg_tile(const WgArgs& g, int t, int& head, int& m0, int& n0) {
+    int p = 0;
+    while (p + 1 < g.count && t >= g.p[p + 1].tile0) ++p;
+    const WgDesc& d = g.p[p];
+    const int local = t - d.tile0;
+    if (d.pack) {
+        head = 2 * local; m0 = n0 = 0;
+    } else {
+        const int per = d.tiles_m * d.tiles_n;
+        head = local / per;
+        const int rem = local - head * per;
+        m0 = (rem / d.tiles_n) * TC_BM; n0 = (rem % d.tiles_n) * TC_BN;
+    }
+    return d;
+}
+
+__device__ __forceinline__ const float* wg_block(const float* base, long long stride, int mn, int head, int mn0, int pack, int w,
+                                                 int& valid) {
+    if (pack) {
+        valid = mn - 32 * (w & 1);
+        return base + (head + (w >> 1)) * stride + 32 * (w & 1);
+    }
+    valid = mn - mn0 - 32 * w;
+    return base + head * stride + mn0 + 32 * w;
+}
+
+__global__ void __launch_bounds__(tc_threads(3), 1) wgrad_group_kernel(const WgArgs g) {
+    constexpr int GROUPS = 3, MMA_WARP = 4 * GROUPS;
+    extern __shared__ __align__(1024) uint8_t smem[];
+    float* epi_stage = reinterpret_cast<float*>(smem + size_t(TC_STAGES) * TC_STAGE_BYTES);
+    uint64_t* bars = reinterpret_cast<uint64_t*>(smem + size_t(TC_STAGES) * TC_STAGE_BYTES + TC_EPI_BYTES);
+    uint32_t* tmem_slot = reinterpret_cast<uint32_t*>(bars + 10);
+    const uint32_t bar0 = smem_u32(bars);
+    auto full_bar = [&](int s) { return bar0 + 8u * s; };
+    auto empty_bar = [&](int s) { return bar0 + 8u * (TC_STAGES + s); };
+    auto tfull_bar = [&](int a) { return bar0 + 8u * (2 * TC_STAGES + a); };
+    auto tempty_bar = [&](int a) { return bar0 + 8u * (2 * TC_STAGES + 2 + a); };
+    const int warp = threadIdx.x >> 5, lane = threadIdx.x & 31;
+
+    if (threadIdx.x == 0) {
+        for (int s = 0; s < TC_STAGES; ++s) { mbar_init(full_bar(s), 4); mbar_init(empty_bar(s), 1); }
+        for (int a = 0; a < 2; ++a) { mbar_init(tfull_bar(a), 1); mbar_init(tempty_bar(a), 4); }
+        fence_barrier_init();
+    }
+    if (warp == MMA_WARP) tmem_alloc(smem_u32(tmem_slot), TC_TMEM_COLS);
+    tc_fence_before();
+    __syncthreads();
+    tc_fence_after();
+    const uint32_t tmem_base = *tmem_slot;
+    const int items = g.tiles * g.splits;
+
+    if (warp < 4 * GROUPS) {
+        const int group = warp >> 2, w = warp & 3, tid = threadIdx.x & 127;
+        int j = 0;
+        for (int i = blockIdx.x; i < items; i += gridDim.x) {
+            const int ks = i / g.tiles;
+            int head, m0, n0;
+            const WgDesc& d = wg_tile(g, i - ks * g.tiles, head, m0, n0);
+            int va_n, vb_n;
+            const float* a_src = wg_block(d.A, d.sA, d.M, head, m0, d.pack, w, va_n);
+            const float* b_src = wg_block(d.B, d.sB, d.N, head, n0, d.pack, w, vb_n);
+            const int kbeg = ks * g.k_per_split, kend = min(g.K, kbeg + g.k_per_split);
+            for (int k0 = kbeg; k0 < kend; k0 += TC_BK, ++j) {
+                if ((j % GROUPS) != group) continue;
+                const int stage = j % TC_STAGES;
+                const uint32_t phase = (j / TC_STAGES) & 1;
+                float4 va[8], vb[8];
+                fetch_block_mn(a_src, d.lda, va_n, k0, kend, d.vec, lane, va);
+                fetch_block_mn(b_src, d.ldb, vb_n, k0, kend, d.vec, lane, vb);
+                mbar_wait(empty_bar(stage), phase ^ 1);
+                uint8_t* sb = smem + size_t(stage) * TC_STAGE_BYTES;
+                store_operand_mn(sb, sb + TC_MN_PART_BYTES, tid, va);
+                store_operand_mn(sb + 2 * TC_MN_PART_BYTES, sb + 3 * TC_MN_PART_BYTES, tid, vb);
+                fence_proxy_async();
+                __syncwarp();
+                if (lane == 0) mbar_arrive(full_bar(stage));
+            }
+        }
+    } else if (warp == MMA_WARP) {
+        if (lane == 0) {
+            int stage = 0, acc = 0;
+            uint32_t phase = 0, acc_phase = 0;
+            for (int i = blockIdx.x; i < items; i += gridDim.x) {
+                const int kbeg = (i / g.tiles) * g.k_per_split, kend = min(g.K, kbeg + g.k_per_split);
+                for (int c0 = kbeg; c0 < kend; c0 += WG_CHUNK) {
+                    mbar_wait(tempty_bar(acc), acc_phase ^ 1);
+                    tc_fence_after();
+                    const uint32_t d_tmem = tmem_base + static_cast<uint32_t>(acc * TC_BN);
+                    uint32_t accumulate = 0;
+                    for (int k0 = c0; k0 < min(kend, c0 + WG_CHUNK); k0 += TC_BK) {
+                        mbar_wait(full_bar(stage), phase);
+                        tc_fence_after();
+                        const uint32_t a_hi = smem_u32(smem + size_t(stage) * TC_STAGE_BYTES), a_lo = a_hi + TC_MN_PART_BYTES;
+                        const uint32_t b_hi = a_hi + 2 * TC_MN_PART_BYTES, b_lo = a_hi + 3 * TC_MN_PART_BYTES;
+#pragma unroll
+                        for (int kk = 0; kk < TC_BK / 8; ++kk) {
+                            const uint32_t koff = kk * 8 * 128;
+                            umma_tf32(d_tmem, make_desc_mn(a_lo + koff), make_desc_mn(b_hi + koff), TC_IDESC_MN, accumulate);
+                            umma_tf32(d_tmem, make_desc_mn(a_hi + koff), make_desc_mn(b_lo + koff), TC_IDESC_MN, 1u);
+                            umma_tf32(d_tmem, make_desc_mn(a_hi + koff), make_desc_mn(b_hi + koff), TC_IDESC_MN, 1u);
+                            accumulate = 1u;
+                        }
+                        umma_commit(empty_bar(stage));
+                        if (++stage == TC_STAGES) { stage = 0; phase ^= 1; }
+                    }
+                    umma_commit(tfull_bar(acc));
+                    if (++acc == 2) { acc = 0; acc_phase ^= 1; }
+                }
+            }
+        }
+        __syncwarp();
+    } else {
+        const int quarter = warp & 3;
+        float* stg = epi_stage + quarter * TC_EPI_WARP_FLOATS;
+        TcArgs ep{};
+        ep.M = TC_BM; ep.N = TC_BN; ep.ldc = TC_BN;
+        ep.alpha = 1.f; ep.beta = 0.f;
+        int acc = 0;
+        uint32_t acc_phase = 0;
+        for (int i = blockIdx.x; i < items; i += gridDim.x) {
+            const int kbeg = (i / g.tiles) * g.k_per_split, kend = min(g.K, kbeg + g.k_per_split);
+            for (int c0 = kbeg; c0 < kend; c0 += WG_CHUNK) {
+                mbar_wait(tfull_bar(acc), acc_phase);
+                tc_fence_after();
+                ep.C = g.partial + static_cast<size_t>(i) * WG_PART_FLOATS;
+                tc_epilogue_tile(ep, tmem_base, acc, tempty_bar(acc), quarter, stg, 0, 0, 0, true, lane, 0, TC_BN / 32,
+                                 c0 > kbeg ? 1.f : -1.f);
+                if (++acc == 2) { acc = 0; acc_phase ^= 1; }
+            }
+        }
+    }
+
+    tc_fence_before();
+    __syncthreads();
+    if (warp == MMA_WARP) tmem_dealloc(tmem_base, TC_TMEM_COLS);
+}
+
+__global__ void __launch_bounds__(256) wgrad_reduce_kernel(const WgArgs g) {
+    const int t = blockIdx.x, idx = blockIdx.y * 256 + threadIdx.x;
+    const int r = idx / (TC_BN / 4), c = (idx % (TC_BN / 4)) * 4;
+    float4 s = make_float4(0.f, 0.f, 0.f, 0.f);
+    for (int ks = 0; ks < g.splits; ++ks) {
+        const float4 v = *reinterpret_cast<const float4*>(g.partial + (static_cast<size_t>(ks) * g.tiles + t) * WG_PART_FLOATS +
+                                                          r * TC_BN + c);
+        s.x += v.x; s.y += v.y; s.z += v.z; s.w += v.w;
+    }
+    int head, m0, n0;
+    const WgDesc& d = wg_tile(g, t, head, m0, n0);
+    const float sv[4] = {s.x, s.y, s.z, s.w};
+#pragma unroll
+    for (int q = 0; q < 4; ++q) {
+        int h = head, row = m0 + r, col = n0 + c + q;
+        if (d.pack) {
+            if ((r >> 6) != (col >> 6)) continue;
+            h += r >> 6; row = r & 63; col &= 63;
+        }
+        if (row >= d.M || col >= d.N) continue;
+        float* p = d.C + h * d.sC + static_cast<size_t>(row) * d.ldc + col;
+        float v = d.alpha * sv[q];
+        if (d.beta != 0.f) v += d.beta * *p;
+        *p = v;
+    }
 }
 
 constexpr int TA_PRODUCER_WARPS = 8, TA_LOADER_WARP = 8, TA_MMA_WARP = 9, TA_KB = 4;
@@ -710,7 +891,7 @@
                 for (int n = 0; n < tiles_n; ++n) {
                     mbar_wait(tfull_bar(acc), acc_phase);
                     tc_fence_after();
-                    tc_epilogue_tile(args, tmem_base, acc, tempty_bar(acc), quarter, stg, mi * TC_BM, n * TC_BN, 0, 0, true, lane,
+                    tc_epilogue_tile(args, tmem_base, acc, tempty_bar(acc), quarter, stg, mi * TC_BM, n * TC_BN, 0, true, lane,
                                      (ew / 4) * CH, CH);
                     if (++acc == 2) { acc = 0; acc_phase ^= 1; }
                 }
@@ -748,28 +929,27 @@
 }
 
 int launch_splitk_reduce(const float* partial, int splits, int M, int N, float alpha, float beta, float* C,
-                         int ldc, const float* bias, cudaStream_t st, int batch, long long sC);
+                         int ldc, const float* bias, cudaStream_t st);
 
 int launch_gemm_tc(int ta, int tb, int M, int N, int K, float alpha, const float* A, int lda, const float* B,
                    int ldb, float beta, float* C, int ldc, const float* bias, void* ws, size_t ws_bytes,
-                   cudaStream_t st, int* taken, int batch, long long sA, long long sB, long long sC, void* pre_ws,
+                   cudaStream_t st, int* taken, void* pre_ws,
                    size_t pre_bytes, const float* bscale, int lds) {
     *taken = 0;
-    if (K < 1 || batch < 1) return GCGCN_OK;
-    if (static_cast<double>(M) * N * K * batch < 2.0e6) return GCGCN_OK;
+    if (K < 1) return GCGCN_OK;
+    if (static_cast<double>(M) * N * K < 2.0e6) return GCGCN_OK;
     TcArgs a;
     a.M = M; a.N = N; a.K = K; a.lda = lda; a.ldb = ldb; a.ldc = ldc;
     a.A = A; a.B = B; a.bias = bias; a.C = C; a.alpha = alpha; a.beta = beta;
     a.tiles_m = ceil_div(M, TC_BM);
     a.tiles_n = ceil_div(N, TC_BN);
-    a.batch = batch; a.sA = sA; a.sB = sB; a.sC = sC;
     a.rd_t = nullptr; a.rd_out = nullptr; a.rd_ld = 0; a.bscale = bscale; a.lds = lds; a.seq_k = 0;
-    const int tiles = a.tiles_m * a.tiles_n * batch;
+    const int tiles = a.tiles_m * a.tiles_n;
     const int sms = sm_count();
     int splits = 1;
     if (tiles < sms && K >= 4096) {
         splits = std::min(std::max(sms / tiles, 1), ceil_div(K, 512));
-        const size_t per = static_cast<size_t>(M) * N * sizeof(float) * batch;
+        const size_t per = static_cast<size_t>(M) * N * sizeof(float);
         if (ws == nullptr) splits = 1;
         else splits = static_cast<int>(std::min<size_t>(splits, ws_bytes / per));
         if (splits < 2) splits = 1;
@@ -801,7 +981,7 @@
     a.Bpre = nullptr;
     a.kblocks = ceil_div(K, TC_BK);
     const size_t blob_total = static_cast<size_t>(a.tiles_n) * a.kblocks * TC_B_BLOB_BYTES;
-    const bool bpre = batch == 1 && splits == 1 && !seq && !ta && M >= 4096 &&
+    const bool bpre = splits == 1 && !seq && !ta && M >= 4096 &&
                       static_cast<size_t>(N) * K * sizeof(float) <= (size_t(8) << 20) && ws != nullptr &&
                       blob_total <= ws_bytes && (reinterpret_cast<uintptr_t>(ws) & 15) == 0;
     if (bpre) {
@@ -811,7 +991,7 @@
     }
     a.Apre = nullptr;
     const size_t ablob_total = static_cast<size_t>(a.tiles_m) * a.kblocks * TC_B_BLOB_BYTES;
-    const bool apre = bscale != nullptr && !bpre && batch == 1 && ta && !tb && K >= 8192 && M <= 2 * TC_BM &&
+    const bool apre = bscale != nullptr && !bpre && ta && !tb && K >= 8192 && M <= 2 * TC_BM &&
                       a.tiles_n >= 2 && (seq ? (a.partial != nullptr || tiles <= sms) : tiles * splits <= sms) &&
                       pre_ws != nullptr && ablob_total <= pre_bytes && (reinterpret_cast<uintptr_t>(pre_ws) & 15) == 0;
     if (bscale != nullptr && !apre)
@@ -842,13 +1022,13 @@
     else if (!a_kc && b_kc) GCGCN_TC_LAUNCH(false, true, 3, false);
     else GCGCN_TC_LAUNCH(false, false, 3, false, false, true);
 #undef GCGCN_TC_LAUNCH
-    timing_set_work(2.0 * M * N * K * batch);
+    timing_set_work(2.0 * M * N * K);
     GCGCN_CHECK_LAUNCH(tmema ? "gemm_tc_nn<A in TMEM>"
                              : apre ? "gemm_tc_tn<presplit A>"
                              : bpre ? (tb ? "gemm_tc_nt<presplit B>" : "gemm_tc_nn<presplit B>")
                              : ta ? (tb ? "gemm_tc_tt" : "gemm_tc_tn<MN-major>") : (tb ? "gemm_tc_nt" : "gemm_tc_nn"));
     if (splits > 1 && a.partial != nullptr)
-        GCGCN_TRY(launch_splitk_reduce(a.partial, splits, M, N, alpha, beta, C, ldc, bias, st, batch, sC));
+        GCGCN_TRY(launch_splitk_reduce(a.partial, splits, M, N, alpha, beta, C, ldc, bias, st));
     *taken = 1;
     return GCGCN_OK;
 }
@@ -863,7 +1043,7 @@
     a.M = M; a.N = N; a.K = K; a.lda = lda; a.ldb = ldb; a.ldc = 0;
     a.A = A; a.B = B; a.bias = nullptr; a.C = nullptr; a.partial = nullptr; a.alpha = 1.f; a.beta = 0.f;
     a.tiles_m = ceil_div(M, TC_BM); a.tiles_n = N / TC_BN; a.k_splits = 1; a.k_per_split = K;
-    a.kblocks = ceil_div(K, TC_BK); a.batch = 1; a.sA = a.sB = a.sC = 0; a.Apre = nullptr;
+    a.kblocks = ceil_div(K, TC_BK); a.Apre = nullptr;
     a.rd_t = T; a.rd_out = out; a.rd_ld = ld; a.bscale = nullptr; a.lds = 0; a.seq_k = 0;
     const size_t blob_total = static_cast<size_t>(a.tiles_n) * a.kblocks * TC_B_BLOB_BYTES;
     if (ws == nullptr || blob_total > ws_bytes || (reinterpret_cast<uintptr_t>(ws) & 15) != 0)
@@ -886,4 +1066,50 @@
     return GCGCN_OK;
 }
 
-}
+int launch_wgrad_group(const WgradProblem* list, int count, int K, void* ws, size_t ws_bytes, cudaStream_t st) {
+    WgArgs g{};
+    double flops = 0.0;
+    int tiles = 0;
+    for (int i = 0; i < count; ++i) {
+        const WgradProblem& q = list[i];
+        if (q.C == nullptr || q.M <= 0 || q.N <= 0 || q.heads <= 0) continue;
+        if (g.count == WG_MAX) return fail(GCGCN_ERR_INVALID_ARG, "wgrad_group: more than %d problems", WG_MAX);
+        WgDesc& d = g.p[g.count++];
+        d.A = q.A; d.B = q.B; d.C = q.C; d.lda = q.lda; d.ldb = q.ldb; d.ldc = q.ldc; d.M = q.M; d.N = q.N;
+        d.sA = q.sA; d.sB = q.sB; d.sC = q.sC; d.alpha = q.alpha; d.beta = q.beta;
+        d.pack = q.heads % 2 == 0 && q.M <= 64 && q.N <= 64;
+        d.vec = q.lda % 4 == 0 && q.ldb % 4 == 0 && (q.heads == 1 || (q.sA % 4 == 0 && q.sB % 4 == 0)) &&
+                (reinterpret_cast<uintptr_t>(q.A) & 15) == 0 && (reinterpret_cast<uintptr_t>(q.B) & 15) == 0;
+        d.tiles_m = ceil_div(q.M, TC_BM); d.tiles_n = ceil_div(q.N, TC_BN);
+        d.tile0 = tiles;
+        tiles += d.pack ? q.heads / 2 : q.heads * d.tiles_m * d.tiles_n;
+        flops += 2.0 * q.M * q.N * K * q.heads;
+    }
+    if (g.count == 0) return GCGCN_OK;
+    const int sms = sm_count();
+    int splits = 0;
+    g.k_per_split = TC_BK;
+    if (K > 0) {
+        splits = std::max(1, std::min(sms / tiles, ceil_div(K, TC_BK)));
+        g.k_per_split = ceil_div(ceil_div(K, splits), TC_BK) * TC_BK;
+        splits = ceil_div(K, g.k_per_split);
+    }
+    g.K = K; g.tiles = tiles; g.splits = splits;
+    const size_t need = static_cast<size_t>(tiles) * splits * WG_PART_FLOATS * sizeof(float);
+    if (ws == nullptr || need > ws_bytes || (reinterpret_cast<uintptr_t>(ws) & 15) != 0)
+        return fail(GCGCN_ERR_WORKSPACE, "wgrad_group: %zu bytes of workspace needed for %d tiles x %d K slices", need, tiles,
+                    splits);
+    g.partial = static_cast<float*>(ws);
+    if (splits > 0) {
+        static std::atomic<unsigned long long> prepared{0};
+        GCGCN_TRY(set_smem_once(prepared, wgrad_group_kernel, TC_SMEM_BYTES, "wgrad_group smem"));
+        wgrad_group_kernel<<<std::min(sms, tiles * splits), tc_threads(3), TC_SMEM_BYTES, st>>>(g);
+        timing_set_work(flops);
+        GCGCN_CHECK_LAUNCH("wgrad_group");
+    }
+    wgrad_reduce_kernel<<<dim3(tiles, WG_PART_FLOATS / 4 / 256), 256, 0, st>>>(g);
+    GCGCN_CHECK_LAUNCH("wgrad_reduce");
+    return GCGCN_OK;
+}
+
+}
diff --git a/gcgcn_b200/functional.py b/gcgcn_b200/functional.py
--- a/gcgcn_b200/functional.py
+++ b/gcgcn_b200/functional.py
@@ -1,5 +1,6 @@
 from __future__ import annotations
 
+import ctypes
 from typing import Optional
 
 import torch
@@ -497,6 +498,16 @@
         return dU, dVd, None, None
 
 
+def wgrad_group(problems, K: int) -> None:
+    arr = (_lib.WgradProblem * max(1, len(problems)))()
+    for i, q in enumerate(problems):
+        for k, v in q.items():
+            setattr(arr[i], k, v)
+    dev = torch.device("cuda", torch.cuda.current_device())
+    ws = workspace(dev, (24 << 20) + 4096)
+    _lib.call("gcgcn_wgrad_group", ctypes.addressof(arr), len(problems), K, ws.data_ptr(), ws.numel(), _stream(dev))
+
+
 def gemm(a: torch.Tensor, b: torch.Tensor, trans_a=False, trans_b=False, bias=None,
          out: Optional[torch.Tensor] = None, alpha=1.0, beta=0.0) -> torch.Tensor:
     a, b = _cuda(a, "A"), _cuda(b, "B")
diff --git a/include/gcgcn_b200.h b/include/gcgcn_b200.h
--- a/include/gcgcn_b200.h
+++ b/include/gcgcn_b200.h
@@ -287,6 +287,16 @@
                const float* A, int32_t lda, const float* B, int32_t ldb, float beta, float* C,
                int32_t ldc, const float* bias, void* ws, size_t ws_bytes, void* stream);
 
+typedef struct gcgcn_wgrad_problem {
+    const float* A;
+    const float* B;
+    float* C;
+    int32_t lda, ldb, ldc, M, N, heads;
+    int64_t sA, sB, sC;
+    float alpha, beta;
+} gcgcn_wgrad_problem;
+int gcgcn_wgrad_group(const gcgcn_wgrad_problem* list, int32_t count, int32_t K, void* ws, size_t ws_bytes, void* stream);
+
 #ifdef __cplusplus
 }
 #endif
```
